# Iasonaspg/GPU-Randomized-Block-Lanczos

Measured on AMD Instinct MI355X. Metric: RBL iters/sec + time-to-k=20 eigenpairs, n=1e7 nnz/row=100 b=32; 1/2/4/8 GPU, higher is better.
Workload: dtype f64

## Files before the change

gpu-randomized-block-lanczos_amd/csrc/kernels.hpp:

```cpp
#pragma once
#include "rbl_common.hpp"

namespace rbl {

struct Panels {
  static constexpr int kMax = 2;
  const double* ptr[kMax] = {nullptr, nullptr};
  int count = 0;
  int w = 0;
};
struct PanelRun {
  const double* base = nullptr;
  const float* base32 = nullptr;
  int64_t stride = 0;
  int count = 0;
  int w = 0;
};

constexpr int64_t kCsrPad = 256;
constexpr int64_t kRowPad = 16;
constexpr int64_t kRowPad32 = 32;

struct CsrDev {
  int64_t nrows = 0;
  int64_t nnz = 0;
  const int64_t* rowptr = nullptr;
  const int32_t* col = nullptr;
  const double* val = nullptr;
  const int64_t* tile_cmin = nullptr;
  const int64_t* tile_cmax = nullptr;
  const int64_t* tile_info = nullptr;
  int64_t ntiles = 0;
  int64_t tiles_per_wg = 0;
  const int32_t* panel_blk = nullptr;
  const uint16_t* panel_cnt = nullptr;
  const uint32_t* panel_st = nullptr;
  const uint8_t* panel_col = nullptr;
  const double* panel_val = nullptr;
  int64_t panel_nblk = 0;
  int panel_rpg = 4;
  int panel_ch = 32;
  bool panel_auto = false;
  bool window_ok16 = false;
  bool window_ok32 = false;
  bool band_ok16 = false;
  bool band_ok32 = false;
  bool band_gram = false;
  bool band_pair = false;
  int64_t row0 = 0;
  const uint16_t* band_pos = nullptr;
  const double* bt = nullptr;
  int bt_ng = 0;
  int64_t bt_tiles_per_wg = 0;
  int64_t q_lo = 0, q_hi = 0;
  const double* zrow = nullptr;
  const void* qloc = nullptr;
  int64_t loc_lo = 0, loc_hi = 0;
  const double* lfix_c = nullptr;
  double* lfix_q = nullptr;
  int* two_wave = nullptr;
  int64_t lfix_lo = 0, lfix_hi = 0;
  const uint64_t* btp_hdr = nullptr;
  const double* btp_val = nullptr;
  const double* bth = nullptr;
  const double* bte = nullptr;
  int64_t seg_ntasks = 0;
  const int64_t* seg_trow = nullptr;
  const int32_t* seg_tinfo = nullptr;
  const int64_t* seg_slot_k0 = nullptr;
  int64_t seg_nlong = 0;
  const int64_t* seg_lrow = nullptr;
  const int64_t* seg_lslot = nullptr;
  double* seg_scratch = nullptr;
  int seg_ntiers = 0;
  bool seg_split = false;
  hipEvent_t seg_wait = nullptr;
  struct Tier {
    const int64_t* rowptr = nullptr;
    const int32_t* col = nullptr;
    const double* val = nullptr;
    int64_t ntasks = 0, nlong = 0;
    const int64_t* trow = nullptr;
    const int32_t* tinfo = nullptr;
    const int64_t* slot_k0 = nullptr;
    const int64_t* lrow = nullptr;
    const int64_t* lslot = nullptr;
    double* scratch = nullptr;
  } seg_tier[3];
};
constexpr int kMaxSegTiers = 3;
constexpr int64_t kSegLen = 4096;
constexpr int64_t kSegPack = 512;

bool rowgram_ok(int b);
int rowgram_grid(int64_t nrows, int per_cu = 2);
constexpr int kRowgramMaxPerCu = 4;
void rowgram(int64_t nrows, int b, const double* X, const double* C, int ldc, double* Y,
             double alpha, double beta, double* slab, int grid, const int* skip, hipStream_t s,
             const float* X32 = nullptr, float* Y32 = nullptr, const int* f64flag = nullptr,
             bool tri = false);
struct RowOpArgs {
  const double* X = nullptr;
  const double* C = nullptr;
  int ldc = 0;
  double* Y = nullptr;
  double alpha = 1.0, beta = 0.0;
  double* slab = nullptr;
  const int* skip = nullptr;
  const float* X32 = nullptr;
  float* Y32 = nullptr;
  const int* f64flag = nullptr;
  const double* C2 = nullptr;
  const double* Z = nullptr;
  double* slab2 = nullptr;
// ... 3 lines not shown
};
bool rowgram_ex(int64_t nrows, int b, const RowOpArgs& a, int grid, hipStream_t s);

int spmm(const CsrDev& A, const double* Qin, int64_t col_off, int b, double* U,
         const double* Qprev, const double* Bi, int variant, hipStream_t s,
         double* ai_slab = nullptr);

bool spmm_seg_ok(const CsrDev& A, int b);
void seg_tier_count(int64_t m, const int64_t* rowptr, const int32_t* col, const uint8_t* tier_of,
                    int ntiers, int32_t* cnt, hipStream_t s);
void seg_tier_fill(int64_t m, const int64_t* rowptr, const int32_t* col, const double* val,
                   const uint8_t* tier_of, int ntiers, int64_t* const* trp, int32_t* const* tcol,
                   double* const* tval, hipStream_t s);
struct TierRule {
  const int32_t* deg = nullptr;
  int64_t row0 = 0, r0 = 0, r1 = 0;
};
void seg_tier_count_rule(int64_t m, const int64_t* rowptr, const int32_t* col, TierRule rule,
                         int32_t* cnt, hipStream_t s);
void seg_tier_fill_rule(int64_t m, const int64_t* rowptr, const int32_t* col, const double* val,
                        TierRule rule, int64_t* const* trp, int32_t* const* tcol,
                        double* const* tval, hipStream_t s);
void spmm_seg_tier(const CsrDev::Tier& T, const double* Q, int64_t col_off, int b, double* out,
                   hipStream_t s);
void push_add(const int64_t* rows, const int64_t* ptr, const int64_t* slot, int64_t nrows,
              const double* recv, int b, double* U, hipStream_t s);
constexpr int64_t kRectSegLen = 1024;
constexpr int64_t kRectPack = 512;
int rect_transpose(int64_t rows, int64_t cols, int64_t nnz, const int64_t* ptr, const int32_t* ind,
                   const double* val, int64_t* tptr, int32_t* tind, double* tval, hipStream_t s);
void spmm_rect(const CsrDev::Tier& T, const double* Q, int b, double* out, const double* Qprev,
               const double* Bi, const double* scale, hipStream_t s, const double* sa = nullptr,
               const double* sw = nullptr);
int rect_colsum_grid(int64_t rows, int b);
void rect_colsum(int64_t rows, int b, const double* a, const double* X, double* part, double* w,
                 hipStream_t s);
bool spmm_panel(const CsrDev& A, const double* Qin, int64_t col_off, int b, double* U,
                const double* Qprev, const double* Bi, hipStream_t s);
int panel_width();
int panel_format(const CsrDev& A, const int32_t* binfo, int R, int64_t nblk, uint16_t* cnt,
                 uint32_t* st, int64_t ncnt, uint8_t* pcol, double* pval, hipStream_t s);
bool spmm_window(const CsrDev& A, const double* Qin, int64_t col_off, int b, double* U,
                 const double* Qprev, const double* Bi, hipStream_t s);
int window_grid();
void ensure_lds_attr(const void* kernel, int bytes);
bool spmm_band(const CsrDev& A, const double* Qin, int64_t col_off, int b, double* U,
               const double* Qprev, const double* Bi, hipStream_t s, double* ai_slab = nullptr,
               int* ai_parts = nullptr);
bool spmm_bt_locfix_ok(const CsrDev& A, int b);
int spmm_bt_halfwidth(const CsrDev& A);
void spmm_bt_locfix_edges(const CsrDev& A, double* Q, const double* Qprev, const double* C,
                          int64_t lo0, int64_t hi0, int64_t lo1, int64_t hi1, hipStream_t s);
void spmm_bt_locfix_rest(const CsrDev& A, double* Q, const double* Qprev, const double* C,
                         hipStream_t s);
bool spmm_bt(const CsrDev& A, const double* Qin, int64_t col_off, int b, double* U,
             const double* Qprev, const double* Bi, hipStream_t s, double* ai_slab = nullptr,
             int* ai_parts = nullptr, const float* Q32 = nullptr, const float* Qprev32 = nullptr);
int bt_half(const double* full, int64_t ntiles, int64_t tpw, int NG, double** half,
            double** edge, hipStream_t s);
int64_t bt_tile_slots(int64_t ntiles, int64_t tiles_per_wg);
void bt_fill(const CsrDev& A, int H, int NG, double* out, hipStream_t s);
constexpr int bt_pack_words(int NG) { return (4 * NG + (2 * NG + 4) / 4 + 2) & ~1; }
int bt_pack(const double* dense, int64_t nslots, int NG, uint64_t* hdr, double** val_out,
            int64_t* nval_out, hipStream_t s);
constexpr int kWindowTileRows = 16;
constexpr int kBandMaxK = 176;
constexpr int kBandLd = 196;
constexpr int kBandRing = 256;
void band_positions(const CsrDev& A, uint16_t* pos, hipStream_t s);

void cheb_axpby(int64_t len, const double* W, const double* Y, const double* Z, double alpha,
                double beta, double gamma, double* out, hipStream_t s);
void cheb_series_term(int64_t len, const double* W, const double* T1, const double* T2, double alpha,
                      double beta, double mu, double mu0, double* Tout, double* ACC, bool first,
                      bool last, hipStream_t s);
int moment_grid(int64_t nrows, int b);
void cheb_moment_term(int64_t nrows, int b, const double* W, const double* T1, const double* T2,
                      double alpha, double beta, double* Tout, double* part, int grid, bool first,
                      bool last, hipStream_t s);
int resid_grid(int64_t nrows);
void resid_partial(int64_t nrows, int kp, const double* Z, const double* X, const double* theta,
                   double* part, int grid, hipStream_t s);
void copy_cols(int64_t nrows, int w, const double* src, int lds, int s0, double* dst, int ldd, int d0,
               hipStream_t s);

int lr_padded_width(int r);
int lr_project_grid(int64_t rows, int b, int rp);
void lr_project(int64_t rows, int b, int rp, const double* P, const double* X, double* part,
                double* w, hipStream_t s);
void lr_small(int r, int rp, int b, const double* S, const double* w, double* c, hipStream_t s);
void lr_update(int64_t rows, int b, int rp, const double* P, const double* c, double* U,
               hipStream_t s);

int gram_splits(int64_t nrows, int nW, int w, int xcols);
void gram_partial(int64_t nrows, const PanelRun& W, const Panels& X, double* slab, int splits,
                  const int* skip, hipStream_t s);
void reduce_slab(const double* slab, int splits, int64_t len, double* out, const int* skip,
                 hipStream_t s);
int reduce_scratch_splits(int splits);
void reduce_slab_many(double* slab, int splits, int64_t len, double* out, hipStream_t s);
void tsmm(int64_t nrows, const PanelRun& X, const double* C, int ldc, const Panels& Y,
          double alpha, double beta, const int* skip, hipStream_t s, double* xslab = nullptr,
          int* xgrid = nullptr);

bool gram44_ok(int64_t nrows, int nW, int w, int xcount, int xw);
int gram44_splits(int64_t nrows, int nW, int w = 32);
void gram44_partial(int64_t nrows, const PanelRun& W, const Panels& X, double* slab, int splits,
                    const int* skip, hipStream_t s);
bool tsmm44_ok(int xw, int ky, int yw);
void tsmm44_f32x(int64_t nrows, const PanelRun& X, const double* C, int ldc, const Panels& Y,
                 double alpha, double beta, hipStream_t s);
int tsmm44_xg_grid(int64_t nrows);
void tsmm44(int64_t nrows, const PanelRun& X, const double* C, int ldc, const Panels& Y,
            double alpha, double beta, const int* skip, hipStream_t s, double* xslab = nullptr,
            int* xgrid = nullptr);

int gram32_splits(int64_t nrows);
void gram32_partial(int64_t nrows, const float* Wb, int64_t wstride, int nW, int w, const float* X0,
                    const float* X1, int xcount, double* slab, int splits, hipStream_t s);
void tsmm32(int64_t nrows, const float* Xb, int64_t xstride, int nX, int w, const double* C, int ldc,
            float* Y0, float* Y1, int ycount, float alpha, float beta, hipStream_t s);
void cvt_f32_to_f64(const float* src, double* dst, int64_t n, hipStream_t s);
void cvt_f64_to_f32(const double* src, float* dst, int64_t n, hipStream_t s);

void chol_step(const double* G, int b, int64_t nglobal, int mode, double* R, double* Rinv,
               double* Rtot, int* need3, int* status, const int* skip, hipStream_t s,
               double* scratch);
void copy_small(const double* src, double* dst, int64_t len, hipStream_t s, const int* skip = nullptr);
void cloc_rinv(double* C, const double* Rinv, int b, const int* skip, hipStream_t s);
void transpose_small(const double* src, double* dst, int b, hipStream_t s);
void stash_step(const double* Ai, const double* Rtot, double* Bprev, int* flags, double* stash,
                int b, hipStream_t s);

struct RmatParams {
  int64_t n = 0;
  int scale = 0;
  int64_t edges = 0;
  double a = 0.57, b = 0.19, c = 0.19;
  uint64_t seed = 0;
  bool relabel = false;
  Scatter perm;
};
constexpr uint64_t kRelabelK = 0x52454C4142454C31ull;
void rmat_degree(const RmatParams& p, int32_t* deg, hipStream_t s);
int rmat_local_csr(const RmatParams& p, int64_t r0, int64_t r1, int64_t max_keys, int nplant,
                   const double* plant_dev, int64_t* rowptr_dev, int32_t** col_dev,
                   double** val_dev, int64_t* nnz_out, hipStream_t s);
void col_footprint(const int32_t* col, int64_t nnz, const int64_t* bounds_dev, int P,
                   unsigned long long* lo, unsigned long long* hi, hipStream_t s);

void circ_count(int64_t n, int64_t width, double p, uint64_t seed, int64_t r0, int64_t r1,
                int32_t* counts, hipStream_t s);
void circ_fill(int64_t n, int64_t width, double p, uint64_t seed, int64_t r0, int64_t r1,
               const int64_t* rowptr, int nplant, const double* plant_dev, int32_t* col,
               double* val, hipStream_t s);
void gather_rows(const double* Q, const int32_t* idx, int64_t nrows, int b, double* out,
                 hipStream_t s);
void mark_cols(const int32_t* col, int64_t nnz, int64_t r0, int64_t r1, uint8_t* mark,
               hipStream_t s);
void remap_cols(int32_t* col, int64_t nnz, const int32_t* map, hipStream_t s);
void hw_count(int64_t n, int64_t W, double p, uint64_t seed, int64_t r0, int64_t r1,
              int32_t* counts, hipStream_t s);
void hw_fill(int64_t n, int64_t W, double p, uint64_t seed, int64_t r0, int64_t r1,
             const int64_t* rowptr, int nplant, const double* plant_dev, int32_t* col,
             double* val, hipStream_t s);
void randn_block(double* Q, int64_t nrows, int b, int64_t r0, uint64_t seed, hipStream_t s,
                 const Scatter* perm = nullptr);
void tile_col_range(const CsrDev& A, int tile_rows, int64_t* cmin, int64_t* cmax, hipStream_t s);
void colmajor_to_rowmajor(const double* src, int64_t nrows, int w, double* dst, hipStream_t s);
void rowmajor_to_colmajor(const double* src, int64_t nrows, int w, double* dst, hipStream_t s);

}
```

gpu-randomized-block-lanczos_amd/csrc/rbl_api.cpp:

```cpp
#include <hip/hip_runtime.h>
#include <rocprofiler-sdk-roctx/roctx.h>

#include <algorithm>
#include <cstdlib>
#include <chrono>
#include <cmath>
#include <cstdio>
#include <cstring>
#include <string>
#include <thread>
#include <vector>

#include "../../include/rbl_hip.h"
#include "comm.hpp"
#include "kernels.hpp"

using namespace rbl;

struct rbl_ctx {
  int device = 0;
  hipStream_t stream = nullptr;
  int nranks = 1, rank = 0;
  Comm* comm = nullptr;
  std::string err;
// ... 116 lines not shown
  std::vector<void*> h_spill;
  double* d_stage = nullptr;
  hipStream_t cstream = nullptr;
  hipEvent_t ev_fin = nullptr, ev_d2h[2] = {nullptr, nullptr};
  std::vector<hipEvent_t> step_ev;
  bool d2h_pending[2] = {false, false};
  float* d_basis32 = nullptr;
  float* d_stage32 = nullptr;
  double* d_Qi64 = nullptr;
  double* d_Qm64 = nullptr;
  double* d_U = nullptr;
  double* d_T = nullptr;
  int64_t T_cols = 0;
  double* d_qext = nullptr;
  size_t qext_cap = 0;
  double* d_slab = nullptr;
  size_t slab_elems = 0;
  double* d_C = nullptr;
  size_t C_elems = 0;
  double* d_small = nullptr;
  int* d_flags = nullptr;
  double* h_pin = nullptr;
  void* h_d2h[2] = {nullptr, nullptr};
  hipEvent_t ev_d2h_slot[2] = {nullptr, nullptr};
  hipStream_t rstream = nullptr;
  hipEvent_t ev_ritz[9] = {};
  double* h_hist = nullptr;
  double* d_stash = nullptr;
  bool stash_direct = true;
  double* dv_pin = nullptr;
  double* dv_hist = nullptr;
  bool flags_clean = false;
  int fetched = 1;
  bool have_bprev = false;
  double* d_lock = nullptr;
  int nlock = 0, lock_cap = 0;
  int filt_deg = 0;
  double filt_lo = 0.0, filt_hi = 0.0, filt_ref = 0.0;
  double* d_filt[3] = {nullptr, nullptr, nullptr};
  int filt_cols = 0;
  std::vector<double> ser_mu;
  double ser_lo = 0.0, ser_hi = 0.0;
  double* d_rv = nullptr;
  double* d_rw = nullptr;
  int ritz_k = 0;

  int timers = 0;
  int reorth_order = 0;
  int spmm_variant = 0;
  int fuse = 7;
  int cloc_step = 0;
  bool cloc_final = false;
  std::vector<int> step_flags;
  double stage_ms[RBL_NUM_STAGES] = {0};
  int64_t comm_stats[RBL_COMM_NSTATS] = {0};
  int64_t comm_host_ns[2] = {0, 0};
  double comm_dev_ms[2] = {0.0, 0.0};
  int64_t path_stats[RBL_PATH_NSTATS] = {0};
  struct Mark { int stage; hipEvent_t a, b; int parent = -1; };
  std::vector<Mark> marks;
  struct OpenStage { int stage; hipStream_t st; };
  std::vector<OpenStage> open_stages;
  std::vector<hipEvent_t> ev_pool;
  size_t ev_used = 0;
};

namespace {

const char* kStageNames[RBL_NUM_STAGES] = {"AQ", "3-term", "qr", "part reorth", "loc reorth",
                                           "Ritz vectors", "comm", "spill wait"};

int fail(rbl_ctx* c, int code, const std::string& msg) {
  if (c) c->err = msg;
  return code;
}

struct DevBuf {
  void* p = nullptr;
  DevBuf() = default;
  DevBuf(const DevBuf&) = delete;
  DevBuf& operator=(const DevBuf&) = delete;
  ~DevBuf() {
    if (p) (void)hipFree(p);
  }
  double* d() const { return static_cast<double*>(p); }
};

#define HIPC(expr)                                                                    \
  do {                                                                                \
    hipError_t _e = (expr);                                                           \
    if (_e != hipSuccess)                                                             \
      return fail(ctx, _e == hipErrorOutOfMemory ? RBL_ERR_OOM : RBL_ERR_HIP,          \
                  std::string(#expr) + ": " + hipGetErrorString(_e));                 \
  } while (0)
#define COMMC(expr)               \
  do {                            \
    int _s = (expr);              \
    if (_s < 0) return _s;        \
  } while (0)
#define CHK(expr)             \
  do {                        \
    int _s = (expr);          \
    if (_s < 0) return _s;    \
  } while (0)

double* slotp(rbl_ctx* ctx, int j) {
// ... 1110 lines not shown
  hipFree(ctx->d_qext);
  ctx->d_qext = nullptr;
  ctx->qext_cap = 0;
  HIPC(hipMalloc(&ctx->d_qext, need * sizeof(double)));
  HIPC(hipMemsetAsync(ctx->d_qext, 0, need * sizeof(double), st));
  ctx->qext_cap = need;
  return RBL_OK;
}

int apply_A_stored(rbl_ctx* ctx, const double* Qin, int64_t off, int b, double* U, const double* Qprev,
                   const double* Bi, double* slab, const double* qloc, const double* lfix_c,
                   double* lfix_q, int64_t lf_lo, int64_t lf_hi, hipEvent_t seg_wait) {
  if (ctx->nloc <= 0) return 0;
  if (ctx->rect) {
    CHK(ensure_rect_y(ctx, b));
    const double* Q = Qin + (0 - off) * b;
    if (ctx->rect_shift) {
      double *t = ctx->d_rect_ts, *sv = ctx->d_rect_ts + b;
      rect_colsum(ctx->n, b, ctx->d_shift_v, Q, ctx->d_rect_part, t, ctx->stream);
      spmm_rect(rect_tier(ctx, 0), Q, b, ctx->d_rect_y, nullptr, nullptr, nullptr, ctx->stream,
                ctx->d_shift_u, t);
      rect_colsum(ctx->rect_m, b, ctx->d_shift_u, ctx->d_rect_y, ctx->d_rect_part, sv, ctx->stream);
      spmm_rect(rect_tier(ctx, 1), ctx->d_rect_y, b, U, Qprev, Bi, nullptr, ctx->stream,
                ctx->d_shift_v, sv);
      ctx->path_stats[RBL_PATH_SPMM] += 1;
      return 0;
    }
    spmm_rect(rect_tier(ctx, 0), Q, b, ctx->d_rect_y, nullptr, nullptr, nullptr, ctx->stream);
    spmm_rect(rect_tier(ctx, 1), ctx->d_rect_y, b, U, Qprev, Bi, nullptr, ctx->stream);
    ctx->path_stats[RBL_PATH_SPMM] += 1;
    return 0;
  }
  if (ctx->csr_dropped && rbl_spmm_kernel_for(ctx, b) != 5)
    return fail(ctx, RBL_ERR_STATE, "the CSR was released (RBL_OPT_KEEP_CSR = 0): only the band-tile "
                                    "SpMM (b in {16, 32}) can run");
  if (!ctx->dense) {
    CsrDev A = csr(ctx);
    if (!qloc && ctx->ghost_active && ctx->nranks > 1 && rbl_spmm_kernel_for(ctx, b) == 6)
      qloc = ctx->ghost_local;
    if (qloc) {
      A.qloc = qloc;
      A.loc_lo = ctx->r0;
      A.loc_hi = ctx->r0 + ctx->nloc;
    }
    A.seg_wait = seg_wait;
    int two_wave = 0;
    A.two_wave = &two_wave;
    if (lfix_c) {
      A.lfix_c = lfix_c;
      A.lfix_q = lfix_q;
      A.lfix_lo = lf_lo;
      A.lfix_hi = lf_hi;
    }
    const int parts = spmm(A, Qin, off, b, U, Qprev, Bi, ctx->spmm_variant, ctx->stream, slab);
    if (parts < 0) return fail(ctx, RBL_ERR_INVALID, "internal: split-source SpMM needs the band-tile kernel");
    ctx->path_stats[RBL_PATH_SPMM] += 1;
    ctx->path_stats[RBL_PATH_SPMM_TWO_WAVE] += two_wave;
    if (lfix_c) {
      ctx->path_stats[RBL_PATH_SPMM_LOC_FUSED] += 1;
      ctx->path_stats[RBL_PATH_LOCFIX_REST] += 1;
      StageScope t(ctx, RBL_STAGE_LOC_REORTH);
      spmm_bt_locfix_rest(A, lfix_q, Qprev, lfix_c, ctx->stream);
    }
    return parts;
  }
  if (b > ctx->qfull_cols) {
    hipFree(ctx->d_qfull);
    ctx->d_qfull = nullptr;
    ctx->qfull_cols = 0;
    HIPC(hipMalloc(&ctx->d_qfull, (size_t)ctx->dense_panels * 32 * b * sizeof(double)));
    HIPC(hipMemsetAsync(ctx->d_qfull, 0, (size_t)ctx->dense_panels * 32 * b * sizeof(double), ctx->stream));
    ctx->qfull_cols = b;
  }
  HIPC(hipMemcpyAsync(ctx->d_qfull, Qin + (0 - off) * b, ctx->n * b * sizeof(double),
                      hipMemcpyDeviceToDevice, ctx->stream));
  PanelRun X;
  X.base = ctx->d_dense;
  X.stride = ctx->nloc * 32;
  X.w = 32;
  X.count = (int)ctx->dense_panels;
  CHK(tsmm_checked(ctx, X, ctx->d_qfull, b, pan1(U, b), 1.0, 0.0, nullptr));
  if (Qprev) {
    transpose_small(Bi, smallp(ctx, S_BT), b, ctx->stream);
    CHK(tsmm_checked(ctx, run1(Qprev, b), smallp(ctx, S_BT), b, pan1(U, b), -1.0, 1.0, nullptr));
  }
  return 0;
}

int ensure_lr_bufs(rbl_ctx* ctx, int b) {
  if (ctx->d_lr_wc && ctx->lr_cols >= b) return RBL_OK;
  HIPC(hipStreamSynchronize(ctx->stream));
  hipFree(ctx->d_lr_wc);
  hipFree(ctx->d_lr_part);
  ctx->d_lr_wc = ctx->d_lr_part = nullptr;
  ctx->lr_cols = 0;
  const size_t grid = (size_t)lr_project_grid(ctx->nloc, b, ctx->lr_rp);
  HIPC(hipMalloc(&ctx->d_lr_wc, (size_t)2 * ctx->lr_rp * b * sizeof(double)));
  HIPC(hipMalloc(&ctx->d_lr_part, grid * ctx->lr_rp * b * sizeof(double)));
  ctx->lr_cols = b;
  return RBL_OK;
}

int apply_A(rbl_ctx* ctx, const double* Qin, int64_t off, int b, double* U, const double* Qprev,
            const double* Bi, double* slab, const double* qloc = nullptr,
            const double* lfix_c = nullptr, double* lfix_q = nullptr, int64_t lf_lo = 0,
            int64_t lf_hi = 0, hipEvent_t seg_wait = nullptr) {
  if (ctx->lr_r == 0 || ctx->nloc <= 0)
    return apply_A_stored(ctx, Qin, off, b, U, Qprev, Bi, slab, qloc, lfix_c, lfix_q, lf_lo, lf_hi,
                          seg_wait);
  if (ctx->nranks > 1 || ctx->rect)
    return fail(ctx, RBL_ERR_STATE, "internal: a low-rank update needs one rank and a square A");
  CHK(ensure_lr_bufs(ctx, b));
  const int parts = apply_A_stored(ctx, Qin, off, b, U, Qprev, Bi, lfix_c ? slab : nullptr, qloc,
                                   lfix_c, lfix_q, lf_lo, lf_hi, seg_wait);
  if (parts < 0) return parts;
// ... 212 lines not shown
    PanelRun X;
    X.base32 = slotp32(ctx, 0);
    X.stride = ctx->slot;
    X.count = nres;
    X.w = b;
    tsmm44_f32x(ctx->nloc, X, d_S, kcols, pan1(Y, kcols), 1.0, 0.0, ctx->stream);
    HIPC(hipGetLastError());
    j0 = nres;
  }
  if (j0 < nblocks) CHK(ensure_qm64(ctx));
  for (int j = j0; j < nblocks; ++j) {
    int st = 0;
    const float* Qj = block_dev32(ctx, j, ctx->nblocks, &st);
    if (st) return fail(ctx, st, "Ritz: H2D of a spilled block failed");
    cvt_f32_to_f64(Qj, ctx->d_Qm64, ctx->nloc * b, ctx->stream);
    CHK(tsmm_checked(ctx, run1(ctx->d_Qm64, b), d_S + (int64_t)j * b * kcols, kcols, pan1(Y, kcols),
                     1.0, j == 0 ? 0.0 : 1.0, nullptr));
  }
  return RBL_OK;
}

int gram32(rbl_ctx* ctx, const float* Wb, int nW, const float* X0, const float* X1, int xcount,
           double* C) {
  const int b = ctx->b;
  const int splits = gram32_splits(ctx->nloc);
  const int64_t len = (int64_t)nW * b * xcount * b;
  if ((size_t)splits * len > ctx->slab_elems)
    return fail(ctx, RBL_ERR_INVALID, "internal: Gram slab too small (fp32)");
  if (ctx->nloc > 0) {
    gram32_partial(ctx->nloc, Wb, ctx->slot, nW, b, X0, X1, xcount, ctx->d_slab, splits, ctx->stream);
    reduce_slab(ctx->d_slab, splits, len, C, nullptr, ctx->stream);
  } else {
    HIPC(hipMemsetAsync(C, 0, len * sizeof(double), ctx->stream));
  }
  HIPC(hipGetLastError());
  return allreduce(ctx, C, (size_t)len);
}
int upd32(rbl_ctx* ctx, const float* Xb, int nX, const double* C, int ldc, float* Y0, float* Y1,
          int ycount) {
  if (ctx->nloc <= 0) return RBL_OK;
  tsmm32(ctx->nloc, Xb, ctx->slot, nX, ctx->b, C, ldc, Y0, Y1, ycount, -1.f, 1.f, ctx->stream);
  HIPC(hipGetLastError());
  return RBL_OK;
}

int rowop_ex(rbl_ctx* ctx, RowOpArgs a, double* G, double* Gx, bool reduce_x, bool comm_x = true) {
  const int b = ctx->b;
  const int gmax = rowgram_grid(ctx->nloc, kRowgramMaxPerCu);
  if ((size_t)2 * gmax * b * b > ctx->slab_elems)
    return fail(ctx, RBL_ERR_INVALID, "internal: row-op slab too small");
  if (G) a.slab = ctx->d_slab;
  if (a.Z) a.slab2 = ctx->d_slab + (size_t)gmax * b * b;
  const int xgrid = rowgram_grid(ctx->nloc, 2);
  int grid = a.Z ? xgrid : 0;
  a.grid_out = &grid;
  if (ctx->nloc > 0) {
    if (!rowgram_ex(ctx->nloc, b, a, grid, ctx->stream))
      return fail(ctx, RBL_ERR_INVALID, "internal: unsupported fused row-op form");
  } else {
    grid = 1;
    if (G) HIPC(hipMemsetAsync(a.slab, 0, (size_t)b * b * sizeof(double), ctx->stream));
    if (a.Z && a.skip == nullptr)
      HIPC(hipMemsetAsync(a.slab2, 0, (size_t)xgrid * b * b * sizeof(double), ctx->stream));
  }
  HIPC(hipGetLastError());
  if (G) {
    reduce_slab(ctx->d_slab, grid, (int64_t)b * b, G, a.skip, ctx->stream);
    CHK(allreduce(ctx, G, (size_t)b * b));
  }
  if (Gx && reduce_x) {
    reduce_slab(ctx->d_slab + (size_t)gmax * b * b, xgrid, (int64_t)b * b, Gx, nullptr, ctx->stream);
    if (comm_x) CHK(allreduce(ctx, Gx, (size_t)b * b));
  }
  return RBL_OK;
}

int tsqr(rbl_ctx* ctx, const double* U, double* Qout, bool g1_ready = false, float* Qout32 = nullptr,
         const double* Zloc = nullptr) {
  StageScope t(ctx, RBL_STAGE_QR);
  ctx->flags_clean = false;
  const int b = ctx->b;
  int* need3 = ctx->d_flags;
  int* status = ctx->d_flags + 2;
  double* G = smallp(ctx, S_G);
  const int* skip3 = need3 + 1;
  const bool fused = rowgram_ok(b);
  auto apply_inplace = [&](const int* skip) -> int {
    if (b <= 64)
      return tsmm_checked(ctx, run1(Qout, b), smallp(ctx, S_RINV), b, pan1(Qout, b), 1.0, 0.0, skip);
    CHK(tsmm_checked(ctx, run1(Qout, b), smallp(ctx, S_RINV), b, pan1(ctx->d_T, b), 1.0, 0.0, skip));
    copy_small(ctx->d_T, Qout, ctx->nloc * b, ctx->stream, skip);
    return RBL_OK;
  };
  const bool three = fused && (ctx->fuse & 1);
  if (!g1_ready) CHK(gram(ctx, run1(U, b), pan1(U, b), G, nullptr));
  chol_step(G, b, ctx->n, 0, smallp(ctx, S_R), smallp(ctx, three ? S_RINV1 : S_RINV), smallp(ctx, S_RTOT),
            need3, status, nullptr, ctx->stream, smallp(ctx, S_CHS0));
  if (three) {
    RowOpArgs a1;
    a1.X = U;
    a1.C = smallp(ctx, S_RINV1);
    a1.ldc = b;
    a1.mode = 1;
    a1.tri = true;
    CHK(rowop_ex(ctx, a1, G, nullptr, false));
    chol_step(G, b, ctx->n, 1, smallp(ctx, S_R), smallp(ctx, S_RINV), smallp(ctx, S_RTOT), need3,
              status, nullptr, ctx->stream, smallp(ctx, S_CHS0));
    RowOpArgs a2;
    a2.X = U;
    a2.C = smallp(ctx, S_RINV1);
    a2.C2 = smallp(ctx, S_RINV);
    a2.ldc = b;
    a2.tri = true;
    a2.Y = Qout;
    a2.Y32 = Qout32;
    a2.f64flag = Qout32 ? need3 : nullptr;
    a2.Z = Zloc;
    a2.mode = 2;
    CHK(rowop_ex(ctx, a2, nullptr, Zloc ? smallp(ctx, S_CLOC) : nullptr, Zloc != nullptr, false));
    CHK(gram(ctx, run1(Qout, b), pan1(Qout, b), G, skip3, Zloc == nullptr));
    if (Zloc) CHK(allreduce(ctx, G, (size_t)2 * b * b));
    chol_step(G, b, ctx->n, 1, smallp(ctx, S_R), smallp(ctx, S_RINV), smallp(ctx, S_RTOT), need3,
              status, skip3, ctx->stream, smallp(ctx, S_CHS0));
    RowOpArgs a3;
    a3.X = Qout;
    a3.C = smallp(ctx, S_RINV);
    a3.ldc = b;
    a3.tri = true;
    a3.Y = Qout;
    a3.skip = skip3;
    a3.Y32 = Qout32;
    a3.mode = 0;
    CHK(rowop_ex(ctx, a3, nullptr, nullptr, false));
    if (Zloc) cloc_rinv(smallp(ctx, S_CLOC), smallp(ctx, S_RINV), b, skip3, ctx->stream);
    HIPC(hipGetLastError());
    return RBL_OK;
  }
  if (Zloc) return fail(ctx, RBL_ERR_INVALID, "internal: local-reorth Gram fusion needs the 3-pass QR");
  if (fused) {
    CHK(rowop(ctx, U, smallp(ctx, S_RINV), Qout, 1.0, 0.0, G, nullptr, nullptr, nullptr, nullptr, true));
  } else {
    CHK(tsmm_checked(ctx, run1(U, b), smallp(ctx, S_RINV), b, pan1(Qout, b), 1.0, 0.0, nullptr));
    CHK(gram(ctx, run1(Qout, b), pan1(Qout, b), G, nullptr));
  }
  chol_step(G, b, ctx->n, 1, smallp(ctx, S_R), smallp(ctx, S_RINV), smallp(ctx, S_RTOT), need3,
            status, nullptr, ctx->stream, smallp(ctx, S_CHS0));
  if (fused) {
    CHK(rowop(ctx, Qout, smallp(ctx, S_RINV), Qout, 1.0, 0.0, G, nullptr, nullptr, Qout32,
              Qout32 ? need3 : nullptr, true));
  } else {
    CHK(apply_inplace(nullptr));
    CHK(gram(ctx, run1(Qout, b), pan1(Qout, b), G, skip3));
  }
  chol_step(G, b, ctx->n, 1, smallp(ctx, S_R), smallp(ctx, S_RINV), smallp(ctx, S_RTOT), need3,
            status, skip3, ctx->stream, smallp(ctx, S_CHS0));
  if (fused) {
    CHK(rowop(ctx, Qout, smallp(ctx, S_RINV), Qout, 1.0, 0.0, nullptr, skip3, nullptr, Qout32,
              nullptr, true));
  } else {
    CHK(apply_inplace(skip3));
    if (Qout32) cvt_f64_to_f32(Qout, Qout32, ctx->nloc * b, ctx->stream);
  }
  HIPC(hipGetLastError());
  return RBL_OK;
}

int halo_exchange(rbl_ctx* ctx, const double* Q, const double** Qin, int64_t* off,
                  bool copy_local = true, hipStream_t st = nullptr) {
  if (ctx->nranks == 1) {
    *Qin = Q;
    *off = 0;
    return RBL_OK;
  }
  if (!st) st = ctx->stream;
  StageScope t(ctx, RBL_STAGE_COMM, st);
  const int b = ctx->b;
  CHK(ensure_qext(ctx, b, st));
  double* ext = ctx->d_qext;
  ctx->ghost_active = use_ghost(ctx, b);
  if (ctx->ghost_active) {
    gather_rows(Q, ctx->d_send_idx, ctx->n_send, b, ctx->d_sendbuf, st);
    HIPC(hipGetLastError());
    std::vector<Comm::Xfer> x(ctx->nranks);
    for (int q = 0; q < ctx->nranks; ++q) {
      if (q == ctx->rank) continue;
      x[q].send = ctx->d_sendbuf + ctx->send_off[q] * b;
      x[q].nsend = (size_t)ctx->send_cnt[q] * b;
      x[q].recv = ext + ctx->ghost_off[q] * b;
      x[q].nrecv = (size_t)ctx->ghost_cnt[q] * b;
    }
    CHK(exchange(ctx, x, st));
    ctx->ghost_local = Q;
    *Qin = ext;
    *off = 0;
    return RBL_OK;
  }
  if (copy_local)
    HIPC(hipMemcpyAsync(ext + (ctx->r0 - ctx->ext_lo) * b, Q, ctx->nloc * b * sizeof(double),
                        hipMemcpyDeviceToDevice, st));
  std::vector<Comm::Xfer> x(ctx->nranks);
  for (int q = 0; q < ctx->nranks; ++q) {
    if (q == ctx->rank) continue;
    const int64_t gl = ctx->give_lo[q], gh = ctx->give_hi[q];
    if (gh > gl) {
      x[q].send = Q + (gl - ctx->r0) * b;
      x[q].nsend = (size_t)(gh - gl) * b;
    }
    const int64_t nl = ctx->need_lo[q], nh = ctx->need_hi[q];
    if (nh > nl) {
      x[q].recv = ext + (nl - ctx->ext_lo) * b;
      x[q].nrecv = (size_t)(nh - nl) * b;
    }
  }
  CHK(exchange(ctx, x, st));
  *Qin = ext;
  *off = ctx->ext_lo;
  return RBL_OK;
}

// ... 76 lines not shown
  return RBL_OK;
}

int push_products(rbl_ctx* ctx, const double* Q, int b, hipStream_t st) {
  StageScope t(ctx, RBL_STAGE_AQ, st);
  CHK(ensure_push(ctx, b));
  const auto& P = ctx->push_tier;
  CsrDev::Tier T;
  T.rowptr = P.rowptr;
  T.col = P.col;
  T.val = P.val;
  T.ntasks = P.ntasks;
  T.nlong = P.nlong;
  T.trow = P.trow;
  T.tinfo = P.tinfo;
  T.slot_k0 = P.slot_k0;
  T.lrow = P.lrow;
  T.lslot = P.lslot;
  T.scratch = P.scratch;
  spmm_seg_tier(T, Q, ctx->r0, b, ctx->d_pushbuf, st);
  HIPC(hipGetLastError());
  return RBL_OK;
}

int push_exchange(rbl_ctx* ctx, int b, hipStream_t st) {
  StageScope t(ctx, RBL_STAGE_COMM, st);
  std::vector<Comm::Xfer> x(ctx->nranks);
  for (int q = 0; q < ctx->nranks; ++q) {
    if (q == ctx->rank) continue;
    x[q].send = ctx->d_pushbuf + ctx->ghost_off[q] * b;
    x[q].nsend = (size_t)ctx->ghost_cnt[q] * b;
    x[q].recv = ctx->d_precv + ctx->send_off[q] * b;
    x[q].nrecv = (size_t)ctx->send_cnt[q] * b;
  }
  CHK(exchange(ctx, x, st));
  return RBL_OK;
}

int push_finish(rbl_ctx* ctx, double* U, int b, hipStream_t st) {
  StageScope t(ctx, RBL_STAGE_AQ, st);
  push_add(ctx->d_ps_rows, ctx->d_ps_ptr, ctx->d_ps_slot, ctx->n_ps_rows, ctx->d_precv, b, U, st);
  HIPC(hipGetLastError());
  return RBL_OK;
}

int push_halo(rbl_ctx* ctx, const double* Q, int b, double* U) {
  if (!push_on(ctx)) return RBL_OK;
  CHK(push_products(ctx, Q, b, ctx->stream));
  CHK(push_exchange(ctx, b, ctx->stream));
  return push_finish(ctx, U, b, ctx->stream);
}

void free_run(rbl_ctx* ctx) {
  if (ctx->cstream) hipStreamSynchronize(ctx->cstream);
  hipFree(ctx->d_basis); ctx->d_basis = nullptr;
  for (void* h : ctx->h_spill)
    if (h) hipHostFree(h);
  ctx->h_spill.clear();
  hipFree(ctx->d_stage); ctx->d_stage = nullptr;
  ctx->resident = INT32_MAX;
  ctx->d2h_pending[0] = ctx->d2h_pending[1] = false;
  hipFree(ctx->d_basis32); ctx->d_basis32 = nullptr;
  hipFree(ctx->d_stage32); ctx->d_stage32 = nullptr;
  hipFree(ctx->d_Qi64); ctx->d_Qi64 = nullptr;
  hipFree(ctx->d_Qm64); ctx->d_Qm64 = nullptr;
  ctx->basis_bits = 64;
  hipFree(ctx->d_U); ctx->d_U = nullptr;
  hipFree(ctx->d_T); ctx->d_T = nullptr;
  hipFree(ctx->d_qext); ctx->d_qext = nullptr; ctx->qext_cap = 0;
  hipFree(ctx->d_sendbuf); ctx->d_sendbuf = nullptr;
  if (ctx->hstream) hipStreamSynchronize(ctx->hstream);
  hipFree(ctx->d_pushbuf); ctx->d_pushbuf = nullptr;
  hipFree(ctx->d_precv); ctx->d_precv = nullptr;
  ctx->push_cap = 0;
  hipFree(ctx->d_slab); ctx->d_slab = nullptr;
  hipFree(ctx->d_C); ctx->d_C = nullptr;
  hipFree(ctx->d_small); ctx->d_small = nullptr;
  hipFree(ctx->d_flags); ctx->d_flags = nullptr;
  hipFree(ctx->d_lock); ctx->d_lock = nullptr;
  ctx->nlock = ctx->lock_cap = 0;
  hipFree(ctx->d_filt[0]); hipFree(ctx->d_filt[1]); hipFree(ctx->d_filt[2]);
  ctx->d_filt[0] = ctx->d_filt[1] = ctx->d_filt[2] = nullptr;
  ctx->filt_cols = 0;
  hipFree(ctx->d_rv); ctx->d_rv = nullptr;
  hipFree(ctx->d_rw); ctx->d_rw = nullptr;
  ctx->ritz_k = 0;
  if (ctx->h_pin) hipHostFree(ctx->h_pin);
  ctx->h_pin = nullptr;
  if (ctx->h_hist) hipHostFree(ctx->h_hist);
  ctx->h_hist = nullptr;
  hipFree(ctx->d_stash);
  ctx->d_stash = nullptr;
  ctx->dv_pin = ctx->dv_hist = nullptr;
  ctx->nblocks = 0;
  ctx->b = 0;
  ctx->have_bprev = false;
}

void free_rect_shift(rbl_ctx* ctx) {
  hipFree(ctx->d_shift_u); ctx->d_shift_u = nullptr;
  hipFree(ctx->d_shift_v); ctx->d_shift_v = nullptr;
  hipFree(ctx->d_rect_ts); ctx->d_rect_ts = nullptr;
  hipFree(ctx->d_rect_part); ctx->d_rect_part = nullptr;
  ctx->rect_ts_cols = 0;
  ctx->rect_shift = false;
}
// ... 331 lines not shown
  const char* name = "none";
  if (ctx->comm) {
    hipSetDevice(ctx->device);
    const int s = ctx->comm->count(&cnt, &ctx->err);
    if (s < 0) return s;
    name = ctx->comm->name();
  }
  *nranks = cnt;
  *rank = ctx->rank;
  if (transport && transport_len > 0) snprintf(transport, (size_t)transport_len, "%s", name);
  return RBL_OK;
}

int rbl_rccl_version(int* version, char* path, int path_len) {
  if (!version) return RBL_ERR_INVALID;
  std::string p, err;
  const int s = rbl::rccl_library(version, &p, &err);
  if (path && path_len > 0) snprintf(path, (size_t)path_len, "%s", s ? err.c_str() : p.c_str());
  return s ? RBL_ERR_RCCL : RBL_OK;
}

int rbl_set_option(rbl_ctx* ctx, int option, int64_t value) {
  if (!ctx) return RBL_ERR_INVALID;
  switch (option) {
    case RBL_OPT_TIMERS:
      if (value < 0 || value > 2) return fail(ctx, RBL_ERR_INVALID, "RBL_OPT_TIMERS: 0, 1 or 2");
      ctx->timers = (int)value;
      return RBL_OK;
    case RBL_OPT_REORTH_ORDER:
      if (value < 0 || value > 1) return fail(ctx, RBL_ERR_INVALID, "reorth order must be 0|1");
      ctx->reorth_order = (int)value;
      return RBL_OK;
    case RBL_OPT_DEVICE_BLOCKS:
      if (value < -1 || value == 1 || value == 2 || value > INT32_MAX)
        return fail(ctx, RBL_ERR_INVALID, "device blocks: 0 (all), -1 (auto) or >= 3");
      ctx->dev_blocks_opt = (int)value;
      return RBL_OK;
    case RBL_OPT_SPMM_KERNEL:
      if (value < 0 || value > 7 || value == 4)
        return fail(ctx, RBL_ERR_INVALID, "spmm kernel must be 0 (auto) or a kernel id 1, 2, 3, 5, 6, 7");
      ctx->spmm_variant = value == 5 ? 4 : value == 6 ? 5 : (int)value;
      return RBL_OK;
    case RBL_OPT_SPLIT_HALO: ctx->split_halo = value != 0; return RBL_OK;
    case RBL_OPT_HALO_OVERLAP: ctx->halo_overlap = value != 0; return RBL_OK;
    case RBL_OPT_HALO_PUSH:
      if (value < 0 || value > 2) return fail(ctx, RBL_ERR_INVALID, "RBL_OPT_HALO_PUSH must be 0|1|2");
      ctx->halo_push_opt = (int)value;
      return RBL_OK;
    case RBL_OPT_KEEP_CSR: ctx->keep_csr = value != 0; return RBL_OK;
    case RBL_OPT_RELABEL:
      if (value < 0 || value > 1) return fail(ctx, RBL_ERR_INVALID, "RBL_OPT_RELABEL must be 0|1");
      ctx->relabel_opt = (int)value;
      return RBL_OK;
    case RBL_OPT_FUSE:
      if (value < 0 || value > 7) return fail(ctx, RBL_ERR_INVALID, "RBL_OPT_FUSE is a 3-bit mask");
      ctx->fuse = (int)value;
      return RBL_OK;
    default: return fail(ctx, RBL_ERR_INVALID, "unknown option");
  }
}

int rbl_set_matrix_csc(rbl_ctx* ctx, int64_t n, int64_t nnz, const int64_t* colptr,
                       const int64_t* rowval, const double* nzval, int index_base) {
  if (!ctx || n < 1 || nnz < 0 || !colptr || (nnz && (!rowval || !nzval)) ||
      (index_base != 0 && index_base != 1))
    return fail(ctx, RBL_ERR_INVALID, "rbl_set_matrix_csc: bad arguments");
  if (colptr[n] - colptr[0] != nnz) return fail(ctx, RBL_ERR_INVALID, "colptr[n] != nnz");
  HIPC(hipSetDevice(ctx->device));
  std::vector<int64_t> rp(n + 1);
  for (int64_t i = 0; i <= n; ++i) rp[i] = colptr[i] - colptr[0];
  ctx->bounds.assign(ctx->nranks + 1, 0);
  rbl_plan_row_partition(n, rp.data(), ctx->nranks, ctx->bounds.data());
  const int64_t r0 = ctx->bounds[ctx->rank], r1 = ctx->bounds[ctx->rank + 1];
  return upload_csr(ctx, n, r0, r1, colptr + r0, rowval, nzval, index_base, index_base);
}

int rbl_set_matrix_csr_rows(rbl_ctx* ctx, int64_t n, int64_t row_begin, int64_t row_end,
                            const int64_t* rowptr, const int64_t* colind, const double* val,
                            int index_base) {
  if (!ctx || n < 1 || row_begin < 0 || row_end < row_begin || row_end > n || !rowptr ||
      (index_base != 0 && index_base != 1))
    return fail(ctx, RBL_ERR_INVALID, "rbl_set_matrix_csr_rows: bad arguments");
  HIPC(hipSetDevice(ctx->device));
  if (ctx->nranks > 1) {
    int64_t mine[2] = {row_begin, row_end};
    std::vector<int64_t> all(2 * ctx->nranks);
    COMMC(ctx->comm->allgather_host(mine, all.data(), 2, ctx->stream, &ctx->err));
    ctx->bounds.assign(ctx->nranks + 1, 0);
    for (int p = 0; p < ctx->nranks; ++p) {
      if (all[2 * p] != (p == 0 ? 0 : all[2 * p - 1]))
        return fail(ctx, RBL_ERR_INVALID, "row slices must tile [0,n) in rank order");
      ctx->bounds[p + 1] = all[2 * p + 1];
    }
    if (ctx->bounds[ctx->nranks] != n) return fail(ctx, RBL_ERR_INVALID, "row slices != n");
  } else {
    if (row_begin != 0 || row_end != n)
      return fail(ctx, RBL_ERR_INVALID, "single rank must own all rows");
    ctx->bounds = {0, n};
  }
  return upload_csr(ctx, n, row_begin, row_end, rowptr, colind, val, index_base, index_base);
}

int rbl_set_matrix_dense(rbl_ctx* ctx, int64_t n, int64_t row_begin, int64_t row_end,
                         const double* A, int64_t lda) {
  if (!ctx || n < 1 || row_begin < 0 || row_end < row_begin || row_end > n || !A ||
      lda < row_end - row_begin || lda < 1)
// ... 501 lines not shown
    double* keep_send = ctx->d_sendbuf;
    const int keep_b = ctx->b;
    ctx->d_qext = ext.d();
    ctx->qext_cap = (size_t)ext_rows * b;
    ctx->d_sendbuf = sendbuf.d();
    ctx->b = b;
    const int st = halo_exchange(ctx, xr.d(), &Qin, &off);
    ctx->d_qext = keep_ext;
    ctx->qext_cap = keep_cap;
    ctx->d_sendbuf = keep_send;
    ctx->b = keep_b;
    if (st < 0) return st;
  }
  {
    const int st = apply_A(ctx, Qin, off, b, y.d(), nullptr, nullptr, nullptr);
    if (st < 0) return st;
  }
  HIPC(hipGetLastError());
  CHK(push_halo(ctx, xr.d(), b, y.d()));
  rowmajor_to_colmajor(y.d(), ctx->nloc, b, x.d(), ctx->stream);
  HIPC(hipMemcpyAsync(Y, x.p, ctx->nloc * b * sizeof(double), hipMemcpyDeviceToHost, ctx->stream));
  HIPC(hipStreamSynchronize(ctx->stream));
  return RBL_OK;
}

int rbl_start(rbl_ctx* ctx, int b, int max_blocks, int basis_bits, const double* omega,
              uint64_t seed) {
  if (!ctx) return RBL_ERR_INVALID;
  if (!has_matrix(ctx)) return fail(ctx, RBL_ERR_STATE, "rbl_start: no matrix");
  if (b < 1 || b > RBL_MAX_BLOCK)
    return fail(ctx, RBL_ERR_INVALID, "block size must be in [1," + std::to_string(RBL_MAX_BLOCK) + "]");
  if (max_blocks < 1) return fail(ctx, RBL_ERR_INVALID, "max_blocks must be >= 1");
  if (basis_bits != 64 && basis_bits != 32)
    return fail(ctx, RBL_ERR_INVALID, "basis_bits must be 64 or 32");
  if (ctx->rect && basis_bits != 64)
    return fail(ctx, RBL_ERR_INVALID, "rbl_start: a rectangular B (rbl_set_matrix_normal) needs the "
                                      "fp64 basis (basis_bits = 64)");
  if (ctx->filt_deg > 0 && basis_bits != 64)
    return fail(ctx, RBL_ERR_INVALID, "rbl_start: a Chebyshev filter (rbl_set_filter) needs the fp64 "
                                      "basis (basis_bits = 64)");
  if (ctx->filt_deg > 0 && (ctx->rect || ctx->nranks > 1))
    return fail(ctx, RBL_ERR_INVALID, "rbl_start: a Chebyshev filter (rbl_set_filter) runs on one rank "
                                      "and a square A only");
  if (ctx->lr_r > 0 && basis_bits != 64)
    return fail(ctx, RBL_ERR_INVALID, "rbl_start: a low-rank update (rbl_set_lowrank) needs the fp64 "
                                      "basis (basis_bits = 64)");
  if (has_series(ctx) && basis_bits != 64)
    return fail(ctx, RBL_ERR_INVALID, "rbl_start: a Chebyshev series (rbl_set_filter_series) needs the "
                                      "fp64 basis (basis_bits = 64)");
  if (has_series(ctx) && (ctx->rect || ctx->nranks > 1))
    return fail(ctx, RBL_ERR_INVALID, "rbl_start: a Chebyshev series (rbl_set_filter_series) runs on "
                                      "one rank and a square A only");
  HIPC(hipSetDevice(ctx->device));
  HIPC(hipStreamSynchronize(ctx->stream));
  int dev_slots = max_blocks + 1;
  const bool same_shape = (ctx->d_basis || ctx->d_basis32) && ctx->b == b &&
                          ctx->max_blocks == max_blocks && ctx->slot == ctx->nloc * b &&
                          ctx->basis_bits == basis_bits;
  const int cur_slots = ctx->resident == INT32_MAX ? ctx->max_blocks + 1 : ctx->resident + 2;
  if (ctx->dev_blocks_opt < 0 && same_shape && ctx->auto_planned) {
    dev_slots = cur_slots;
  } else if (ctx->dev_blocks_opt != 0) {
    int g = ctx->dev_blocks_opt;
    if (g < 0) {
      size_t fr = 0, tot = 0;
      HIPC(hipMemGetInfo(&fr, &tot));
      const double blk64 = (double)std::max<int64_t>(ctx->nloc, 1) * b * 8.0;
      const double blk = blk64 * (basis_bits == 64 ? 1.0 : 0.5);
      const double mine = ctx->d_basis ? (double)(ctx->resident == INT32_MAX ? ctx->max_blocks + 1 : ctx->resident + 2) * blk64
                        : ctx->d_basis32 ? (double)(ctx->resident == INT32_MAX ? ctx->max_blocks + 1 : ctx->resident + 2) * blk64 * 0.5
                        : 0.0;
      const double work = 2.0 + (ctx->nranks > 1 ? 1.0 : 0.0) +
                          (basis_bits == 32 ? 1.0 + (direct32_ok(ctx, b) ? 0.0 : 1.0) : 0.0);
      const double other = work * blk64 + blk + 8.0 * (double)gram_slab_elems(ctx, b, max_blocks, basis_bits);
      g = (int)std::max(3.0, std::floor((0.8 * ((double)fr + mine) - other) / blk));
    }
    dev_slots = std::min(dev_slots, std::max(3, g));
  }
  const bool reuse = same_shape && cur_slots == dev_slots;
  ctx->nlock = 0;
  ctx->cloc_step = 0;
  ctx->step_flags.clear();
  const int alloc_st = [&]() -> int {
  if (reuse) {
    ctx->nblocks = 0;
    if (ctx->cstream) HIPC(hipStreamSynchronize(ctx->cstream));
    ctx->d2h_pending[0] = ctx->d2h_pending[1] = false;
    HIPC(hipMemsetAsync(ctx->d_flags, 0, 4 * sizeof(int), ctx->stream));
  } else {
  free_run(ctx);
  ctx->b = b;
  ctx->max_blocks = max_blocks;
  ctx->slot = ctx->nloc * b;
  const int64_t nl = std::max<int64_t>(ctx->nloc, 1);
  ctx->basis_bits = basis_bits;
  ctx->auto_planned = ctx->dev_blocks_opt < 0;
  if (basis_bits == 64) {
    HIPC(hipMalloc(&ctx->d_basis, (size_t)dev_slots * nl * b * sizeof(double)));
    if (dev_slots < max_blocks + 1) {
      ctx->resident = dev_slots - 2;
      ctx->h_spill.assign(max_blocks + 1 - ctx->resident, nullptr);
      HIPC(hipMalloc(&ctx->d_stage, (size_t)nl * b * sizeof(double)));
      if (!ctx->cstream) {
        HIPC(hipStreamCreateWithFlags(&ctx->cstream, hipStreamNonBlocking));
        HIPC(hipEventCreateWithFlags(&ctx->ev_fin, hipEventDisableTiming));
        HIPC(hipEventCreateWithFlags(&ctx->ev_d2h[0], hipEventDisableTiming));
        HIPC(hipEventCreateWithFlags(&ctx->ev_d2h[1], hipEventDisableTiming));
      }
    }
  } else {
    const size_t bytes32 = ((size_t)dev_slots * nl + kRowPad32) * b * sizeof(float);
    HIPC(hipMalloc(&ctx->d_basis32, bytes32));
    HIPC(hipMemsetAsync(ctx->d_basis32, 0, bytes32, ctx->stream));
    if (dev_slots < max_blocks + 1) {
      ctx->resident = dev_slots - 2;
      ctx->h_spill.assign(max_blocks + 1 - ctx->resident, nullptr);
      HIPC(hipMalloc(&ctx->d_stage32, ((size_t)nl + kRowPad32) * b * sizeof(float)));
      HIPC(hipMemsetAsync(ctx->d_stage32, 0, ((size_t)nl + kRowPad32) * b * sizeof(float), ctx->stream));
      if (!ctx->cstream) {
        HIPC(hipStreamCreateWithFlags(&ctx->cstream, hipStreamNonBlocking));
        HIPC(hipEventCreateWithFlags(&ctx->ev_fin, hipEventDisableTiming));
        HIPC(hipEventCreateWithFlags(&ctx->ev_d2h[0], hipEventDisableTiming));
        HIPC(hipEventCreateWithFlags(&ctx->ev_d2h[1], hipEventDisableTiming));
      }
    }
    HIPC(hipMalloc(&ctx->d_Qi64, (nl + kRowPad) * b * sizeof(double)));
    if (!direct32_ok(ctx, b)) HIPC(hipMalloc(&ctx->d_Qm64, (nl + kRowPad) * b * sizeof(double)));
  }
  HIPC(hipMalloc(&ctx->d_U, (nl + kRowPad) * b * sizeof(double)));
  ctx->T_cols = b;
  HIPC(hipMalloc(&ctx->d_T, nl * b * sizeof(double)));
  if (ctx->nranks > 1) {
    CHK(ensure_qext(ctx, b, ctx->stream));
    if (ctx->ghost)
      HIPC(hipMalloc(&ctx->d_sendbuf, std::max<int64_t>(ctx->n_send, 1) * b * sizeof(double)));
  }
  const size_t slab = gram_slab_elems(ctx, b, max_blocks, basis_bits);
  ctx->slab_elems = slab;
  HIPC(hipMalloc(&ctx->d_slab, slab * sizeof(double)));
  ctx->C_elems = (size_t)std::max(1, max_blocks) * b * 2 * b;
  HIPC(hipMalloc(&ctx->d_C, ctx->C_elems * sizeof(double)));
  HIPC(hipMalloc(&ctx->d_small, (size_t)S_NSMALL * b * b * sizeof(double)));
  HIPC(hipMalloc(&ctx->d_flags, 4 * sizeof(int)));
  HIPC(hipMemset(ctx->d_flags, 0, 4 * sizeof(int)));
  {
#ifdef RBL_VARIANTS
    const char* e = std::getenv("RBL_STASH_COPY");
    ctx->stash_direct = !(e && std::atoi(e) == 1);
#else
    ctx->stash_direct = true;
#endif
    const unsigned hf = ctx->stash_direct ? (hipHostMallocMapped | hipHostMallocCoherent) : hipHostMallocDefault;
    HIPC(hipHostMalloc(&ctx->h_pin, stash_rec(b) * sizeof(double), hf));
    HIPC(hipHostMalloc(&ctx->h_hist, (size_t)(max_blocks + 2) * stash_rec(b) * sizeof(double), hf));
    if ((size_t)ctx->nloc * b * sizeof(double) >= 4 * kD2HPiece && !d2h_direct()) {
      CHK(ensure_d2h_slots(ctx));
      CHK(ensure_ritz_stream(ctx));
    }
    if (ctx->stash_direct) {
      HIPC(hipHostGetDevicePointer(reinterpret_cast<void**>(&ctx->dv_pin), ctx->h_pin, 0));
      HIPC(hipHostGetDevicePointer(reinterpret_cast<void**>(&ctx->dv_hist), ctx->h_hist, 0));
    } else {
      HIPC(hipMalloc(&ctx->d_stash, stash_rec(b) * sizeof(double)));
    }
  }
  }
  if (ctx->push && ctx->nranks > 1 && use_ghost(ctx, b)) {
    const char* inj = std::getenv("RBL_FAULT_PUSH_ALLOC");
    if (inj && *inj && std::atoi(inj) == ctx->rank)
      return fail(ctx, RBL_ERR_OOM, "rbl_start: push buffers (injected by RBL_FAULT_PUSH_ALLOC)");
    CHK(ensure_push(ctx, b));
  }
  if (has_filter(ctx)) CHK(ensure_filter_bufs(ctx, b));
  return RBL_OK;
  }();
  if (ctx->nranks > 1) {
    const int64_t mine = alloc_st;
    std::vector<int64_t> all(ctx->nranks);
    COMMC(ctx->comm->allgather_host(&mine, all.data(), 1, ctx->stream, &ctx->err));
    int bad = -1;
    for (int q = 0; q < ctx->nranks && bad < 0; ++q)
      if (all[q] != RBL_OK) bad = q;
    if (bad >= 0) {
      (void)hipGetLastError();
      free_run(ctx);
      if (alloc_st != RBL_OK) return alloc_st;
      return fail(ctx, (int)all[bad], "rbl_start: rank " + std::to_string(bad) +
                                          " could not allocate its run buffers");
    }
  } else if (alloc_st != RBL_OK) {
    (void)hipGetLastError();
    return alloc_st;
  }

  if (omega) {
    double* d_tmp = ctx->d_U;
    HIPC(hipMemcpyAsync(d_tmp, omega, ctx->nloc * b * sizeof(double), hipMemcpyHostToDevice,
// ... 39 lines not shown
    return fail(ctx, RBL_ERR_STATE, "rbl_step: rbl_fetch the asynchronous steps first");
  const int rc = step_impl(ctx, i, part_reorth, A_out, B_out, false);
  if (ctx && rc >= 0) ctx->fetched = ctx->nblocks;
  return rc;
}
int rbl_step_async(rbl_ctx* ctx, int i, int part_reorth) {
  return step_impl(ctx, i, part_reorth, nullptr, nullptr, true);
}
int rbl_fetch(rbl_ctx* ctx, int i0, int i1, double* A_out, double* B_out, int* status_out) {
  if (!ctx) return RBL_ERR_INVALID;
  if (i0 != ctx->fetched || i1 < i0 || i1 > ctx->nblocks)
    return fail(ctx, RBL_ERR_INVALID, "rbl_fetch: [i0, i1) must start at the first unfetched step");
  HIPC(hipSetDevice(ctx->device));
  const int last = i1 - 1;
  if (last >= 1 && last < (int)ctx->step_ev.size() && ctx->step_ev[last])
    HIPC(hipEventSynchronize(ctx->step_ev[last]));
  else
    HIPC(hipStreamSynchronize(ctx->stream));
  harvest_timers(ctx);
  const int b = ctx->b;
  int rc = RBL_OK;
  for (int j = i0; j < i1; ++j) {
    const double* h = ctx->h_hist + (size_t)j * stash_rec(b);
    const int* fl = reinterpret_cast<const int*>(h + 2 * b * b);
    double* A = A_out ? A_out + (size_t)(j - i0) * b * b : nullptr;
    double* B = B_out ? B_out + (size_t)(j - i0) * b * b : nullptr;
    for (int r = 0; r < b; ++r)
      for (int c = 0; c < b; ++c) {
        if (A) A[c * b + r] = h[r * b + c];
        if (B) B[c * b + r] = h[b * b + r * b + c];
      }
    const int st = fl[2] ? RBL_ERR_NUMERIC : fl[3] ? RBL_WARN_QR_SHIFTED : RBL_OK;
    if (status_out) status_out[j - i0] = st;
    if (st == RBL_ERR_NUMERIC && rc >= 0) rc = fail(ctx, RBL_ERR_NUMERIC, "QR breakdown (shifted CholQR failed)");
  }
  ctx->fetched = i1;
  return rc;
}
namespace {
int step_impl(rbl_ctx* ctx, int i, int part_reorth, double* A_out, double* B_out, bool async) {
  if (!ctx) return RBL_ERR_INVALID;
  if ((!ctx->d_basis && !ctx->d_basis32) || ctx->nblocks < 1) return fail(ctx, RBL_ERR_STATE, "rbl_step before rbl_start");
  if (i != ctx->nblocks) return fail(ctx, RBL_ERR_STATE, "rbl_step: i must equal the current block count");
  if (i > ctx->max_blocks) return fail(ctx, RBL_ERR_STATE, "rbl_step: basis full (max_blocks)");
  HIPC(hipSetDevice(ctx->device));
  const int b = ctx->b;
  const bool f32 = ctx->basis_bits == 32;
  if (!ctx->flags_clean) HIPC(hipMemsetAsync(ctx->d_flags, 0, 4 * sizeof(int), ctx->stream));
  ctx->flags_clean = false;
  if (f32 && (part_reorth & 2))
    return fail(ctx, RBL_ERR_INVALID, "rbl_step: locked-vector reorth needs the fp64 basis");
  const bool direct32 = f32 && i >= 2 && direct32_ok(ctx, b);
  if (f32 && !direct32) CHK(ensure_qm64(ctx));
  double* Qi = f32 ? ctx->d_Qi64 : slotp(ctx, i - 1);
  double* Qm = i >= 2 ? (f32 ? ctx->d_Qm64 : slotp(ctx, i - 2)) : nullptr;
  float* Qi32 = f32 ? slotp32(ctx, i - 1) : nullptr;
  float* Qm32 = f32 && i >= 2 ? slotp32(ctx, i - 2) : nullptr;
  if (f32) {
    if ((part_reorth & 1) && i >= 3) {
      StageScope t(ctx, RBL_STAGE_PART_REORTH);
      const int nW = i - 2;
      const int nres = std::min(nW, ctx->resident);
      if (ctx->reorth_order == 0) {
        CHK(gram32(ctx, slotp32(ctx, 0), nres, Qi32, Qm32, 2, ctx->d_C));
        CHK(upd32(ctx, slotp32(ctx, 0), nres, ctx->d_C, 2 * b, Qi32, Qm32, 2));
      } else {
        for (int j = 0; j < nres; ++j) {
          CHK(gram32(ctx, slotp32(ctx, j), 1, Qi32, Qm32, 2, ctx->d_C));
          CHK(upd32(ctx, slotp32(ctx, j), 1, ctx->d_C, 2 * b, Qi32, Qm32, 2));
        }
      }
      for (int j = nres; j < nW; ++j) {
        int st = 0;
        const float* Wj = block_dev32(ctx, j, i, &st);
        if (st) return fail(ctx, st, "partial reorth: H2D of a spilled block failed");
        CHK(gram32(ctx, Wj, 1, Qi32, Qm32, 2, ctx->d_C));
        CHK(upd32(ctx, Wj, 1, ctx->d_C, 2 * b, Qi32, Qm32, 2));
      }
    }
    if (spilled(ctx) && i >= 2 && i - 2 >= ctx->resident) {
      HIPC(hipEventRecord(ctx->ev_fin, ctx->stream));
      HIPC(hipStreamWaitEvent(ctx->cstream, ctx->ev_fin, 0));
      CHK(spill_slot(ctx, i - 2, sizeof(float)));
      HIPC(hipMemcpyAsync(ctx->h_spill[i - 2 - ctx->resident], Qm32,
                          ctx->slot * sizeof(float), hipMemcpyDeviceToHost, ctx->cstream));
      HIPC(hipEventRecord(ctx->ev_d2h[i & 1], ctx->cstream));
      ctx->d2h_pending[i & 1] = true;
    }
    if (i >= 2) {
      StageScope t(ctx, RBL_STAGE_LOC_REORTH);
      CHK(gram32(ctx, Qm32, 1, Qi32, nullptr, 1, ctx->d_C));
      CHK(upd32(ctx, Qm32, 1, ctx->d_C, b, Qi32, nullptr, 1));
      if (!direct32) {
        cvt_f32_to_f64(Qi32, ctx->d_Qi64, ctx->nloc * b, ctx->stream);
        cvt_f32_to_f64(Qm32, ctx->d_Qm64, ctx->nloc * b, ctx->stream);
      }
      HIPC(hipGetLastError());
    }
  }

  if (!f32) CHK(reorth_pair(ctx, i, part_reorth));
  if (!f32 && spilled(ctx) && i >= 2 && i - 2 >= ctx->resident) {
    HIPC(hipEventRecord(ctx->ev_fin, ctx->stream));
    HIPC(hipStreamWaitEvent(ctx->cstream, ctx->ev_fin, 0));
    CHK(spill_slot(ctx, i - 2, sizeof(double)));
    HIPC(hipMemcpyAsync(ctx->h_spill[i - 2 - ctx->resident], slotp(ctx, i - 2),
// ... 54 lines not shown
      CHK(tsmm_checked(ctx, run1(Qm, b), smallp(ctx, S_BT), b, pan1(ctx->d_U, b), -1.0, 1.0, nullptr));
    }
    HIPC(hipGetLastError());
  } else {
    const double* Qin = nullptr;
    const float* Qin32 = nullptr;
    int64_t off = 0;
    const int kid = rbl_spmm_kernel_for(ctx, b);
    const bool seg_split = !direct32 && kid == 6 && ctx->seg_split;
    const bool split = ctx->nranks > 1 && !ctx->dense &&
                       (direct32 || kid == 5 || seg_split) && ctx->split_halo;
    const bool overlap = split && seg_split && ctx->halo_overlap;
    hipEvent_t halo_ev = nullptr;
    if (overlap) {
      if (!ctx->hstream) {
        HIPC(hipStreamCreateWithFlags(&ctx->hstream, hipStreamNonBlocking));
        HIPC(hipEventCreateWithFlags(&ctx->ev_qready, hipEventDisableTiming));
        HIPC(hipEventCreateWithFlags(&ctx->ev_halo, hipEventDisableTiming));
      }
      HIPC(hipEventRecord(ctx->ev_qready, ctx->stream));
      HIPC(hipStreamWaitEvent(ctx->hstream, ctx->ev_qready, 0));
      CHK(halo_exchange(ctx, Qi, &Qin, &off, false, ctx->hstream));
      HIPC(hipEventRecord(ctx->ev_halo, ctx->hstream));
      halo_ev = ctx->ev_halo;
      if (push_on(ctx)) {
        if (!ctx->ev_push_ready) {
          HIPC(hipEventCreateWithFlags(&ctx->ev_push_ready, hipEventDisableTiming));
          HIPC(hipEventCreateWithFlags(&ctx->ev_push_done, hipEventDisableTiming));
        }
        CHK(push_products(ctx, Qi, b, ctx->stream));
        HIPC(hipEventRecord(ctx->ev_push_ready, ctx->stream));
        HIPC(hipStreamWaitEvent(ctx->hstream, ctx->ev_push_ready, 0));
        CHK(push_exchange(ctx, b, ctx->hstream));
        HIPC(hipEventRecord(ctx->ev_push_done, ctx->hstream));
        pushed = true;
      }
    } else if (direct32) {
      CHK(halo_exchange32(ctx, Qi32, &Qin32, &off, !split));
    } else {
      CHK(halo_exchange(ctx, Qi, &Qin, &off, !split));
    }
    StageScope t(ctx, RBL_STAGE_AQ);
    if (direct32) {
      CsrDev A = csr(ctx);
      if (split) {
        A.qloc = Qi32;
        A.loc_lo = ctx->r0;
        A.loc_hi = ctx->r0 + ctx->nloc;
      }
      if (!spmm_bt(A, nullptr, off, b, ctx->d_U, nullptr, smallp(ctx, S_BPREV), ctx->stream,
                   ctx->d_slab, &ai_parts, Qin32, Qm32))
        return fail(ctx, RBL_ERR_INVALID, "internal: fp32 band-tile SpMM not applicable");
    } else {
      ai_parts = apply_A(ctx, Qin, off, b, ctx->d_U, Qm, i >= 2 ? smallp(ctx, S_BPREV) : nullptr,
                         ctx->d_slab, split ? Qi : nullptr, Cloc, Qi, lf_lo, lf_hi, halo_ev);
    }
    if (ai_parts < 0) return ai_parts;
    HIPC(hipGetLastError());
    if (halo_ev) HIPC(hipStreamWaitEvent(ctx->stream, halo_ev, 0));
  }
  if (pushed) {
    HIPC(hipStreamWaitEvent(ctx->stream, ctx->ev_push_done, 0));
    CHK(push_finish(ctx, ctx->d_U, b, ctx->stream));
  } else if (!direct32 && ai_parts == 0) {
    CHK(push_halo(ctx, Qi, b, ctx->d_U));
  }
  {
    StageScope t(ctx, RBL_STAGE_3TERM);
    if (ai_parts > 0) {
      reduce_slab(ctx->d_slab, ai_parts, (int64_t)b * b, smallp(ctx, S_AI), nullptr, ctx->stream);
      HIPC(hipGetLastError());
      CHK(allreduce(ctx, smallp(ctx, S_AI), (size_t)b * b));
    } else {
      CHK(gram(ctx, run1(Qi, b), pan1(ctx->d_U, b), smallp(ctx, S_AI), nullptr));
    }
    if (fused)
      CHK(rowop(ctx, Qi, smallp(ctx, S_AI), ctx->d_U, -1.0, 1.0, smallp(ctx, S_G), nullptr,
                direct32 ? Qi32 : nullptr));
    else
      CHK(tsmm_checked(ctx, run1(Qi, b), smallp(ctx, S_AI), b, pan1(ctx->d_U, b), -1.0, 1.0, nullptr));
  }
  if (ctx->d2h_pending[i & 1]) {
    StageScope t(ctx, RBL_STAGE_SPILL_WAIT);
    HIPC(hipStreamWaitEvent(ctx->stream, ctx->ev_d2h[i & 1], 0));
    ctx->d2h_pending[i & 1] = false;
  }
  if (!f32) {
    const int guess = i >= 2 ? ctx->step_flags[i - 1] : 0;
    const bool zfuse = fused && (ctx->fuse & 3) == 3 && !modifies(i + 1, guess) && i + 1 <= ctx->max_blocks;
    CHK(tsqr(ctx, ctx->d_U, slotp(ctx, i), fused, nullptr, zfuse ? Qi : nullptr));
    if (zfuse) {
      ctx->cloc_step = i + 1;
      ctx->cloc_final = false;
    }
  } else {
    CHK(tsqr(ctx, ctx->d_U, ctx->d_Qi64, fused, slotp32(ctx, i)));
  }
  const size_t rec = stash_rec(b);
  double* rec_dev = !ctx->stash_direct ? ctx->d_stash
                    : async            ? ctx->dv_hist + (size_t)i * rec
                                       : ctx->dv_pin;
  stash_step(smallp(ctx, S_AI), smallp(ctx, S_RTOT), smallp(ctx, S_BPREV), ctx->d_flags, rec_dev,
             b, ctx->stream);
  ctx->flags_clean = true;
  if (async) {
    if (!ctx->stash_direct)
      HIPC(hipMemcpyAsync(ctx->h_hist + (size_t)i * rec, ctx->d_stash, rec * sizeof(double),
                          hipMemcpyDeviceToHost, ctx->stream));
    if ((int)ctx->step_ev.size() <= i) ctx->step_ev.resize(i + 1, nullptr);
    if (!ctx->step_ev[i]) HIPC(hipEventCreateWithFlags(&ctx->step_ev[i], hipEventDisableTiming));
    HIPC(hipEventRecord(ctx->step_ev[i], ctx->stream));
    HIPC(hipGetLastError());
    ctx->nblocks = i + 1;
    return RBL_OK;
  }
  if (!ctx->stash_direct)
    HIPC(hipMemcpyAsync(ctx->h_pin, ctx->d_stash, rec * sizeof(double), hipMemcpyDeviceToHost, ctx->stream));
  HIPC(hipStreamSynchronize(ctx->stream));
  int flags[4];
  memcpy(flags, ctx->h_pin + 2 * b * b, sizeof(flags));
  harvest_timers(ctx);
  for (int r = 0; r < b; ++r)
    for (int c = 0; c < b; ++c) {
      if (A_out) A_out[c * b + r] = ctx->h_pin[r * b + c];
      if (B_out) B_out[c * b + r] = ctx->h_pin[b * b + r * b + c];
    }
  ctx->nblocks = i + 1;
  if (flags[2]) return fail(ctx, RBL_ERR_NUMERIC, "QR breakdown (shifted CholQR failed)");
  return flags[3] ? RBL_WARN_QR_SHIFTED : RBL_OK;
}
int d2h_staged(rbl_ctx* ctx, void* dst, const void* src, size_t bytes) {
  if (bytes < 4 * kD2HPiece || d2h_direct()) {
    HIPC(hipMemcpyAsync(dst, src, bytes, hipMemcpyDeviceToHost, ctx->stream));
    return RBL_OK;
  }
  CHK(ensure_d2h_slots(ctx));
  const unsigned hw = std::max(1u, std::thread::hardware_concurrency());
  const char* envt = std::getenv("RBL_D2H_THREADS");
  const int nthr = (int)std::min(envt ? std::max(1u, (unsigned)atoi(envt)) : 8u, hw);
  auto host_copy = [&](size_t p) {
    const size_t off = p * kD2HPiece, len = std::min(kD2HPiece, bytes - off);
    char* d = static_cast<char*>(dst) + off;
    const char* s = static_cast<const char*>(ctx->h_d2h[p & 1]);
    const size_t part = ((len + nthr - 1) / nthr + 4095) & ~size_t(4095);
    std::vector<std::thread> th;
    for (size_t o = part; o < len; o += part)
// ... 61 lines not shown
    while (p + 1 < kRitzPieces && (size_t)r0p[p + 1] * kcp * sizeof(double) <= o) ++p;
    return p;
  };
  auto scatter = [&](size_t q, size_t a, size_t e) {
    const char* slot = static_cast<const char*>(ctx->h_d2h[q & 1]);
    const size_t base = q * kD2HPiece;
    for (size_t o = base + a; o < base + e;) {
      const int p = piece_of(o);
      const int64_t r0 = r0p[p], m = r0p[p + 1] - r0;
      const size_t colb = (size_t)m * sizeof(double);
      const size_t within = o - (size_t)r0 * kcp * sizeof(double);
      const size_t c = within / colb, inr = within % colb;
      const size_t run = std::min(base + e, o + (colb - inr));
      if ((int)c < k)
        memcpy(reinterpret_cast<char*>(V_out + (int64_t)c * nl + r0) + inr, slot + (o - base), run - o);
      o = run;
    }
  };
  const unsigned hw = std::max(1u, std::thread::hardware_concurrency());
  const char* envt = std::getenv("RBL_D2H_THREADS");
  const int nthr = (int)std::min(envt ? std::max(1u, (unsigned)atoi(envt)) : 8u, hw);
  const size_t nq = (bytes + kD2HPiece - 1) / kD2HPiece;
  int waited = -1;
  for (size_t q = 0; q <= nq; ++q) {
    if (q < nq) {
      const size_t off = q * kD2HPiece, len = std::min(kD2HPiece, bytes - off);
      for (const int pl = piece_of(off + len - 1); waited < pl;)
        HIPC(hipEventSynchronize(ctx->ev_ritz[++waited]));
      HIPC(hipMemcpyAsync(ctx->h_d2h[q & 1], src + off, len, hipMemcpyDeviceToHost, ctx->stream));
      HIPC(hipEventRecord(ctx->ev_d2h_slot[q & 1], ctx->stream));
    }
    if (q > 0) {
      const size_t pq = q - 1, len = std::min(kD2HPiece, bytes - pq * kD2HPiece);
      HIPC(hipEventSynchronize(ctx->ev_d2h_slot[pq & 1]));
      const size_t part = ((len + nthr - 1) / nthr + 4095) & ~size_t(4095);
      std::vector<std::thread> th;
      for (size_t o = part; o < len; o += part)
        th.emplace_back([=, &scatter] { scatter(pq, o, std::min(len, o + part)); });
      scatter(pq, 0, std::min(part, len));
      for (auto& t : th) t.join();
    }
  }
  HIPC(hipStreamSynchronize(ctx->rstream));
  HIPC(hipStreamSynchronize(ctx->stream));
  return RBL_OK;
}
}

int rbl_ritz(rbl_ctx* ctx, int nblocks, int k, const double* S, double* V_out) {
  if (!ctx || nblocks < 1 || k < 1 || !S) return fail(ctx, RBL_ERR_INVALID, "rbl_ritz: bad arguments");
  if (nblocks > ctx->nblocks) return fail(ctx, RBL_ERR_INVALID, "rbl_ritz: more blocks than computed");
  if (k > nblocks * ctx->b) return fail(ctx, RBL_ERR_INVALID, "rbl_ritz: k > nblocks*b");
  HIPC(hipSetDevice(ctx->device));
  const int b = ctx->b;
  const int64_t rows = (int64_t)nblocks * b;
  const int64_t nl = std::max<int64_t>(ctx->nloc, 1);
  size_t free_b = 0, total_b = 0;
  HIPC(hipMemGetInfo(&free_b, &total_b));
  int kc = std::min(k, 64);
  auto chunk_bytes = [&](int w) { return (double)((w + 1) & ~1) * (double)(rows + 2 * nl) * 8.0; };
  while (kc > 1 && chunk_bytes(kc) > 0.7 * (double)free_b) kc = (kc + 1) / 2;
  const int kcp = (kc + 1) & ~1;
  if (chunk_bytes(kc) > 0.7 * (double)free_b)
    return fail(ctx, RBL_ERR_OOM, "rbl_ritz: no room for one Ritz column");
#ifdef RBL_VARIANTS
  const bool trace = std::getenv("RBL_RITZ_TRACE") != nullptr;
#else
  const bool trace = false;
#endif
  auto tnow = [] { return std::chrono::duration<double, std::milli>(
                       std::chrono::steady_clock::now().time_since_epoch()).count(); };
  const double t0 = trace ? tnow() : 0.0;
  double t_alloc = 0.0, t_comp = 0.0, t_d2h = 0.0;
  DevBuf own_S, own_V, own_Vcm;
  double *pS = nullptr, *pV = nullptr, *pVcm = nullptr;
  if (kcp <= b && ctx->d_U && ctx->d_T && ctx->d_C && (size_t)rows * kcp <= ctx->C_elems) {
    pS = ctx->d_C;
    pV = ctx->d_U;
    pVcm = ctx->d_T;
  } else {
    HIPC(hipMalloc(&own_S.p, rows * kcp * sizeof(double)));
    HIPC(hipMalloc(&own_V.p, nl * kcp * sizeof(double)));
    HIPC(hipMalloc(&own_Vcm.p, nl * kcp * sizeof(double)));
    pS = own_S.d();
    pV = own_V.d();
    pVcm = own_Vcm.d();
  }
  if (trace) t_alloc = tnow() - t0;
  const bool pipelined = V_out && ctx->nloc > 0 && kc >= k && pV == ctx->d_U &&
                         (ctx->basis_bits == 64 || tsmm44_ok(b, kcp, kcp)) &&
                         nblocks <= ctx->resident && ctx->nloc >= 64 * kRitzPieces &&
                         (size_t)ctx->nloc * kcp * sizeof(double) >= 4 * kD2HPiece &&
                         !d2h_direct() && !ritz_serial();
  std::vector<double> srm((size_t)rows * kcp);
  if (pipelined) {
    for (int64_t r = 0; r < rows; ++r)
      for (int c = 0; c < kcp; ++c) srm[(size_t)r * kcp + c] = c < k ? S[(size_t)c * rows + r] : 0.0;
    HIPC(hipMemcpyAsync(pS, srm.data(), rows * kcp * sizeof(double), hipMemcpyHostToDevice, ctx->stream));
    ctx->path_stats[RBL_PATH_RITZ_PIECES] += 1;
    CHK(ritz_pipelined(ctx, nblocks, k, kcp, pS, pV, pVcm, V_out));
    harvest_timers(ctx);
    if (trace) fprintf(stderr, "rbl_ritz: pipelined, %d row pieces, total %.2f ms\n", kRitzPieces, tnow() - t0);
    return RBL_OK;
  }
  for (int c0 = 0; c0 < k; c0 += kc) {
    const int w = std::min(kc, k - c0);
// ... 328 lines not shown
    m[2] = 2.0 * d[col] - m0;
    for (int j = 2; j <= degree; ++j) {
      const double* dj = d.data() + (size_t)3 * b + (size_t)(j - 2) * 2 * b;
      m[2 * j] = 2.0 * dj[col] - m0;
      m[2 * j - 1] = 2.0 * dj[b + col] - m1;
    }
  }
  return RBL_OK;
}

int rbl_bench_moment_pass(rbl_ctx* ctx, int64_t len_rows, int b, int reps, double* ms) {
  if (!ctx || len_rows < 1 || b < 1 || b > RBL_MAX_BLOCK || reps < 1 || !ms)
    return fail(ctx, RBL_ERR_INVALID, "rbl_bench_moment_pass: bad arguments");
  HIPC(hipSetDevice(ctx->device));
  const int grid = moment_grid(len_rows, b);
  DevBuf w, t1, t2, slab, dots;
  const size_t bytes = (size_t)len_rows * b * sizeof(double);
  for (DevBuf* p : {&w, &t1, &t2}) {
    HIPC(hipMalloc(&p->p, bytes));
    HIPC(hipMemsetAsync(p->p, 0, bytes, ctx->stream));
  }
  HIPC(hipMalloc(&slab.p, (size_t)grid * 2 * b * sizeof(double)));
  HIPC(hipMalloc(&dots.p, (size_t)2 * b * sizeof(double)));
  hipEvent_t e0 = nullptr, e1 = nullptr;
  HIPC(hipEventCreate(&e0));
  HIPC(hipEventCreate(&e1));
  auto pass = [&] {
    cheb_moment_term(len_rows, b, w.d(), t1.d(), t2.d(), 0.5, 0.25, w.d(), slab.d(), grid, false, false,
                     ctx->stream);
    reduce_slab(slab.d(), grid, (int64_t)2 * b, dots.d(), nullptr, ctx->stream);
  };
  int st = RBL_OK;
  pass();
  if (hipEventRecord(e0, ctx->stream) != hipSuccess) st = RBL_ERR_HIP;
  for (int r = 0; r < reps; ++r) pass();
  if (hipEventRecord(e1, ctx->stream) != hipSuccess || hipEventSynchronize(e1) != hipSuccess) st = RBL_ERR_HIP;
  float el = 0.f;
  if (hipEventElapsedTime(&el, e0, e1) != hipSuccess || hipGetLastError() != hipSuccess) st = RBL_ERR_HIP;
  *ms = (double)el / reps;
  (void)hipEventDestroy(e0);
  (void)hipEventDestroy(e1);
  if (st != RBL_OK) return fail(ctx, st, "rbl_bench_moment_pass: a HIP call failed");
  return RBL_OK;
}

int rbl_ritz_project(rbl_ctx* ctx, int nblocks, int k, const double* S, double* H_out) {
  if (!ctx || nblocks < 1 || k < 1 || !S || !H_out)
    return fail(ctx, RBL_ERR_INVALID, "rbl_ritz_project: bad arguments");
  if (k > RBL_MAX_BLOCK)
    return fail(ctx, RBL_ERR_INVALID, "rbl_ritz_project: k must be <= " + std::to_string(RBL_MAX_BLOCK));
  if (ctx->nranks > 1) return fail(ctx, RBL_ERR_INVALID, "rbl_ritz_project: one rank only");
  if (!ctx->d_basis && !ctx->d_basis32) return fail(ctx, RBL_ERR_STATE, "rbl_ritz_project before rbl_start");
  if (nblocks > ctx->nblocks) return fail(ctx, RBL_ERR_INVALID, "rbl_ritz_project: more blocks than computed");
  if (k > nblocks * ctx->b) return fail(ctx, RBL_ERR_INVALID, "rbl_ritz_project: k > nblocks*b");
  HIPC(hipSetDevice(ctx->device));
  HIPC(hipStreamSynchronize(ctx->stream));
  hipFree(ctx->d_rv);
  hipFree(ctx->d_rw);
  ctx->d_rv = ctx->d_rw = nullptr;
  ctx->ritz_k = 0;
  const int b = ctx->b;
  const int kp = (k + 1) & ~1;
  const int64_t rows = (int64_t)nblocks * b;
  const int64_t nl = std::max<int64_t>(ctx->nloc, 1);
  const size_t vbytes = (size_t)(nl + kRowPad) * kp * sizeof(double);
  HIPC(hipMalloc(&ctx->d_rv, vbytes));
  HIPC(hipMalloc(&ctx->d_rw, vbytes));
  HIPC(hipMemsetAsync(ctx->d_rv, 0, vbytes, ctx->stream));
  HIPC(hipMemsetAsync(ctx->d_rw, 0, vbytes, ctx->stream));
  std::vector<double> srm((size_t)rows * kp);
  for (int64_t r = 0; r < rows; ++r)
    for (int c = 0; c < kp; ++c) srm[(size_t)r * kp + c] = c < k ? S[(size_t)c * rows + r] : 0.0;
  DevBuf dS;
  HIPC(hipMalloc(&dS.p, rows * kp * sizeof(double)));
  HIPC(hipMemcpyAsync(dS.p, srm.data(), rows * kp * sizeof(double), hipMemcpyHostToDevice, ctx->stream));
  {
    StageScope t(ctx, RBL_STAGE_RITZ);
    if (ctx->basis_bits == 64) CHK(combine_blocks(ctx, nblocks, kp, dS.d(), ctx->d_rv));
    else CHK(combine_blocks32(ctx, nblocks, kp, dS.d(), ctx->d_rv));
  }
  {
    StageScope t(ctx, RBL_STAGE_AQ);
    const int cw = (b == 16 || b == 32) ? b : kp;
    if (cw == kp) {
      const int st = apply_A(ctx, ctx->d_rv, 0, kp, ctx->d_rw, nullptr, nullptr, nullptr);
      if (st < 0) return st;
    } else {
      const size_t cbytes = (size_t)(nl + kRowPad) * cw * sizeof(double);
      DevBuf xc, yc;
      HIPC(hipMalloc(&xc.p, cbytes));
      HIPC(hipMalloc(&yc.p, cbytes));
      HIPC(hipMemsetAsync(xc.p, 0, cbytes, ctx->stream));
      HIPC(hipMemsetAsync(yc.p, 0, cbytes, ctx->stream));
      for (int c0 = 0; c0 < kp; c0 += cw) {
        const int w = std::min(cw, kp - c0);
        if (w < cw && c0 > 0) HIPC(hipMemsetAsync(xc.p, 0, cbytes, ctx->stream));
        copy_cols(ctx->nloc, w, ctx->d_rv, kp, c0, xc.d(), cw, 0, ctx->stream);
        const int st = apply_A(ctx, xc.d(), 0, cw, yc.d(), nullptr, nullptr, nullptr);
        if (st < 0) return st;
        copy_cols(ctx->nloc, w, yc.d(), cw, 0, ctx->d_rw, kp, c0, ctx->stream);
      }
      HIPC(hipGetLastError());
      HIPC(hipStreamSynchronize(ctx->stream));
    }
    HIPC(hipGetLastError());
  }
  std::vector<double> h((size_t)kp * kp, 0.0);
  if (ctx->nloc > 0) {
    StageScope t(ctx, RBL_STAGE_RITZ);
    const int splits = gram_splits(ctx->nloc, 1, kp, kp);
    DevBuf slab, dH;
    HIPC(hipMalloc(&slab.p, (size_t)splits * kp * kp * sizeof(double)));
    HIPC(hipMalloc(&dH.p, (size_t)kp * kp * sizeof(double)));
    gram_partial(ctx->nloc, run1(ctx->d_rv, kp), pan1(ctx->d_rw, kp), slab.d(), splits, nullptr, ctx->stream);
    reduce_slab(slab.d(), splits, (int64_t)kp * kp, dH.d(), nullptr, ctx->stream);
    HIPC(hipGetLastError());
    HIPC(hipMemcpyAsync(h.data(), dH.p, (size_t)kp * kp * sizeof(double), hipMemcpyDeviceToHost, ctx->stream));
    HIPC(hipStreamSynchronize(ctx->stream));
  }
  HIPC(hipStreamSynchronize(ctx->stream));
  harvest_timers(ctx);
  for (int r = 0; r < k; ++r)
    for (int c = 0; c < k; ++c) H_out[(size_t)c * k + r] = h[(size_t)r * kp + c];
  ctx->ritz_k = k;
  return RBL_OK;
}

int rbl_ritz_finish(rbl_ctx* ctx, int k, const double* Y, const double* theta, double* V_out,
                    double* resid_out) {
  if (!ctx || k < 1 || !Y || !theta) return fail(ctx, RBL_ERR_INVALID, "rbl_ritz_finish: bad arguments");
  if (!ctx->d_rv || !ctx->d_rw || ctx->ritz_k != k)
    return fail(ctx, RBL_ERR_STATE, "rbl_ritz_finish: no rbl_ritz_project of this k precedes it");
  return rbl_ritz_finish_cols(ctx, k, k, Y, theta, V_out, resid_out);
}

int rbl_ritz_finish_cols(rbl_ctx* ctx, int kproj, int k, const double* Y, const double* theta,
                         double* V_out, double* resid_out) {
  if (!ctx || k < 1 || kproj < k || !Y || !theta)
    return fail(ctx, RBL_ERR_INVALID, "rbl_ritz_finish_cols: bad arguments (needs 1 <= k <= kproj)");
  if (!ctx->d_rv || !ctx->d_rw || ctx->ritz_k != kproj)
    return fail(ctx, RBL_ERR_STATE, "rbl_ritz_finish_cols: no rbl_ritz_project of this kproj precedes it");
  HIPC(hipSetDevice(ctx->device));
  const int kpr = (kproj + 1) & ~1;
  const int kp = (k + 1) & ~1;
  const int64_t nl = std::max<int64_t>(ctx->nloc, 1);
  std::vector<double> yrm((size_t)kpr * kp, 0.0), th(kp, 0.0), res(kp, 0.0);
  for (int r = 0; r < kproj; ++r)
    for (int c = 0; c < k; ++c) yrm[(size_t)r * kp + c] = Y[(size_t)c * kproj + r];
  for (int c = 0; c < k; ++c) th[c] = theta[c];
  const int grid = resid_grid(ctx->nloc);
  DevBuf dY, dTh, X, Z, part, dres;
  HIPC(hipMalloc(&dY.p, (size_t)kpr * kp * sizeof(double)));
  HIPC(hipMalloc(&dTh.p, kp * sizeof(double)));
  HIPC(hipMalloc(&X.p, (size_t)nl * kp * sizeof(double)));
  HIPC(hipMalloc(&Z.p, (size_t)nl * kp * sizeof(double)));
  HIPC(hipMalloc(&part.p, (size_t)grid * kp * sizeof(double)));
  HIPC(hipMalloc(&dres.p, kp * sizeof(double)));
  HIPC(hipMemcpyAsync(dY.p, yrm.data(), (size_t)kpr * kp * sizeof(double), hipMemcpyHostToDevice, ctx->stream));
  HIPC(hipMemcpyAsync(dTh.p, th.data(), kp * sizeof(double), hipMemcpyHostToDevice, ctx->stream));
  if (ctx->nloc > 0) {
    StageScope t(ctx, RBL_STAGE_RITZ);
    CHK(tsmm_checked(ctx, run1(ctx->d_rv, kpr), dY.d(), kp, pan1(X.d(), kp), 1.0, 0.0, nullptr));
    CHK(tsmm_checked(ctx, run1(ctx->d_rw, kpr), dY.d(), kp, pan1(Z.d(), kp), 1.0, 0.0, nullptr));
    resid_partial(ctx->nloc, kp, Z.d(), X.d(), dTh.d(), part.d(), grid, ctx->stream);
    reduce_slab(part.d(), grid, kp, dres.d(), nullptr, ctx->stream);
    HIPC(hipGetLastError());
    HIPC(hipMemcpyAsync(res.data(), dres.p, kp * sizeof(double), hipMemcpyDeviceToHost, ctx->stream));
    if (V_out) {
      rowmajor_to_colmajor(X.d(), ctx->nloc, kp, ctx->d_rw, ctx->stream);
      HIPC(hipGetLastError());
      CHK(d2h_staged(ctx, V_out, ctx->d_rw, (size_t)ctx->nloc * k * sizeof(double)));
    }
  }
  HIPC(hipStreamSynchronize(ctx->stream));
  harvest_timers(ctx);
  if (resid_out)
    for (int c = 0; c < k; ++c) resid_out[c] = std::sqrt(res[c]);
  hipFree(ctx->d_rv);
  hipFree(ctx->d_rw);
  ctx->d_rv = ctx->d_rw = nullptr;
  ctx->ritz_k = 0;
  return RBL_OK;
}

int rbl_get_block(rbl_ctx* ctx, int j, double* Q_out) {
  if (!ctx || j < 1 || j > ctx->nblocks || !Q_out) return fail(ctx, RBL_ERR_INVALID, "rbl_get_block: bad block");
  HIPC(hipSetDevice(ctx->device));
  const int b = ctx->b;
  int st = 0;
  const double* src = ctx->basis_bits == 64 ? block_dev(ctx, j - 1, ctx->nblocks, &st) : nullptr;
  if (st) return fail(ctx, st, "rbl_get_block: H2D of a spilled block failed");
  if (ctx->basis_bits == 32) {
    CHK(ensure_qm64(ctx));
    const float* s32 = block_dev32(ctx, j - 1, ctx->nblocks, &st);
    if (st) return fail(ctx, st, "rbl_get_block: H2D of a spilled block failed");
    cvt_f32_to_f64(s32, ctx->d_Qm64, ctx->nloc * b, ctx->stream);
    src = ctx->d_Qm64;
  }
  rowmajor_to_colmajor(src, ctx->nloc, b, ctx->d_T, ctx->stream);
  HIPC(hipMemcpyAsync(Q_out, ctx->d_T, ctx->nloc * b * sizeof(double), hipMemcpyDeviceToHost,
                      ctx->stream));
  HIPC(hipStreamSynchronize(ctx->stream));
  return RBL_OK;
}

int rbl_num_blocks(rbl_ctx* ctx) { return ctx ? ctx->nblocks : 0; }

int rbl_restart(rbl_ctx* ctx, int nblocks, const double* S) {
  if (ctx) ctx->cloc_step = 0;
  if (!ctx || !S || nblocks < 1 || nblocks > ctx->nblocks)
    return fail(ctx, RBL_ERR_INVALID, "rbl_restart: bad arguments");
  if (!ctx->d_basis) return fail(ctx, RBL_ERR_STATE, "rbl_restart: needs an fp64 run (rbl_start)");
  if (spilled(ctx)) return fail(ctx, RBL_ERR_STATE, "rbl_restart: needs an HBM-resident basis");
  HIPC(hipSetDevice(ctx->device));
  const int b = ctx->b;
  CHK(basis_combine(ctx, nblocks, b, S, ctx->d_T));
  HIPC(hipMemcpyAsync(slotp(ctx, 0), ctx->d_T, ctx->nloc * b * sizeof(double),
                      hipMemcpyDeviceToDevice, ctx->stream));
  HIPC(hipMemsetAsync(ctx->d_flags, 0, 4 * sizeof(int), ctx->stream));
  HIPC(hipStreamSynchronize(ctx->stream));
  ctx->nblocks = 1;
  ctx->fetched = 1;
  return RBL_OK;
}

int rbl_lock(rbl_ctx* ctx, int nblocks, int nvec, const double* S) {
  if (ctx) ctx->cloc_step = 0;
  if (!ctx || !S || nblocks < 1 || nblocks > ctx->nblocks || nvec < 0)
    return fail(ctx, RBL_ERR_INVALID, "rbl_lock: bad arguments");
  if (!ctx->d_basis) return fail(ctx, RBL_ERR_STATE, "rbl_lock: needs an fp64 run (rbl_start)");
  if (spilled(ctx)) return fail(ctx, RBL_ERR_STATE, "rbl_lock: needs an HBM-resident basis");
  if (nvec == 0) return RBL_OK;
  HIPC(hipSetDevice(ctx->device));
  const int64_t nl = std::max<int64_t>(ctx->nloc, 1);
  if (ctx->nlock + nvec > ctx->lock_cap) {
    const int cap = std::max(2 * ctx->lock_cap, ctx->nlock + nvec);
    double* d = nullptr;
    HIPC(hipMalloc(&d, (size_t)cap * nl * sizeof(double)));
    if (ctx->nlock)
      HIPC(hipMemcpyAsync(d, ctx->d_lock, (size_t)ctx->nlock * nl * sizeof(double),
                          hipMemcpyDeviceToDevice, ctx->stream));
    HIPC(hipStreamSynchronize(ctx->stream));
    hipFree(ctx->d_lock);
    ctx->d_lock = d;
    ctx->lock_cap = cap;
  }
  const int64_t rows = (int64_t)nblocks * ctx->b;
  for (int v = 0; v < nvec; ++v)
    CHK(basis_combine(ctx, nblocks, 1, S + v * rows, ctx->d_lock + (int64_t)(ctx->nlock + v) * nl));
  ctx->nlock += nvec;
  return RBL_OK;
}

int rbl_num_locked(rbl_ctx* ctx) { return ctx ? ctx->nlock : 0; }

int rbl_get_locked(rbl_ctx* ctx, double* V_out) {
  if (!ctx || !V_out) return fail(ctx, RBL_ERR_INVALID, "rbl_get_locked: bad arguments");
  if (ctx->nlock == 0) return RBL_OK;
  HIPC(hipSetDevice(ctx->device));
  const int64_t nl = std::max<int64_t>(ctx->nloc, 1);
  for (int j = 0; j < ctx->nlock; ++j)
    HIPC(hipMemcpy(V_out + (int64_t)j * ctx->nloc, ctx->d_lock + (int64_t)j * nl,
                   ctx->nloc * sizeof(double), hipMemcpyDeviceToHost));
  return RBL_OK;
}

int rbl_reorth_last(rbl_ctx* ctx, int nblocks, int flags) {
  if (ctx) ctx->cloc_step = 0;
  if (!ctx || nblocks < 1 || nblocks > ctx->nblocks)
    return fail(ctx, RBL_ERR_INVALID, "rbl_reorth_last: bad arguments");
  if (!ctx->d_basis) return fail(ctx, RBL_ERR_STATE, "rbl_reorth_last: needs an fp64 run");
  if (spilled(ctx)) return fail(ctx, RBL_ERR_STATE, "rbl_reorth_last: needs an HBM-resident basis");
  HIPC(hipSetDevice(ctx->device));
  CHK(reorth_pair(ctx, nblocks, flags));
  HIPC(hipStreamSynchronize(ctx->stream));
  harvest_timers(ctx);
  return RBL_OK;
}

int rbl_num_stages(void) { return RBL_NUM_STAGES; }
const char* rbl_stage_name(int stage) {
  return (stage >= 0 && stage < RBL_NUM_STAGES) ? kStageNames[stage] : "";
}
int rbl_timers(rbl_ctx* ctx, double* ms, int nstages) {
  if (!ctx || !ms) return RBL_ERR_INVALID;
  for (int s = 0; s < nstages && s < RBL_NUM_STAGES; ++s) ms[s] = ctx->stage_ms[s];
  return RBL_OK;
}
int rbl_allgather_host(rbl_ctx* ctx, const int64_t* mine, int64_t* all, int n) {
  if (!ctx || n < 0 || (n > 0 && (!mine || !all))) return fail(ctx, RBL_ERR_INVALID, "rbl_allgather_host: bad arguments");
  if (n == 0) return RBL_OK;
  HIPC(hipSetDevice(ctx->device));
  if (ctx->nranks == 1) {
    memcpy(all, mine, (size_t)n * sizeof(int64_t));
    return RBL_OK;
  }
  COMMC(ctx->comm->allgather_host(mine, all, (size_t)n, ctx->stream, &ctx->err));
  return RBL_OK;
}

int rbl_comm_stats(rbl_ctx* ctx, int64_t* out, int nstats, int reset) {
  if (!ctx || nstats < 0 || (nstats > 0 && !out)) return RBL_ERR_INVALID;
  for (int i = 0; i < nstats && i < RBL_COMM_NSTATS; ++i) out[i] = ctx->comm_stats[i];
  if (nstats > RBL_COMM_HALO_PUSH) out[RBL_COMM_HALO_PUSH] = ctx->push ? 1 : 0;
  if (nstats > RBL_COMM_PUSH_ROWS) out[RBL_COMM_PUSH_ROWS] = ctx->push_pred_rows;
  if (nstats > RBL_COMM_PULL_ROWS) out[RBL_COMM_PULL_ROWS] = ctx->pull_pred_rows;
  const int64_t tm[4] = {ctx->comm_host_ns[0], ctx->comm_host_ns[1],
                         (int64_t)(ctx->comm_dev_ms[0] * 1e6), (int64_t)(ctx->comm_dev_ms[1] * 1e6)};
  for (int i = RBL_COMM_PULL_ROWS + 1; i < nstats; ++i)
    out[i] = i <= RBL_COMM_EXCHANGE_DEV_NS ? tm[i - RBL_COMM_ALLREDUCE_HOST_NS] : 0;
  if (reset) {
    for (int64_t& v : ctx->comm_stats) v = 0;
    ctx->comm_host_ns[0] = ctx->comm_host_ns[1] = 0;
    ctx->comm_dev_ms[0] = ctx->comm_dev_ms[1] = 0.0;
  }
  return RBL_OK;
}

int rbl_path_stats(rbl_ctx* ctx, int64_t* out, int nstats, int reset) {
  if (!ctx || nstats < 0 || (nstats > 0 && !out)) return RBL_ERR_INVALID;
  for (int i = 0; i < nstats; ++i) out[i] = i < RBL_PATH_NSTATS ? ctx->path_stats[i] : 0;
  if (reset)
    for (int64_t& v : ctx->path_stats) v = 0;
  return RBL_OK;
}

// ... 15 lines not shown
```

gpu-randomized-block-lanczos_amd/csrc/rowop.hip:

```cpp
#include <atomic>

#include "kernels.hpp"

namespace rbl {

namespace {

constexpr int kRowThreads = 256;
#ifndef RBL_RG_WPE_G
#define RBL_RG_WPE_G 2
#endif
#ifndef RBL_RG_WPE
#define RBL_RG_WPE 3
#endif
#ifndef RBL_RG_WPE_M1
#define RBL_RG_WPE_M1 RBL_RG_WPE_G
#endif
constexpr int kBlockRows = 16;

typedef double d4v __attribute__((ext_vector_type(4)));
__device__ __forceinline__ double mfma4r(double a, double b, double c) {
  return __builtin_amdgcn_mfma_f64_4x4x4f64(a, b, c, 0, 0, 0);
}
#ifndef RBL_ROWOP_NT
#define RBL_ROWOP_NT 1
#endif
__device__ __forceinline__ d2v ldnt(const d2v* p) {
  if constexpr (RBL_ROWOP_NT) return __builtin_nontemporal_load(p);
  return *p;
}
__device__ __forceinline__ void stnt(d2v v, d2v* p) {
  if constexpr (RBL_ROWOP_NT) __builtin_nontemporal_store(v, p);
  else *p = v;
}

template <bool TRI, int CG>
__device__ __forceinline__ void mfma_row(const int k0, double a, const double* cb, double (&acc)[CG]) {
#pragma unroll
  for (int cp = 0; cp < CG / 2; ++cp) {
    const bool z0 = TRI && k0 > 8 * cp + 3, z1 = TRI && k0 > 8 * cp + 7;
    if (z0 && z1) continue;
    const d2v bf = *reinterpret_cast<const d2v*>(cb + 8 * cp);
    if (!z0) acc[2 * cp] = mfma4r(a, bf.x, acc[2 * cp]);
    if (!z1) acc[2 * cp + 1] = mfma4r(a, bf.y, acc[2 * cp + 1]);
  }
  if constexpr (CG % 2) {
    if (!(TRI && k0 > 4 * (CG - 1) + 3)) acc[CG - 1] = mfma4r(a, cb[8 * (CG / 2)], acc[CG - 1]);
  }
}

template <int B, bool GRAM, bool XF = false, bool YF = false, int MODE = 0, bool XG = false,
          bool TRI = false>
__global__ __launch_bounds__(kRowThreads) __attribute__((amdgpu_waves_per_eu(MODE == 1 ? RBL_RG_WPE_M1 : GRAM || XG ? RBL_RG_WPE_G : RBL_RG_WPE))) void k_rowgram(int64_t nrows, const double* X,
                                                         const double* __restrict__ C, int ldc,
                                                         double* Y, double alpha, double beta,
                                                         double* __restrict__ slab, const int* skip,
                                                         const float* X32, float* Y32,
                                                         const int* f64flag, const double* __restrict__ C2,
                                                         const double* __restrict__ Z,
                                                         double* __restrict__ slab2) {
  if (skip && *skip) return;
  constexpr bool TWO = MODE == 2, STORE = MODE != 1;
  const bool w64 = !YF || (f64flag && *f64flag);
  constexpr int CG = B / 4;
  constexpr int NH = B / 8;
  constexpr int LDC = B + 8;
  constexpr int kYPer = 16 * B / 128;
  constexpr int NG = CG * (CG + 1) / 2;
  constexpr int NT = B / 16;
  constexpr int kMain = B * LDC + (TWO ? B * LDC : 0) + 4 * 16 * B;
  constexpr int kRed = GRAM || XG ? 4 * B * B : 0;
  __shared__ __attribute__((aligned(16))) double lds[kMain > kRed ? kMain : kRed];
  double* cs = lds;
  double* cs2 = lds + B * LDC;
  double* gs = lds;
  const int tid = threadIdx.x, lane = tid & 63, wave = tid >> 6;
  const int q = lane >> 4, g = (lane >> 2) & 3, j = lane & 3;

  for (int e = tid; e < B * B; e += kRowThreads) {
    const int k = e / B, c = e % B;
    cs[k * LDC + perm8(c)] = alpha * C[(int64_t)k * ldc + c];
    if constexpr (TWO) cs2[k * LDC + perm8(c)] = C2[(int64_t)k * ldc + c];
  }
  __syncthreads();

  double* ot = lds + B * LDC + (TWO ? B * LDC : 0) + wave * 16 * B;
  auto swz = [](int row, int c) { return row * B + (c ^ (4 * ((row >> 2) & 3))); };

  const int64_t nblk = (nrows + kBlockRows - 1) / kBlockRows;
  const int64_t stride = (int64_t)gridDim.x * 4;
  int64_t blk = (int64_t)blockIdx.x * 4 + wave;

  auto load_x = [&](int64_t b0, d2v (&xa)[1][NH]) {
#pragma unroll
    for (int rt = 0; rt < 1; ++rt) {
      int64_t r = b0 * kBlockRows + 16 * rt + (lane & 15);
      r = r < nrows ? r : nrows - 1;
#pragma unroll
      for (int h = 0; h < NH; ++h)
        if constexpr (XF) {
          const float2 f = *reinterpret_cast<const float2*>(X32 + r * B + 8 * h + 2 * q);
          xa[rt][h] = d2v{(double)f.x, (double)f.y};
        } else {
          xa[rt][h] = ldnt(reinterpret_cast<const d2v*>(X + r * B + 8 * h + 2 * q));
        }
    }
  };
  auto load_y = [&](int64_t b0, d2v (&yr)[1][kYPer]) {
#pragma unroll
    for (int rt = 0; rt < 1; ++rt)
#pragma unroll
      for (int m = 0; m < kYPer; ++m) {
        const int e = 2 * lane + 128 * m;
        int64_t r = b0 * kBlockRows + 16 * rt + e / B;
        r = r < nrows ? r : nrows - 1;
        yr[rt][m] = ldnt(reinterpret_cast<const d2v*>(Y + r * B + (e % B)));
      }
  };

  auto load_z = [&](int64_t b0, double (&za)[4][NT]) {
#pragma unroll
    for (int s4 = 0; s4 < 4; ++s4) {
      int64_t r = b0 * kBlockRows + 4 * s4 + q;
      r = r < nrows ? r : nrows - 1;
#pragma unroll
      for (int it = 0; it < NT; ++it) za[s4][it] = Z[r * B + 16 * it + (lane & 15)];
    }
  };

  double gacc[GRAM ? NG : 1];
#pragma unroll
  for (int p = 0; p < (GRAM ? NG : 1); ++p) gacc[p] = 0.0;
  d4v gx[XG ? NT : 1][XG ? NT : 1];
#pragma unroll
  for (int it = 0; it < (XG ? NT : 1); ++it)
#pragma unroll
    for (int jt = 0; jt < (XG ? NT : 1); ++jt) gx[it][jt] = d4v{0.0, 0.0, 0.0, 0.0};

  d2v xa[1][NH], ya[1][kYPer];
  double za[XG ? 4 : 1][XG ? NT : 1];
  const bool by = MODE == 0 && beta != 0.0;
  const int64_t blk_c = blk < nblk ? blk : nblk - 1;
  load_x(blk_c, xa);
  if (by) load_y(blk_c, ya);
  if constexpr (XG) load_z(blk_c, za);
  for (; blk < nblk; blk += stride) {
    asm volatile("" ::: "memory");
    d2v xn[1][NH], yn[1][kYPer];
    double zn[XG ? 4 : 1][XG ? NT : 1];
    {
      const int64_t bn = blk + stride < nblk ? blk + stride : nblk - 1;
      load_x(bn, xn);
      if (by) load_y(bn, yn);
      if constexpr (XG) load_z(bn, zn);
    }
    double acc[1][CG];
#pragma unroll
    for (int rt = 0; rt < 1; ++rt) {
      if (by) {
#pragma unroll
        for (int m = 0; m < kYPer; ++m) {
          const int e = 2 * lane + 128 * m;
          *reinterpret_cast<d2v*>(ot + swz(e / B, e % B)) = beta * ya[rt][m];
        }
#pragma unroll
        for (int cg = 0; cg < CG; ++cg) acc[rt][cg] = ot[swz(4 * g + q, 4 * cg + j)];
      } else {
#pragma unroll
        for (int cg = 0; cg < CG; ++cg) acc[rt][cg] = 0.0;
      }
#pragma unroll
      for (int h = 0; h < NH; ++h)
#pragma unroll
        for (int v = 0; v < 2; ++v) {
          const double a = v ? xa[rt][h].y : xa[rt][h].x;
          const double* cb = cs + (8 * h + 2 * q + v) * LDC + 2 * j;
          mfma_row<TRI>(8 * h + v, a, cb, acc[rt]);
        }
      if constexpr (TWO) {
#pragma unroll
        for (int cg = 0; cg < CG; ++cg) ot[swz(4 * g + q, 4 * cg + j)] = acc[rt][cg];
        d2v x2[NH];
#pragma unroll
        for (int h = 0; h < NH; ++h) x2[h] = *reinterpret_cast<const d2v*>(ot + swz(lane & 15, 8 * h + 2 * q));
#pragma unroll
        for (int cg = 0; cg < CG; ++cg) acc[rt][cg] = 0.0;
#pragma unroll
        for (int h = 0; h < NH; ++h)
#pragma unroll
          for (int v = 0; v < 2; ++v) {
            const double a = v ? x2[h].y : x2[h].x;
            const double* cb = cs2 + (8 * h + 2 * q + v) * LDC + 2 * j;
            mfma_row<TRI>(8 * h + v, a, cb, acc[rt]);
          }
      }
      const int64_t rbase = blk * kBlockRows + 16 * rt;
      if constexpr (GRAM) {
        const bool live = rbase + 4 * g + q < nrows;
        double am[CG];
#pragma unroll
        for (int cg = 0; cg < CG; ++cg) am[cg] = live ? acc[rt][cg] : 0.0;
        int p = 0;
#pragma unroll
        for (int ic = 0; ic < CG; ++ic)
#pragma unroll
          for (int jc = ic; jc < CG; ++jc, ++p) gacc[p] = mfma4r(am[ic], am[jc], gacc[p]);
      }
      if constexpr (STORE || XG) {
#pragma unroll
        for (int cg = 0; cg < CG; ++cg) ot[swz(4 * g + q, 4 * cg + j)] = acc[rt][cg];
      }
      if constexpr (XG) {
#pragma unroll
        for (int s4 = 0; s4 < 4; ++s4) {
          const bool lz = rbase + 4 * s4 + q < nrows;
#pragma unroll
          for (int jt = 0; jt < NT; ++jt) {
            const double yb = ot[swz(4 * s4 + q, 16 * jt + (lane & 15))];
#pragma unroll
            for (int it = 0; it < NT; ++it)
              gx[it][jt] = __builtin_amdgcn_mfma_f64_16x16x4f64(lz ? za[s4][it] : 0.0, yb, gx[it][jt], 0, 0, 0);
          }
        }
      }
#pragma unroll
      for (int m = 0; m < (STORE ? kYPer : 0); ++m) {
        const int e = 2 * lane + 128 * m;
        const int64_t r = rbase + e / B;
        const d2v v = *reinterpret_cast<const d2v*>(ot + swz(e / B, e % B));
        if (r < nrows) {
          if (w64) stnt(v, reinterpret_cast<d2v*>(Y + r * B + (e % B)));
          else *reinterpret_cast<float2*>(Y32 + r * B + (e % B)) = make_float2((float)v.x, (float)v.y);
        }
      }
    }
#pragma unroll
    for (int rt = 0; rt < 1; ++rt) {
#pragma unroll
      for (int h = 0; h < NH; ++h) xa[rt][h] = xn[rt][h];
#pragma unroll
      for (int m = 0; m < kYPer; ++m) ya[rt][m] = yn[rt][m];
    }
    if constexpr (XG) {
#pragma unroll
      for (int s4 = 0; s4 < 4; ++s4)
#pragma unroll
        for (int it = 0; it < NT; ++it) za[s4][it] = zn[s4][it];
// ... 45 lines not shown
  int v = per.load(std::memory_order_relaxed);
  if (v == 0) {
    int nb = 0;
    if (hipOccupancyMaxActiveBlocksPerMultiprocessor(&nb, k_rowgram<B, GRAM, XF, YF, MODE, XG, TRI>,
                                                     kRowThreads, 0) != hipSuccess || nb < 1)
      nb = 2;
    v = nb < kMaxPerCu ? nb : kMaxPerCu;
    per.store(v, std::memory_order_relaxed);
  }
  return v;
}

template <int B, bool GRAM, bool XF, bool YF, int MODE, bool XG, bool TRI>
void launch_rg_t(const RowOpArgs& a, int64_t nrows, int grid, hipStream_t s) {
  if (grid <= 0) grid = rowgram_grid(nrows, rg_per_cu<B, GRAM, XF, YF, MODE, XG, TRI>());
  if (a.grid_out) *a.grid_out = grid;
  hipLaunchKernelGGL((k_rowgram<B, GRAM, XF, YF, MODE, XG, TRI>), dim3(grid), dim3(kRowThreads), 0, s,
                     nrows, a.X, a.C, a.ldc, a.Y, a.alpha, a.beta, a.slab, a.skip, a.X32, a.Y32,
                     a.f64flag, a.C2, a.Z, a.slab2);
}
template <int B, bool GRAM, bool XF, bool YF, int MODE, bool XG>
void launch_rg(const RowOpArgs& a, int64_t nrows, int grid, hipStream_t s) {
  if constexpr (!XF) {
    if (a.tri) return launch_rg_t<B, GRAM, XF, YF, MODE, XG, true>(a, nrows, grid, s);
  }
  launch_rg_t<B, GRAM, XF, YF, MODE, XG, false>(a, nrows, grid, s);
}

template <int B>
bool launch_rowgram(const RowOpArgs& a, int64_t nrows, int grid, hipStream_t s) {
  const bool gram = a.slab != nullptr, xg = a.Z != nullptr;
  if (a.mode == 0 && !xg) {
    if (a.X32 && a.Y32) {
      if (gram) launch_rg<B, true, true, true, 0, false>(a, nrows, grid, s);
      else launch_rg<B, false, true, true, 0, false>(a, nrows, grid, s);
    } else if (a.X32) {
      if (gram) launch_rg<B, true, true, false, 0, false>(a, nrows, grid, s);
      else launch_rg<B, false, true, false, 0, false>(a, nrows, grid, s);
    } else if (a.Y32) {
      if (gram) launch_rg<B, true, false, true, 0, false>(a, nrows, grid, s);
      else launch_rg<B, false, false, true, 0, false>(a, nrows, grid, s);
    } else {
      if (gram) launch_rg<B, true, false, false, 0, false>(a, nrows, grid, s);
      else launch_rg<B, false, false, false, 0, false>(a, nrows, grid, s);
    }
    return true;
  }
  if (a.X32) return false;
  if (a.mode == 0 && xg && !gram) {
    if (a.Y32) launch_rg<B, false, false, true, 0, true>(a, nrows, grid, s);
    else launch_rg<B, false, false, false, 0, true>(a, nrows, grid, s);
    return true;
  }
  if (a.mode == 1 && gram && !xg && !a.Y32) {
    launch_rg<B, true, false, false, 1, false>(a, nrows, grid, s);
    return true;
  }
  if (a.mode == 2 && !gram) {
    if (xg) {
      if (a.Y32) launch_rg<B, false, false, true, 2, true>(a, nrows, grid, s);
      else launch_rg<B, false, false, false, 2, true>(a, nrows, grid, s);
    } else {
      if (a.Y32) launch_rg<B, false, false, true, 2, false>(a, nrows, grid, s);
      else launch_rg<B, false, false, false, 2, false>(a, nrows, grid, s);
    }
    return true;
  }
  return false;
}

}

bool rowgram_ok(int b) { return b == 16 || b == 32; }

int rowgram_grid(int64_t nrows, int per_cu) {
  int64_t g = (int64_t)per_cu * window_grid();
  const int64_t need = (nrows + 4 * kBlockRows - 1) / (4 * kBlockRows);
  if (g > need) g = need;
  return (int)(g < 1 ? 1 : g);
}

bool rowgram_ex(int64_t nrows, int b, const RowOpArgs& a, int grid, hipStream_t s) {
  if (b == 32) return launch_rowgram<32>(a, nrows, grid, s);
  if (b == 16) return launch_rowgram<16>(a, nrows, grid, s);
  return false;
}

void rowgram(int64_t nrows, int b, const double* X, const double* C, int ldc, double* Y,
             double alpha, double beta, double* slab, int grid, const int* skip, hipStream_t s,
             const float* X32, float* Y32, const int* f64flag, bool tri) {
  RowOpArgs a;
  a.tri = tri;
  a.X = X;
  a.C = C;
  a.ldc = ldc;
  a.Y = Y;
  a.alpha = alpha;
  a.beta = beta;
  a.slab = slab;
  a.skip = skip;
  a.X32 = X32;
  a.Y32 = Y32;
  a.f64flag = f64flag;
  rowgram_ex(nrows, b, a, grid, s);
}

}
```

gpu-randomized-block-lanczos_amd/csrc/smallmat.hip:

```cpp
#include <cstdlib>

#include "kernels.hpp"

namespace rbl {

constexpr int kMaxB = 64;

template <bool LDS>
struct SmallMat {
  double* p;
  int ld;
  __device__ double& operator()(int r, int c) const { return p[r * ld + c]; }
};

template <bool LDS>
__global__ __launch_bounds__(256) void k_chol(const double* __restrict__ G, int b, int64_t nglob,
                                              int mode, double* R, double* Rinv, double* Rtot,
                                              int* need3, int* status, const int* skip,
                                              double* scratch) {
  if (skip && *skip) return;
  __shared__ double Ml[LDS ? kMaxB * (kMaxB + 1) : 1];
  __shared__ double Xl[LDS ? kMaxB * (kMaxB + 1) : 1];
  __shared__ int fail;
  __shared__ double shift;
// ... 448 lines not shown
__global__ void k_copy(const double* __restrict__ src, double* __restrict__ dst, int64_t len,
                       const int* skip) {
  if (skip && *skip) return;
  for (int64_t e = (int64_t)blockIdx.x * blockDim.x + threadIdx.x; e < len;
       e += (int64_t)gridDim.x * blockDim.x)
    dst[e] = src[e];
}
void copy_small(const double* src, double* dst, int64_t len, hipStream_t s, const int* skip) {
  int64_t blocks = (len + 255) / 256;
  if (blocks > 8192) blocks = 8192;
  if (blocks < 1) blocks = 1;
  hipLaunchKernelGGL(k_copy, dim3((unsigned)blocks), dim3(256), 0, s, src, dst, len, skip);
}

__global__ void k_stash(const double* __restrict__ Ai, const double* __restrict__ Rtot,
                        double* __restrict__ Bprev, int* __restrict__ flags,
                        double* __restrict__ stash, int bb) {
  for (int e = threadIdx.x; e < bb; e += blockDim.x) {
    stash[e] = Ai[e];
    const double r = Rtot[e];
    stash[bb + e] = r;
    Bprev[e] = r;
  }
  if (threadIdx.x < 4) {
    reinterpret_cast<int*>(stash + 2 * bb)[threadIdx.x] = flags[threadIdx.x];
    flags[threadIdx.x] = 0;
  }
  __threadfence_system();
}
void stash_step(const double* Ai, const double* Rtot, double* Bprev, int* flags, double* stash,
                int b, hipStream_t s) {
  hipLaunchKernelGGL(k_stash, dim3(1), dim3(256), 0, s, Ai, Rtot, Bprev, flags, stash, b * b);
}

__global__ void k_cloc_rinv(double* __restrict__ C, const double* __restrict__ Rinv, int b,
                            const int* __restrict__ skip) {
  if (skip && *skip) return;
  __shared__ double c[kMaxB * kMaxB];
  const int bb = b * b;
  for (int e = threadIdx.x; e < bb; e += blockDim.x) c[e] = C[e];
  __syncthreads();
  for (int e = threadIdx.x; e < bb; e += blockDim.x) {
    const int r = e / b, col = e % b;
    double acc = 0.0;
    for (int k = 0; k <= col; ++k) acc += c[r * b + k] * Rinv[k * b + col];
    C[e] = acc;
  }
}
void cloc_rinv(double* C, const double* Rinv, int b, const int* skip, hipStream_t s) {
  if (getenv("RBL_DIAG_CLOC_NOFIX")) return;
  hipLaunchKernelGGL(k_cloc_rinv, dim3(1), dim3(256), 0, s, C, Rinv, b, skip);
}

__global__ void k_transpose_small(const double* __restrict__ src, double* __restrict__ dst, int b) {
  for (int e = threadIdx.x; e < b * b; e += blockDim.x) dst[(e % b) * b + e / b] = src[e];
}
void transpose_small(const double* src, double* dst, int b, hipStream_t s) {
  hipLaunchKernelGGL(k_transpose_small, dim3(1), dim3(256), 0, s, src, dst, b);
}

}
```

gpu-randomized-block-lanczos_amd/csrc/spmm_bt.hip:

```cpp
#include <cstdlib>
#include <type_traits>

#include <hipcub/hipcub.hpp>

#include "kernels.hpp"

namespace rbl {

namespace bt {
constexpr int kThreads = 256;
constexpr int kRing = 256;
template <int B>
struct Geo {
  static constexpr int kRowBytes = B == 32 ? 320 : 128;
  static constexpr int kRingBytes = kRing * kRowBytes;
  static constexpr int kBtOff = kRingBytes;
  static constexpr int kBtBytes = B * B * 8;
  static constexpr int kUStride = B == 32 ? 336 : 128;
  static constexpr int kUWave = 16 * kUStride;
  static constexpr int kUOff = kBtOff + kBtBytes;
  static constexpr int kLds = kUOff + 4 * kUWave;
  static constexpr int kCtOff = kLds;
  static constexpr int kTrOff = kLds + 9216;
  static_assert(kLds + 9216 + 4 * 4 * 2304 <= 160 * 1024, "LDS budget");
};
__device__ __forceinline__ int pi_slot(int i) {
  const int c = (i >> 2) == 0 ? 0 : (i >> 2) == 1 ? 2 : (i >> 2) == 2 ? 3 : 1;
  return 4 * (i & 3) + c;
}
}

__device__ __forceinline__ double mfma44(double a, double b, double c) {
  return __builtin_amdgcn_mfma_f64_4x4x4f64(a, b, c, 0, 0, 0);
}

struct BtArgs {
  int64_t nrows;
  int64_t ntiles;
  int64_t tiles_per_wg;
  const double* A;
  const double* Q;
  int64_t col_off;
  int64_t q_lo, q_hi;
  const double* zrow;
  const void* Qloc;
  int64_t loc_lo, loc_hi;
  int64_t row0;
  double* U;
  const double* Qprev;
  const float* Q32;
  const float* Qprev32;
  const double* Bi;
  double* ai_slab;
  const uint64_t* hdr;
  const double* pv;
  const double* Ah;
  const double* Ae;
  const double* Cl;
  double* Qw;
  int64_t lf_lo, lf_hi;
};

constexpr int kCtLd = 36;
constexpr int kCtBytes = 32 * kCtLd * 8;
constexpr int kTrLd = 18;
constexpr int kTrBytes = 16 * kTrLd * 8;
#ifndef RBL_BT_QNT
#define RBL_BT_QNT 0
#endif
__device__ __forceinline__ d2v qld(const d2v* p) {
  if constexpr (RBL_BT_QNT) return __builtin_nontemporal_load(p);
  return *p;
}
__device__ __forceinline__ void lf_loads(const double* rraw, const double* rprev, int lane,
                                         d2v (&raw)[4], d2v (&qa)[4]) {
  const int q = lane >> 4, j = lane & 3;
#pragma unroll
  for (int p = 0; p < 4; ++p) raw[p] = qld(reinterpret_cast<const d2v*>(rraw + 2 * j) + 4 * p);
#pragma unroll
  for (int m = 0; m < 4; ++m) qa[m] = qld(reinterpret_cast<const d2v*>(rprev + 2 * q) + 4 * m);
}
__device__ __forceinline__ void lf_table(const double* C, double* ct, int tid, int nthreads) {
  for (int idx = tid; idx < 32 * 32; idx += nthreads) ct[(idx >> 5) * kCtLd + (idx & 31)] = -C[idx];
}
__device__ __forceinline__ void lf_block(const d2v (&raw)[4], const d2v (&qa)[4], const double* ct,
                                         int lane, double (&acc)[4][2]) {
  const int q = lane >> 4, j = lane & 3;
#pragma unroll
  for (int p = 0; p < 4; ++p) {
    acc[p][0] = raw[p].x;
    acc[p][1] = raw[p].y;
  }
#pragma unroll
  for (int m = 0; m < 4; ++m)
#pragma unroll
    for (int s = 0; s < 2; ++s) {
      const double av = s ? qa[m].y : qa[m].x;
      const double* crow = ct + (8 * m + 2 * q + s) * kCtLd + 2 * j;
#pragma unroll
      for (int p = 0; p < 4; ++p) {
        const d2v bv = *reinterpret_cast<const d2v*>(crow + 8 * p);
        acc[p][0] = __builtin_amdgcn_mfma_f64_4x4x4f64(av, bv.x, acc[p][0], 0, 0, 0);
        acc[p][1] = __builtin_amdgcn_mfma_f64_4x4x4f64(av, bv.y, acc[p][1], 0, 0, 0);
      }
    }
}

template <int B, int NG, bool EPI, bool AIG, int VAR = 0>
__global__ __launch_bounds__(bt::kThreads) __attribute__((amdgpu_waves_per_eu(1, 1)))
void k_spmm_bt(BtArgs a) {
  using L = bt::Geo<B>;
  constexpr int NP = B / 8;
  constexpr int NS = B / 2;
  constexpr int NE = B / 4;
  constexpr int H = 8 * (NG - 1);
  constexpr int kRoundRows = 64;
  constexpr int kRingSpan = kRoundRows + 2 * H;
  static_assert(kRingSpan + kRoundRows <= bt::kRing, "ring holds a round and the next one's rows");
  extern __shared__ __attribute__((aligned(16))) unsigned char smem[];

  const int tid = threadIdx.x, lane = tid & 63;
  const int wave = __builtin_amdgcn_readfirstlane(tid >> 6);
  const int64_t T0 = (int64_t)blockIdx.x * a.tiles_per_wg;
  const int64_t T1 = T0 + a.tiles_per_wg < a.ntiles ? T0 + a.tiles_per_wg : a.ntiles;
  if (T0 >= T1) return;
  const int q = lane >> 4, j = lane & 3, G = (lane >> 2) & 3, i16 = lane & 15;
  const int64_t gq = a.row0 - H;

  auto qload = [&](int64_t rho, int s) -> d2v {
    const int64_t c = rho + gq;
    const bool in = c >= a.q_lo && c < a.q_hi;
    const bool own = c >= a.loc_lo && c < a.loc_hi;
    if constexpr (VAR & 64) {
      const float* p = own ? static_cast<const float*>(a.Qloc) + (c - a.loc_lo) * B
                           : in ? a.Q32 + (c - a.col_off) * B : reinterpret_cast<const float*>(a.zrow);
      const float2 f = reinterpret_cast<const float2*>(p)[s];
      return d2v{(double)f.x, (double)f.y};
    } else {
      const double* p = own ? static_cast<const double*>(a.Qloc) + (c - a.loc_lo) * B
                            : in ? a.Q + (c - a.col_off) * B : a.zrow;
      return qld(reinterpret_cast<const d2v*>(p) + s);
    }
  };
  auto ring_ptr = [&](int64_t rho, int s) -> d2v* {
    return reinterpret_cast<d2v*>(smem + (unsigned)(rho & (bt::kRing - 1)) * L::kRowBytes + 16u * s);
  };

  if constexpr (EPI) {
    double* btab = reinterpret_cast<double*>(smem + L::kBtOff);
    for (int idx = tid; idx < B * B; idx += bt::kThreads) {
      const int sp = idx & 1, jj = (idx >> 1) & 3, qq = (idx >> 3) & 3, p = (idx >> 5) % NP,
                e = (idx >> 5) / NP;
      const int x = 8 * (e >> 1) + 2 * qq + (e & 1), y = 8 * p + 2 * jj + sp;
      btab[idx] = -a.Bi[y * B + x];
    }
  }
  constexpr bool LF = (VAR & 1024) != 0;
  static_assert(!LF || (B == 32 && !(VAR & (64 | 128))), "fused local reorth: b = 32, fp64, dense tiles");
  double* const ct = reinterpret_cast<double*>(smem + L::kCtOff);
  const int64_t own_lo = 16 * T0 + H > a.lf_lo ? 16 * T0 + H : a.lf_lo;
  int64_t own_hi = 16 * T1 - H < a.nrows ? 16 * T1 - H : a.nrows;
  own_hi = own_hi < a.lf_hi ? own_hi : a.lf_hi;
  auto lf_issue = [&](int64_t rho0, d2v (&raw)[4], d2v (&qa)[4]) {
    const int64_t cr = rho0 + gq + 4 * G + q, ca = rho0 + gq + i16;
    const bool inr = cr >= a.q_lo && cr < a.q_hi;
    const bool ownr = cr >= a.loc_lo && cr < a.loc_hi;
    const int64_t la = ca - a.row0;
    const double* rp = ownr ? static_cast<const double*>(a.Qloc) + (cr - a.loc_lo) * B
                            : inr ? a.Q + (cr - a.col_off) * B : a.zrow;
    lf_loads(rp, la >= a.lf_lo && la < a.lf_hi ? a.Qprev + la * B : a.zrow, lane, raw, qa);
  };
  auto lf_finish = [&](int64_t rho0, const d2v (&raw)[4], const d2v (&qa)[4]) {
    double f[4][2];
    lf_block(raw, qa, ct, lane, f);
    const int64_t rr = rho0 + 4 * G + q;
    const int64_t lr = rr + gq - a.row0;
    const bool wb = lr >= own_lo && lr < own_hi;
#pragma unroll
    for (int p = 0; p < 4; ++p) {
      const d2v v = d2v{f[p][0], f[p][1]};
      *ring_ptr(rr, 4 * p + j) = v;
      if (wb) reinterpret_cast<d2v*>(a.Qw + lr * B + 2 * j)[4 * p] = v;
    }
  };
  if constexpr (LF) {
    lf_table(a.Cl, ct, tid, bt::kThreads);
    __syncthreads();
    for (int bb = wave; bb < kRingSpan / 16; bb += 4) {
      d2v raw[4], qa[4];
      lf_issue(16 * T0 + 16 * bb, raw, qa);
      lf_finish(16 * T0 + 16 * bb, raw, qa);
    }
  } else {
    for (int idx = tid; idx < kRingSpan * NS; idx += bt::kThreads) {
      const int64_t rho = 16 * T0 + idx / NS;
      *ring_ptr(rho, idx % NS) = qload(rho, idx % NS);
    }
  }

  const int64_t tslot0 = 4 * (int64_t)blockIdx.x;
  const int64_t tslot_r = 4 * (int64_t)gridDim.x;
  constexpr bool HALF = (VAR & 2048) != 0;
  constexpr int NGL = (NG - 1) / 2, NGH = NG - NGL;
  static_assert(!HALF || !(VAR & 128), "half tiles are dense");
  auto slot_of = [&](int64_t t) -> int64_t {
    const int64_t w = t / a.tiles_per_wg, lt = t - w * a.tiles_per_wg;
    return ((lt >> 2) * gridDim.x + w) * 4 + (lt & 3);
  };
  struct HalfPlan {
    int64_t own = 0;
    int64_t src[NG / 2 > 0 ? NG / 2 : 1] = {};
    bool edge = false;
  };
  auto half_plan = [&](int64_t t) -> HalfPlan {
    HalfPlan hp;
    if constexpr (HALF) {
      const int64_t lt = t - T0;
      hp.own = (lt >> 2) * tslot_r + tslot0 + (lt & 3);
      hp.edge = t < NGL;
      if (!hp.edge) {
#pragma unroll
        for (int g = 0; g < NGL; ++g) {
          const int64_t ls = lt - NGL + g;
          hp.src[g] = ls >= 0 ? (ls >> 2) * tslot_r + tslot0 + (ls & 3) : 0;
        }
        if (lt < NGL) {
#pragma unroll
          for (int g = 0; g < NGL; ++g)
            if (lt - NGL + g < 0) hp.src[g] = slot_of(t - NGL + g);
        }
      }
    }
    return hp;
  };
  auto tile_a = [&](int64_t t, int g, int h, const HalfPlan& hp) -> d2v {
    if constexpr (HALF) {
      const int64_t ts = g >= NGL ? hp.own : hp.src[g < NGL ? g : 0];
      const int gh = g >= NGL ? g - NGL : NGL - g;
      const double* ph = a.Ah + ((((ts * NGH + gh) * 2 + h) * 64) + lane) * 2;
// ... 579 lines not shown
        } else {
#pragma unroll
          for (int i = 0; i < 4; ++i) *ring_ptr(rn + 4 * i + q, i16) = st[i];
        }
      }
      __syncthreads();
    }
    double* red = reinterpret_cast<double*>(smem);
    if constexpr (AIG && !R1) {
      if (p4 > 0) {
#pragma unroll
        for (int x = 0; x < NXG; ++x)
#pragma unroll
          for (int y = 0; y < NYQ; ++y) red[((p4 - 1) * NA + x * NYQ + y) * 64 + lane] = ai[x][y];
      }
    }
    __syncthreads();
    if constexpr (AIG && !R1) {
      if (p4 == 0) {
        double* out = a.ai_slab + (int64_t)blockIdx.x * B * B;
        const int xb = 2 * bt::pi_slot(4 * G + q);
#pragma unroll
        for (int x = 0; x < NXG; ++x)
#pragma unroll
          for (int y = 0; y < NYQ; ++y) {
            double v = ai[x][y];
#pragma unroll
            for (int w = 0; w < 3; ++w) v += red[(w * NA + x * NYQ + y) * 64 + lane];
            out[(xb + x) * B + 8 * (y >> 1) + 2 * j + (y & 1)] = v;
          }
      }
    }
  };
  if (role) run(std::integral_constant<int, 1>());
  else run(std::integral_constant<int, 0>());
}

template <int NG, bool EPI, bool AIG, int VAR>
static void launch_bt2_v(const BtArgs& a, int grid, hipStream_t s) {
  constexpr int lds = bt::Geo<32>::kLds + ((VAR & 2048) ? 9216 + 4 * ((NG - 1) / 2) * kTrBytes
                                                       : (VAR & 1024) ? kCtBytes : 0);
  ensure_lds_attr(reinterpret_cast<const void*>(&k_spmm_bt2<NG, EPI, AIG, VAR>), lds);
  hipLaunchKernelGGL((k_spmm_bt2<NG, EPI, AIG, VAR>), dim3(grid), dim3(512), lds, s, a);
}
static bool bt2_on() {
  const char* e = getenv("RBL_BT2");
  return e ? atoi(e) != 0 : false;
}
#endif

template <int B, int NG, bool EPI, bool AIG, int VAR>
static void launch_bt_v(const BtArgs& a, int grid, hipStream_t s) {
  constexpr int lds = bt::Geo<B>::kLds + ((VAR & 2048) ? 9216 + 4 * ((NG - 1) / 2) * kTrBytes
                                                      : (VAR & 1024) ? kCtBytes : 0);
  ensure_lds_attr(reinterpret_cast<const void*>(&k_spmm_bt<B, NG, EPI, AIG, VAR>), lds);
  hipLaunchKernelGGL((k_spmm_bt<B, NG, EPI, AIG, VAR>), dim3(grid), dim3(bt::kThreads), lds, s, a);
}
template <int B, int NG, bool EPI, bool AIG>
static void launch_bt_t(const BtArgs& a, int grid, hipStream_t s, bool f32) {
#ifndef RBL_VARIANTS
  if (f32) return launch_bt_v<B, NG, EPI, AIG, 3 | 64>(a, grid, s);
  launch_bt_v<B, NG, EPI, AIG, 3>(a, grid, s);
#else
  static const int var = [] {
    const char* e = getenv("RBL_BT_VAR");
    return e ? atoi(e) : 3;
  }();
  if (a.hdr) {
    if (f32) return launch_bt_v<B, NG, EPI, AIG, 3 | 64 | 128>(a, grid, s);
    if constexpr (B == 32 && NG == 9 && EPI && AIG) {
      if (var == 35) return launch_bt_v<B, NG, EPI, AIG, 35 | 128>(a, grid, s);
    }
    return launch_bt_v<B, NG, EPI, AIG, 3 | 128>(a, grid, s);
  }
  if (a.Ah) {
    if (f32) return launch_bt_v<B, NG, EPI, AIG, 3 | 64 | 2048>(a, grid, s);
    if constexpr (B == 32 && NG == 9 && EPI && AIG) {
      if (var == 2) return launch_bt_v<B, NG, EPI, AIG, 2 | 2048>(a, grid, s);
      if (var == 4099) return launch_bt_v<B, NG, EPI, AIG, 3 | 2048 | 4096>(a, grid, s);
    }
    return launch_bt_v<B, NG, EPI, AIG, 3 | 2048>(a, grid, s);
  }
  if (f32) return launch_bt_v<B, NG, EPI, AIG, 3 | 64>(a, grid, s);
  if constexpr (B == 32 && NG == 9 && EPI && AIG) {
    if (var == 0) return launch_bt_v<B, NG, EPI, AIG, 0>(a, grid, s);
    if (var == 35) return launch_bt_v<B, NG, EPI, AIG, 35>(a, grid, s);
    if (var == 259) return launch_bt_v<B, NG, EPI, AIG, 259>(a, grid, s);
    if (var == 515) return launch_bt_v<B, NG, EPI, AIG, 515>(a, grid, s);
  }
  launch_bt_v<B, NG, EPI, AIG, 3>(a, grid, s);
#endif
}

bool spmm_bt(const CsrDev& A, const double* Qin, int64_t col_off, int b, double* U,
             const double* Qprev, const double* Bi, hipStream_t s, double* ai_slab, int* ai_parts,
             const float* Q32, const float* Qprev32) {
  if ((b != 32 && b != 16) || !(A.bt || A.bth || A.btp_hdr) || A.ntiles <= 0 || !(A.bt_ng == 5 || A.bt_ng == 9)) return false;
  BtArgs a;
  a.nrows = A.nrows;
  a.ntiles = A.ntiles;
  a.tiles_per_wg = A.bt_tiles_per_wg;
  a.A = A.bt;
  a.Ah = A.bth;
  a.Ae = A.bte;
  a.Q = Qin;
  a.col_off = col_off;
  a.q_lo = A.q_lo;
  a.q_hi = A.q_hi;
  a.zrow = A.zrow;
  a.Qloc = A.qloc;
  a.loc_lo = A.qloc ? A.loc_lo : 0;
  a.loc_hi = A.qloc ? A.loc_hi : 0;
  a.row0 = A.row0;
  a.U = U;
  a.Qprev = Qprev;
  a.Q32 = Q32;
  a.Qprev32 = Qprev32;
  a.Bi = Bi;
  a.hdr = A.btp_hdr;
  a.pv = A.btp_val;
  const int grid = (int)((A.ntiles + A.bt_tiles_per_wg - 1) / A.bt_tiles_per_wg);
  const bool f32 = Q32 != nullptr;
  const bool epi = Qprev != nullptr || Qprev32 != nullptr;
  const bool aig = ai_slab != nullptr;
  a.ai_slab = ai_slab;
  if (ai_parts) *ai_parts = aig ? grid : 0;
  a.Cl = A.lfix_c;
  a.Qw = A.lfix_q;
  if (A.lfix_c) {
    if (b != 32 || f32 || a.hdr || !epi || !aig) return false;
    a.lf_lo = A.lfix_lo;
    a.lf_hi = A.lfix_hi;
#ifdef RBL_VARIANTS
    if (bt2_on()) {
      if (A.two_wave) *A.two_wave = 1;
      if (a.Ah) {
        if (A.bt_ng == 9) launch_bt2_v<9, true, true, 1024 | 2048>(a, grid, s);
        else launch_bt2_v<5, true, true, 1024 | 2048>(a, grid, s);
      } else {
        if (A.bt_ng == 9) launch_bt2_v<9, true, true, 1024>(a, grid, s);
        else launch_bt2_v<5, true, true, 1024>(a, grid, s);
      }
      return true;
    }
    if (a.Ah) {
      if (A.bt_ng == 9) launch_bt_v<32, 9, true, true, 3 | 1024 | 2048>(a, grid, s);
      else launch_bt_v<32, 5, true, true, 3 | 1024 | 2048>(a, grid, s);
      return true;
    }
#endif
    {
      if (A.bt_ng == 9) launch_bt_v<32, 9, true, true, 3 | 1024>(a, grid, s);
      else launch_bt_v<32, 5, true, true, 3 | 1024>(a, grid, s);
    }
    return true;
  }
#ifdef RBL_VARIANTS
  if (bt2_on() && b == 32 && epi && aig && !f32 && !a.hdr) {
    if (A.two_wave) *A.two_wave = 1;
    a.lf_lo = 0;
    a.lf_hi = 0;
    if (a.Ah) {
      if (A.bt_ng == 9) launch_bt2_v<9, true, true, 2048>(a, grid, s);
      else launch_bt2_v<5, true, true, 2048>(a, grid, s);
    } else {
      if (A.bt_ng == 9) launch_bt2_v<9, true, true, 0>(a, grid, s);
      else launch_bt2_v<5, true, true, 0>(a, grid, s);
    }
    return true;
  }
#endif
  const int key = (b == 32 ? 8 : 0) | (A.bt_ng == 9 ? 4 : 0) | (epi ? 2 : 0) | (aig ? 1 : 0);
  switch (key) {
#define RBL_BT_CASE(K, BB, NG, E, G) \
    case K: launch_bt_t<BB, NG, E, G>(a, grid, s, f32); break;
    RBL_BT_CASE(0, 16, 5, false, false) RBL_BT_CASE(1, 16, 5, false, true)
    RBL_BT_CASE(2, 16, 5, true, false)  RBL_BT_CASE(3, 16, 5, true, true)
    RBL_BT_CASE(4, 16, 9, false, false) RBL_BT_CASE(5, 16, 9, false, true)
    RBL_BT_CASE(6, 16, 9, true, false)  RBL_BT_CASE(7, 16, 9, true, true)
    RBL_BT_CASE(8, 32, 5, false, false) RBL_BT_CASE(9, 32, 5, false, true)
    RBL_BT_CASE(10, 32, 5, true, false) RBL_BT_CASE(11, 32, 5, true, true)
    RBL_BT_CASE(12, 32, 9, false, false) RBL_BT_CASE(13, 32, 9, false, true)
    RBL_BT_CASE(14, 32, 9, true, false) RBL_BT_CASE(15, 32, 9, true, true)
#undef RBL_BT_CASE
  }
  return true;
}

template <int H>
__global__ __launch_bounds__(64) void k_locfix(double* Q, const double* __restrict__ Qprev,
                                               const double* __restrict__ C, int64_t nrows,
                                               int64_t ntiles, int64_t tpw, const double* zrow,
                                               int64_t wlo, int64_t whi) {
  __shared__ __attribute__((aligned(16))) double ct[32 * kCtLd];
  const int lane = threadIdx.x;
  lf_table(C, ct, lane, 64);
  __syncthreads();
  constexpr int per = H / 16;
  const int64_t wg = blockIdx.x / (2 * per);
  const int side = (blockIdx.x / per) & 1, kb = blockIdx.x % per;
  const int64_t T0 = wg * tpw, T1 = T0 + tpw < ntiles ? T0 + tpw : ntiles;
  const int64_t lo = side == 0 ? 16 * T0 : (16 * T0 + H > 16 * T1 - H ? 16 * T0 + H : 16 * T1 - H);
  int64_t hi = side == 0 ? (16 * T1 < 16 * T0 + H ? 16 * T1 : 16 * T0 + H) : 16 * T1;
  hi = hi < nrows ? hi : nrows;
  const int64_t r0 = lo + 16 * kb;
  if (r0 >= hi) return;
  const int q = lane >> 4, j = lane & 3, G = (lane >> 2) & 3, i16 = lane & 15;
  const int64_t rr = r0 + 4 * G + q, ra = r0 + i16;
  d2v raw[4], qa[4];
  lf_loads(rr < nrows ? Q + rr * 32 : zrow, ra < nrows ? Qprev + ra * 32 : zrow, lane, raw, qa);
  double f[4][2];
  lf_block(raw, qa, ct, lane, f);
  if (rr < hi && rr >= wlo && rr < whi) {
#pragma unroll
    for (int p = 0; p < 4; ++p) reinterpret_cast<d2v*>(Q + rr * 32 + 2 * j)[4 * p] = d2v{f[p][0], f[p][1]};
  }
}

__global__ __launch_bounds__(64) void k_locfix_ranges(double* Q, const double* __restrict__ Qprev,
                                                      const double* __restrict__ C, int64_t nrows,
                                                      const double* zrow, int64_t lo0, int64_t hi0,
                                                      int64_t lo1, int64_t hi1) {
  __shared__ __attribute__((aligned(16))) double ct[32 * kCtLd];
  const int lane = threadIdx.x;
  lf_table(C, ct, lane, 64);
  __syncthreads();
  const int64_t nb0 = (hi0 - lo0 + 15) / 16;
  const int64_t r0 = blockIdx.x < nb0 ? lo0 + 16 * (int64_t)blockIdx.x : lo1 + 16 * ((int64_t)blockIdx.x - nb0);
  const int64_t hi = blockIdx.x < nb0 ? hi0 : hi1;
  if (r0 >= hi) return;
  const int q = lane >> 4, j = lane & 3, G = (lane >> 2) & 3, i16 = lane & 15;
  const int64_t rr = r0 + 4 * G + q, ra = r0 + i16;
  d2v raw[4], qa[4];
  lf_loads(rr < nrows ? Q + rr * 32 : zrow, ra < nrows ? Qprev + ra * 32 : zrow, lane, raw, qa);
  double f[4][2];
  lf_block(raw, qa, ct, lane, f);
  if (rr < hi) {
#pragma unroll
    for (int p = 0; p < 4; ++p) reinterpret_cast<d2v*>(Q + rr * 32 + 2 * j)[4 * p] = d2v{f[p][0], f[p][1]};
  }
}

bool spmm_bt_locfix_ok(const CsrDev& A, int b) {
  return b == 32 && (A.bt || A.bth) && !A.btp_hdr && A.ntiles > 0 && (A.bt_ng == 5 || A.bt_ng == 9);
}

int spmm_bt_halfwidth(const CsrDev& A) { return 8 * (A.bt_ng - 1); }

void spmm_bt_locfix_edges(const CsrDev& A, double* Q, const double* Qprev, const double* C,
                          int64_t lo0, int64_t hi0, int64_t lo1, int64_t hi1, hipStream_t s) {
  const int64_t nb = (hi0 - lo0 + 15) / 16 + (hi1 - lo1 + 15) / 16;
  if (nb > 0)
    hipLaunchKernelGGL(k_locfix_ranges, dim3((unsigned)nb), dim3(64), 0, s, Q, Qprev, C, A.nrows, A.zrow,
                       lo0, hi0, lo1, hi1);
}

void spmm_bt_locfix_rest(const CsrDev& A, double* Q, const double* Qprev, const double* C,
                         hipStream_t s) {
  const int64_t grid = (A.ntiles + A.bt_tiles_per_wg - 1) / A.bt_tiles_per_wg;
  if (A.bt_ng == 9)
    hipLaunchKernelGGL(k_locfix<64>, dim3((unsigned)(grid * 8)), dim3(64), 0, s, Q, Qprev, C, A.nrows,
                       A.ntiles, A.bt_tiles_per_wg, A.zrow, A.lfix_lo, A.lfix_hi);
  else
    hipLaunchKernelGGL(k_locfix<32>, dim3((unsigned)(grid * 4)), dim3(64), 0, s, Q, Qprev, C, A.nrows,
                       A.ntiles, A.bt_tiles_per_wg, A.zrow, A.lfix_lo, A.lfix_hi);
}

__global__ void k_bt_fill(int64_t nrows, const int64_t* __restrict__ rowptr,
                          const int32_t* __restrict__ col, const double* __restrict__ val,
                          int64_t row0, int H, int NG, int64_t tpw, int64_t grid,
                          double* __restrict__ out) {
  const int64_t r = ((int64_t)blockIdx.x * blockDim.x + threadIdx.x) >> 6;
  const int lane = threadIdx.x & 63;
  if (r >= nrows) return;
  const int64_t t = r >> 4;
  const int64_t wg = t / tpw, lt = t % tpw;
  const int64_t ts = ((lt >> 2) * grid + wg) * 4 + (lt & 3);
  const int i = (int)(r & 15);
  for (int64_t e = rowptr[r] + lane; e < rowptr[r + 1]; e += 64) {
    const int rho = (int)((int64_t)col[e] - (row0 - H) - 16 * t);
    const int g = rho >> 4, u = (rho >> 2) & 3, qq = rho & 3;
    const int64_t idx = ((((ts * NG + g) * 2 + (u >> 1)) * 64) + 16 * qq + i) * 2 + (u & 1);
    atomicAdd(out + idx, val[e]);
  }
}

#ifdef RBL_VARIANTS
__global__ void k_bt_symcheck(const double* __restrict__ full, int64_t ntiles, int64_t tpw,
                              int64_t grid, int NG, int* bad) {
  const int NGL = (NG - 1) / 2;
  const int64_t per = (int64_t)NGL * 256;
  const int64_t total = (ntiles - NGL) * per;
  auto slot = [&](int64_t t) {
    const int64_t w = t / tpw, lt = t - w * tpw;
    return ((lt >> 2) * grid + w) * 4 + (lt & 3);
  };
  auto at = [&](int64_t ts, int g, int r, int c) {
    const int u = c >> 2;
    return full[((((ts * NG + g) * 2 + (u >> 1)) * 64) + r + 16 * (c & 3)) * 2 + (u & 1)];
  };
  for (int64_t e = (int64_t)blockIdx.x * blockDim.x + threadIdx.x; e < total;
       e += (int64_t)gridDim.x * blockDim.x) {
    const int64_t t = NGL + e / per;
    const int g = (int)((e % per) >> 8), r = (int)(e & 15), c = (int)((e >> 4) & 15);
    const double x = at(slot(t), g, r, c), y = at(slot(t - NGL + g), NG - 1 - g, c, r);
    if (__double_as_longlong(x) != __double_as_longlong(y)) *bad = 1;
  }
}
__global__ void k_bt_half(const double* __restrict__ full, int64_t nslots, int NG,
                          double* __restrict__ half) {
  const int NGL = (NG - 1) / 2, NGH = NG - NGL;
  const int64_t total = nslots * NGH * 256;
  for (int64_t e = (int64_t)blockIdx.x * blockDim.x + threadIdx.x; e < total;
       e += (int64_t)gridDim.x * blockDim.x) {
    const int64_t ts = e / (NGH * 256);
    const int64_t rest = e - ts * NGH * 256;
    half[e] = full[(ts * NG + NGL) * 256 + rest];
  }
// ... 140 lines not shown
```

gpu-randomized-block-lanczos_amd/rbl/_lib.py:

```python
from __future__ import annotations

import ctypes as C
import os

import numpy as np

_HERE = os.path.dirname(os.path.abspath(__file__))
LIB_PATH = os.environ.get("RBL_LIB") or os.path.join(_HERE, "librbl_hip.so")

RBL_OK = 0
RBL_WARN_NOT_CONVERGED = 1
RBL_WARN_QR_SHIFTED = 2
RBL_ERR_INVALID = -1
RBL_ERR_HIP = -2
RBL_ERR_OOM = -3
RBL_ERR_RCCL = -4
RBL_ERR_STATE = -5
RBL_ERR_NUMERIC = -6

RBL_OPT_TIMERS = 0
RBL_OPT_REORTH_ORDER = 1
RBL_OPT_SPMM_KERNEL = 2
RBL_OPT_DEVICE_BLOCKS = 3
RBL_OPT_SPLIT_HALO = 4
RBL_OPT_KEEP_CSR = 5
RBL_OPT_FUSE = 6
RBL_OPT_HALO_OVERLAP = 7
RBL_OPT_RELABEL = 8
RBL_OPT_HALO_PUSH = 9
RBL_PATH_SPMM = 0
RBL_PATH_SPMM_LOC_FUSED = 1
RBL_PATH_LOC_SEPARATE = 2
RBL_PATH_LOC_GRAM = 3
RBL_PATH_LOCFIX_EDGES = 4
RBL_PATH_LOCFIX_REST = 5
RBL_PATH_SPMM_TWO_WAVE = 6
RBL_PATH_RITZ_PIECES = 7
RBL_PATH_NSTATS = 8
RBL_BUILD_VARIANTS = 1
RBL_SPMM_KERNEL_RECT = 8
RBL_MATRIX_FORMAT_RECT = 5

_p = C.c_void_p
_i64 = C.c_int64
_u64 = C.c_uint64
_pd = C.POINTER(C.c_double)
_pi64 = C.POINTER(C.c_int64)
_pi32 = C.POINTER(C.c_int32)
_pu8 = C.POINTER(C.c_uint8)

SIGNATURES = {
    "rbl_abi_version": (C.c_int, []),
    "rbl_build_flags": (C.c_int, []),
    "rbl_create": (C.c_int, [C.POINTER(_p), C.c_int]),
    "rbl_get_unique_id": (C.c_int, [_pu8]),
    "rbl_create_dist": (C.c_int, [C.POINTER(_p), C.c_int, C.c_int, C.c_int, _pu8]),
    "rbl_local_group_create": (C.c_int, [C.POINTER(_p), C.c_int]),
    "rbl_local_group_free": (C.c_int, [_p]),
    "rbl_create_local": (C.c_int, [C.POINTER(_p), C.c_int, _p, C.c_int]),
    "rbl_create_shm": (C.c_int, [C.POINTER(_p), C.c_int, C.c_int, C.c_int, C.c_char_p]),
    "rbl_free": (C.c_int, [_p]),
    "rbl_last_error": (C.c_char_p, [_p]),
    "rbl_comm_info": (C.c_int, [_p, C.POINTER(C.c_int), C.POINTER(C.c_int), C.c_char_p, C.c_int]),
    "rbl_rccl_version": (C.c_int, [C.POINTER(C.c_int), C.c_char_p, C.c_int]),
    "rbl_set_option": (C.c_int, [_p, C.c_int, _i64]),
    "rbl_device_memory": (C.c_int, [_p, _pi64, _pi64]),
    "rbl_set_matrix_csc": (C.c_int, [_p, _i64, _i64, _pi64, _pi64, _pd, C.c_int]),
    "rbl_set_matrix_csr_rows": (C.c_int, [_p, _i64, _i64, _i64, _pi64, _pi64, _pd, C.c_int]),
    "rbl_set_matrix_dense": (C.c_int, [_p, _i64, _i64, _i64, _pd, _i64]),
    "rbl_set_matrix_normal": (C.c_int, [_p, _i64, _i64, _i64, _pi64, _pi64, _pd, C.c_int, C.c_int]),
    "rbl_rect_info": (C.c_int, [_p, _pi64, _pi64, _pi64]),
    "rbl_get_matrix_rect": (C.c_int, [_p, C.c_int, _pi64, _pi32, _pd]),
    "rbl_apply_rect": (C.c_int, [_p, C.c_int, C.c_int, _pd, _pd]),
    "rbl_left_vectors": (C.c_int, [_p, C.c_int, _pd, _pd, _pd]),
    "rbl_set_rect_shift": (C.c_int, [_p, _pd, _pd]),
    "rbl_get_rect_shift": (C.c_int, [_p, _pd, _pd]),
    "rbl_apply_rect_shifted": (C.c_int, [_p, C.c_int, C.c_int, _pd, _pd]),
    "rbl_gen_matrix_hashwindow": (C.c_int, [_p, _i64, _i64, C.c_double, _u64, C.c_int, _pd]),
    "rbl_gen_matrix_circuit": (C.c_int, [_p, _i64, _i64, C.c_double, _u64, C.c_int, _pd]),
    "rbl_gen_matrix_rmat": (C.c_int, [_p, _i64, C.c_int, _i64, C.c_double, C.c_double, C.c_double,
                                      _u64, C.c_int, _pd]),
    "rbl_matrix_info": (C.c_int, [_p, _pi64, _pi64, _pi64, _pi64]),
    "rbl_get_matrix_csr": (C.c_int, [_p, _pi64, _pi32, _pd]),
    "rbl_row_ids": (C.c_int, [_p, _pi64]),
    "rbl_apply": (C.c_int, [_p, C.c_int, _pd, _pd]),
    "rbl_spmm_kernel_for": (C.c_int, [_p, C.c_int]),
    "rbl_matrix_format": (C.c_int, [_p]),
    "rbl_start": (C.c_int, [_p, C.c_int, C.c_int, C.c_int, _pd, _u64]),
    "rbl_step": (C.c_int, [_p, C.c_int, C.c_int, _pd, _pd]),
    "rbl_step_async": (C.c_int, [_p, C.c_int, C.c_int]),
    "rbl_comm_selftest": (C.c_int, [C.c_int, C.c_char_p, C.c_int]),
# ... 129 lines not shown
```

gpu-randomized-block-lanczos_amd/rbl/rbl_gpu.py:

```python
from __future__ import annotations

import math
import time
from dataclasses import dataclass, field

import numpy as np
import scipy.sparse as sp

from . import _lib
from ._lib import RBLError, dptr, i32ptr, i64ptr, lib, u8ptr
from .host import (TBand, dsbev, eig_topk, fix_signs,
                   residual_norms, sort_eig_abs, speculation_depth)

KRYL_SZ_GPU = 1200
RESIDUAL_TOL = 1e-7


class LocalGroup:

    def __init__(self, nranks: int):
        import ctypes as C
        self._h = C.c_void_p()
        st = lib.rbl_local_group_create(C.byref(self._h), nranks)
        if st < 0:
# ... 371 lines not shown
        theta = np.ascontiguousarray(theta, dtype=np.float64)
        k = theta.size
        if Y.ndim != 2 or Y.shape[1] != k or Y.shape[0] < k:
            raise ValueError("ritz_finish: Y must be kk x k (kk >= k) and theta of length k")
        V = np.zeros((r1 - r0, k), order="F")
        res = np.zeros(k)
        if Y.shape[0] == k:
            self._check(lib.rbl_ritz_finish(self._h, k, dptr(Y), dptr(theta), dptr(V), dptr(res)),
                        "rbl_ritz_finish")
        else:
            self._check(lib.rbl_ritz_finish_cols(self._h, Y.shape[0], k, dptr(Y), dptr(theta), dptr(V),
                                                 dptr(res)), "rbl_ritz_finish_cols")
        return V, res

    def timers(self) -> dict:
        names = _lib.stage_names()
        ms = np.zeros(len(names))
        self._check(lib.rbl_timers(self._h, dptr(ms), len(names)), "rbl_timers")
        return dict(zip(names, ms.tolist()))

    def reset_timers(self) -> None:
        self._check(lib.rbl_reset_timers(self._h), "rbl_reset_timers")

    def device_memory(self) -> tuple:
        f, t = np.zeros(1, np.int64), np.zeros(1, np.int64)
        self._check(lib.rbl_device_memory(self._h, i64ptr(f), i64ptr(t)), "rbl_device_memory")
        return int(f[0]), int(t[0])

    def comm_info(self) -> dict:
        import ctypes as C
        n, r = C.c_int(0), C.c_int(0)
        buf = C.create_string_buffer(32)
        self._check(lib.rbl_comm_info(self._h, C.byref(n), C.byref(r), buf, 32), "rbl_comm_info")
        out = {"nranks": n.value, "rank": r.value, "transport": buf.value.decode()}
        if out["transport"] == "rccl":
            out.update(rccl_version())
        return out

    def comm_stats(self, reset: bool = False, times: bool = False) -> dict:
        out = np.zeros(12, np.int64)
        self._check(lib.rbl_comm_stats(self._h, i64ptr(out), 12, int(reset)), "rbl_comm_stats")
        keys = ("allreduce_calls", "allreduce_bytes", "exchange_calls", "send_bytes",
                "recv_bytes", "halo_push", "push_rows_pred", "pull_rows_pred")
        if times:
            keys += ("allreduce_host_ns", "exchange_host_ns", "allreduce_dev_ns", "exchange_dev_ns")
        return dict(zip(keys, (int(x) for x in out)))

    def path_stats(self, reset: bool = False) -> dict:
        from . import _lib as L
        out = np.zeros(L.RBL_PATH_NSTATS, np.int64)
        self._check(lib.rbl_path_stats(self._h, i64ptr(out), L.RBL_PATH_NSTATS, int(reset)),
                    "rbl_path_stats")
        return dict(zip(("spmm", "spmm_loc_fused", "loc_separate", "loc_gram", "locfix_edges",
                         "locfix_rest", "spmm_two_wave", "ritz_pieces"), (int(x) for x in out)))

    def allgather(self, values) -> np.ndarray:
        mine = np.ascontiguousarray(np.asarray(values, dtype=np.int64).ravel())
        out = np.zeros(self.nranks * mine.size, np.int64)
        self._check(lib.rbl_allgather_host(self._h, i64ptr(mine), i64ptr(out), mine.size),
                    "rbl_allgather_host")
        return out.reshape(self.nranks, mine.size)

    def synchronize(self) -> None:
        self._check(lib.rbl_synchronize(self._h), "rbl_synchronize")


@dataclass
class RBLInfo:
    iters: int = 0
    nblocks: int = 0
    converged: bool = False
    status: int = 0
    qr_shifted_steps: int = 0
    eig_ms: float = 0.0
    fetch_ms: float = 0.0
    ritz_ms: float = 0.0
    start_ms: float = 0.0
    enqueue_ms: float = 0.0
    spec_steps: int = 0
    spec_wasted: int = 0
    resid: list = field(default_factory=list)
    trace_A: list = field(default_factory=list)
    trace_B: list = field(default_factory=list)


def rccl_version() -> dict:
    import ctypes as C
    v = C.c_int(0)
    buf = C.create_string_buffer(512)
    st = lib.rbl_rccl_version(C.byref(v), buf, 512)
    if st != 0:
        raise RBLError(st, f"rbl_rccl_version: {buf.value.decode()}")
    code = v.value
    return {"rccl_version": f"{code // 10000}.{code // 100 % 100}.{code % 100}",
            "rccl_version_code": code, "rccl_path": buf.value.decode()}


def set_update(ctx: Context, update) -> None:
    if update is None:
        return
    try:
        P, S = update
    except (TypeError, ValueError):
        raise ValueError("update must be a pair (P, S)") from None
    ctx.set_lowrank(P, S)


# ... 121 lines not shown
```

include/rbl_hip.h:

```cpp
#ifndef RBL_HIP_H
#define RBL_HIP_H

#include <stdint.h>

#ifdef __cplusplus
extern "C" {
#endif

#define RBL_ABI_VERSION 2
#define RBL_MAX_BLOCK 512

#define RBL_OK                  0
#define RBL_WARN_NOT_CONVERGED  1
#define RBL_WARN_QR_SHIFTED     2
#define RBL_ERR_INVALID        -1
#define RBL_ERR_HIP            -2
#define RBL_ERR_OOM            -3
#define RBL_ERR_RCCL           -4
#define RBL_ERR_STATE          -5
#define RBL_ERR_NUMERIC        -6

#define RBL_STAGE_AQ          0
#define RBL_STAGE_3TERM       1
#define RBL_STAGE_QR          2
#define RBL_STAGE_PART_REORTH 3
#define RBL_STAGE_LOC_REORTH  4
#define RBL_STAGE_RITZ        5
#define RBL_STAGE_COMM        6
#define RBL_STAGE_SPILL_WAIT  7
#define RBL_NUM_STAGES        8

#define RBL_OPT_TIMERS        0
#define RBL_OPT_REORTH_ORDER  1
#define RBL_OPT_DEVICE_BLOCKS 3
#define RBL_OPT_SPMM_KERNEL   2
#define RBL_OPT_SPLIT_HALO    4
#define RBL_OPT_KEEP_CSR      5
#define RBL_OPT_FUSE          6

#define RBL_OPT_HALO_OVERLAP  7

#define RBL_OPT_RELABEL       8

#define RBL_OPT_HALO_PUSH     9

typedef struct rbl_ctx rbl_ctx;

int rbl_abi_version(void);
#define RBL_BUILD_VARIANTS 1
int rbl_build_flags(void);

int rbl_create(rbl_ctx** ctx, int device);
int rbl_get_unique_id(uint8_t unique_id[128]);
int rbl_comm_selftest(int device, char* msg, int msg_len);
int rbl_create_dist(rbl_ctx** ctx, int device, int nranks, int rank, const uint8_t unique_id[128]);
typedef struct rbl_group rbl_group;
int rbl_local_group_create(rbl_group** group, int nranks);
int rbl_local_group_free(rbl_group* group);
int rbl_create_local(rbl_ctx** ctx, int device, rbl_group* group, int rank);
int rbl_create_shm(rbl_ctx** ctx, int device, int nranks, int rank, const char* path);
int rbl_free(rbl_ctx* ctx);
const char* rbl_last_error(const rbl_ctx* ctx);
int rbl_comm_info(rbl_ctx* ctx, int* nranks, int* rank, char* transport, int transport_len);
int rbl_rccl_version(int* version, char* path, int path_len);
int rbl_set_option(rbl_ctx* ctx, int option, int64_t value);
int rbl_device_memory(rbl_ctx* ctx, int64_t* free_bytes, int64_t* total_bytes);

int rbl_set_matrix_csc(rbl_ctx* ctx, int64_t n, int64_t nnz, const int64_t* colptr,
                       const int64_t* rowval, const double* nzval, int index_base);
int rbl_set_matrix_csr_rows(rbl_ctx* ctx, int64_t n, int64_t row_begin, int64_t row_end,
                            const int64_t* rowptr, const int64_t* colind, const double* val,
                            int index_base);
int rbl_set_matrix_dense(rbl_ctx* ctx, int64_t n, int64_t row_begin, int64_t row_end,
                         const double* A, int64_t lda);
#define RBL_SPMM_KERNEL_RECT   8
#define RBL_MATRIX_FORMAT_RECT 5
int rbl_set_matrix_normal(rbl_ctx* ctx, int64_t nrows, int64_t ncols, int64_t nnz,
                          const int64_t* ptr, const int64_t* ind, const double* val,
                          int index_base, int layout);
int rbl_rect_info(rbl_ctx* ctx, int64_t* nrows, int64_t* ncols, int64_t* nnz);
int rbl_get_matrix_rect(rbl_ctx* ctx, int trans, int64_t* rowptr, int32_t* colind, double* val);
int rbl_apply_rect(rbl_ctx* ctx, int trans, int b, const double* X, double* Y);
int rbl_left_vectors(rbl_ctx* ctx, int k, const double* V, const double* sigma, double* U_out);
int rbl_set_rect_shift(rbl_ctx* ctx, const double* u, const double* v);
int rbl_get_rect_shift(rbl_ctx* ctx, double* u_out, double* v_out);
int rbl_apply_rect_shifted(rbl_ctx* ctx, int trans, int b, const double* X, double* Y);
int rbl_gen_matrix_hashwindow(rbl_ctx* ctx, int64_t n, int64_t halfwidth, double density,
                              uint64_t seed, int nplant, const double* plant);
int rbl_gen_matrix_rmat(rbl_ctx* ctx, int64_t n, int scale, int64_t edges, double a, double b,
                        double c, uint64_t seed, int nplant, const double* plant);
int rbl_gen_matrix_circuit(rbl_ctx* ctx, int64_t n, int64_t width, double p_edge, uint64_t seed,
                           int nplant, const double* plant);
int rbl_matrix_info(rbl_ctx* ctx, int64_t* n, int64_t* row_begin, int64_t* row_end,
                    int64_t* nnz_local);
int rbl_row_ids(rbl_ctx* ctx, int64_t* ids);
int rbl_get_matrix_csr(rbl_ctx* ctx, int64_t* rowptr, int32_t* colind, double* val);
int rbl_apply(rbl_ctx* ctx, int b, const double* X, double* Y);
// ... 15 lines not shown
int rbl_bench_series_pass(rbl_ctx* ctx, int64_t len, int reps, double* fused_ms, double* pair_ms);
int rbl_cheb_moments(rbl_ctx* ctx, int b, int degree, double lo, double hi, const double* X,
                     uint64_t seed, double* mom_out);
int rbl_bench_moment_pass(rbl_ctx* ctx, int64_t len_rows, int b, int reps, double* ms);

int rbl_set_lowrank(rbl_ctx* ctx, int r, const double* P, const double* S);
int rbl_get_lowrank(rbl_ctx* ctx, int* r_out, double* P_out, double* S_out);
int rbl_bench_lowrank_pass(rbl_ctx* ctx, int64_t rows, int b, int r, int reps, double* project_ms,
                           double* update_ms);

int rbl_ritz_project(rbl_ctx* ctx, int nblocks, int k, const double* S, double* H_out);
int rbl_ritz_finish(rbl_ctx* ctx, int k, const double* Y, const double* theta, double* V_out,
                    double* resid_out);
int rbl_ritz_finish_cols(rbl_ctx* ctx, int kproj, int k, const double* Y, const double* theta,
                         double* V_out, double* resid_out);

int rbl_restart(rbl_ctx* ctx, int nblocks, const double* S);
int rbl_lock(rbl_ctx* ctx, int nblocks, int nvec, const double* S);
int rbl_num_locked(rbl_ctx* ctx);
int rbl_get_locked(rbl_ctx* ctx, double* V_out);
int rbl_reorth_last(rbl_ctx* ctx, int nblocks, int flags);

int rbl_num_stages(void);
const char* rbl_stage_name(int stage);
int rbl_timers(rbl_ctx* ctx, double* ms, int nstages);
int rbl_reset_timers(rbl_ctx* ctx);
int rbl_synchronize(rbl_ctx* ctx);

#define RBL_COMM_ALLREDUCE_CALLS 0
#define RBL_COMM_ALLREDUCE_BYTES 1
#define RBL_COMM_EXCHANGE_CALLS  2
#define RBL_COMM_SEND_BYTES      3
#define RBL_COMM_RECV_BYTES      4
#define RBL_COMM_NSTATS          5
#define RBL_COMM_HALO_PUSH       5
#define RBL_COMM_PUSH_ROWS       6
#define RBL_COMM_PULL_ROWS       7
#define RBL_COMM_ALLREDUCE_HOST_NS 8
#define RBL_COMM_EXCHANGE_HOST_NS  9
#define RBL_COMM_ALLREDUCE_DEV_NS  10
#define RBL_COMM_EXCHANGE_DEV_NS   11
int rbl_comm_stats(rbl_ctx* ctx, int64_t* out, int nstats, int reset);

int rbl_allgather_host(rbl_ctx* ctx, const int64_t* mine, int64_t* all, int n);

#define RBL_PATH_SPMM            0
#define RBL_PATH_SPMM_LOC_FUSED  1
#define RBL_PATH_LOC_SEPARATE    2
#define RBL_PATH_LOC_GRAM        3
#define RBL_PATH_LOCFIX_EDGES    4
#define RBL_PATH_LOCFIX_REST     5
#define RBL_PATH_SPMM_TWO_WAVE   6
#define RBL_PATH_RITZ_PIECES     7
#define RBL_PATH_NSTATS          8
int rbl_path_stats(rbl_ctx* ctx, int64_t* out, int nstats, int reset);

int rbl_plan_row_partition(int64_t n, const int64_t* rowptr, int nranks, int64_t* bounds_out);
int rbl_plan_halo(int64_t nrows_local, const int64_t* rowptr, const int64_t* colind,
                  int index_base, int nranks, const int64_t* bounds, int64_t* lo, int64_t* hi);
int rbl_hashwindow_rows_host(int64_t n, int64_t halfwidth, double density, uint64_t seed,
                             int nplant, const double* plant, int64_t row_begin,
                             int64_t row_end, int64_t* rowptr_out, int64_t* colind_out,
                             double* val_out);

#ifdef __cplusplus
}
#endif
#endif
```

Baseline: 45.02.

## Defer CholQR second-pass apply and fuse it into the next band-tile SpMM

Adds a deferred CholQR mode for single-rank fp64 b=32 runs. The final triangular apply that writes Q_i is postponed and folded into the next step's band-tile SpMM kernel, which reads U and the two R-inverse tables from LDS. A materialise path writes the pending block back whenever any other API needs the basis. The aim is to drop one full pass that writes and re-reads the basis block each iteration. In exchange it adds extra LDS and MFMA work to the SpMM kernel, skip-flag plumbing, and more state management that carries correctness risk.

```diff
diff --git a/gpu-randomized-block-lanczos_amd/csrc/kernels.hpp b/gpu-randomized-block-lanczos_amd/csrc/kernels.hpp
--- a/gpu-randomized-block-lanczos_amd/csrc/kernels.hpp
+++ b/gpu-randomized-block-lanczos_amd/csrc/kernels.hpp
@@ -60,6 +60,10 @@
   double* lfix_q = nullptr;
   int* two_wave = nullptr;
   int64_t lfix_lo = 0, lfix_hi = 0;
+  const double* defer_u = nullptr;
+  const double* defer_r1 = nullptr;
+  const double* defer_r2 = nullptr;
+  const int* bt_skip = nullptr;
   const uint64_t* btp_hdr = nullptr;
   const double* btp_val = nullptr;
   const double* bth = nullptr;
@@ -169,7 +173,7 @@
 void spmm_bt_locfix_edges(const CsrDev& A, double* Q, const double* Qprev, const double* C,
                           int64_t lo0, int64_t hi0, int64_t lo1, int64_t hi1, hipStream_t s);
 void spmm_bt_locfix_rest(const CsrDev& A, double* Q, const double* Qprev, const double* C,
-                         hipStream_t s);
+                         hipStream_t s, const int* skip = nullptr);
 bool spmm_bt(const CsrDev& A, const double* Qin, int64_t col_off, int b, double* U,
              const double* Qprev, const double* Bi, hipStream_t s, double* ai_slab = nullptr,
              int* ai_parts = nullptr, const float* Q32 = nullptr, const float* Qprev32 = nullptr);
@@ -245,6 +249,7 @@
                double* scratch);
 void copy_small(const double* src, double* dst, int64_t len, hipStream_t s, const int* skip = nullptr);
 void cloc_rinv(double* C, const double* Rinv, int b, const int* skip, hipStream_t s);
+void copy_flags(const int* src, int* dst, int n, hipStream_t s);
 void transpose_small(const double* src, double* dst, int b, hipStream_t s);
 void stash_step(const double* Ai, const double* Rtot, double* Bprev, int* flags, double* stash,
                 int b, hipStream_t s);
diff --git a/gpu-randomized-block-lanczos_amd/csrc/rbl_api.cpp b/gpu-randomized-block-lanczos_amd/csrc/rbl_api.cpp
--- a/gpu-randomized-block-lanczos_amd/csrc/rbl_api.cpp
+++ b/gpu-randomized-block-lanczos_amd/csrc/rbl_api.cpp
@@ -192,6 +192,10 @@
   int cloc_step = 0;
   bool cloc_final = false;
   std::vector<int> step_flags;
+  bool qr_defer = true;
+  int pend_block = -1;
+  const double* pend_u = nullptr;
+  bool pend_consume = false;
   double stage_ms[RBL_NUM_STAGES] = {0};
   int64_t comm_stats[RBL_COMM_NSTATS] = {0};
   int64_t comm_host_ns[2] = {0, 0};
@@ -1408,6 +1412,23 @@
       A.lfix_lo = lf_lo;
       A.lfix_hi = lf_hi;
     }
+    if (ctx->pend_consume) {
+      if (!lfix_c || !ctx->pend_u || U == ctx->pend_u)
+        return fail(ctx, RBL_ERR_INVALID, "internal: deferred CholQR apply without the fused local reorth");
+      CsrDev D = A;
+      D.defer_u = ctx->pend_u;
+      D.defer_r1 = smallp(ctx, S_RINV1);
+      D.defer_r2 = smallp(ctx, S_RINV);
+      D.bt_skip = ctx->d_flags + 4;
+      int dparts = 0;
+      if (!spmm_bt(D, Qin, off, b, U, Qprev, Bi, ctx->stream, slab, &dparts))
+        return fail(ctx, RBL_ERR_INVALID, "internal: deferred CholQR apply not applicable to this SpMM");
+      A.bt_skip = ctx->d_flags + 5;
+      ctx->path_stats[RBL_PATH_SPMM_QR_DEFERRED] += 1;
+      ctx->pend_block = -1;
+      ctx->pend_u = nullptr;
+      ctx->pend_consume = false;
+    }
     const int parts = spmm(A, Qin, off, b, U, Qprev, Bi, ctx->spmm_variant, ctx->stream, slab);
     if (parts < 0) return fail(ctx, RBL_ERR_INVALID, "internal: split-source SpMM needs the band-tile kernel");
     ctx->path_stats[RBL_PATH_SPMM] += 1;
@@ -1416,7 +1437,7 @@
       ctx->path_stats[RBL_PATH_SPMM_LOC_FUSED] += 1;
       ctx->path_stats[RBL_PATH_LOCFIX_REST] += 1;
       StageScope t(ctx, RBL_STAGE_LOC_REORTH);
-      spmm_bt_locfix_rest(A, lfix_q, Qprev, lfix_c, ctx->stream);
+      spmm_bt_locfix_rest(A, lfix_q, Qprev, lfix_c, ctx->stream, A.bt_skip);
     }
     return parts;
   }
@@ -1735,7 +1756,7 @@
   if (G) a.slab = ctx->d_slab;
   if (a.Z) a.slab2 = ctx->d_slab + (size_t)gmax * b * b;
   const int xgrid = rowgram_grid(ctx->nloc, 2);
-  int grid = a.Z ? xgrid : 0;
+  int grid = a.Z && a.mode != 1 ? xgrid : 0;
   a.grid_out = &grid;
   if (ctx->nloc > 0) {
     if (!rowgram_ex(ctx->nloc, b, a, grid, ctx->stream))
@@ -1752,14 +1773,15 @@
     CHK(allreduce(ctx, G, (size_t)b * b));
   }
   if (Gx && reduce_x) {
-    reduce_slab(ctx->d_slab + (size_t)gmax * b * b, xgrid, (int64_t)b * b, Gx, nullptr, ctx->stream);
+    reduce_slab(ctx->d_slab + (size_t)gmax * b * b, a.mode == 1 ? grid : xgrid, (int64_t)b * b, Gx,
+                a.skip, ctx->stream);
     if (comm_x) CHK(allreduce(ctx, Gx, (size_t)b * b));
   }
   return RBL_OK;
 }
 
 int tsqr(rbl_ctx* ctx, const double* U, double* Qout, bool g1_ready = false, float* Qout32 = nullptr,
-         const double* Zloc = nullptr) {
+         const double* Zloc = nullptr, bool defer = false) {
   StageScope t(ctx, RBL_STAGE_QR);
   ctx->flags_clean = false;
   const int b = ctx->b;
@@ -1779,16 +1801,21 @@
   if (!g1_ready) CHK(gram(ctx, run1(U, b), pan1(U, b), G, nullptr));
   chol_step(G, b, ctx->n, 0, smallp(ctx, S_R), smallp(ctx, three ? S_RINV1 : S_RINV), smallp(ctx, S_RTOT),
             need3, status, nullptr, ctx->stream, smallp(ctx, S_CHS0));
+  if (defer && !(three && Zloc && !Qout32 && ctx->nranks == 1))
+    return fail(ctx, RBL_ERR_INVALID, "internal: the deferred CholQR apply needs the 3-pass QR with Zloc");
   if (three) {
+    if (defer) copy_flags(need3, ctx->d_flags + 4, 2, ctx->stream);
     RowOpArgs a1;
     a1.X = U;
     a1.C = smallp(ctx, S_RINV1);
     a1.ldc = b;
     a1.mode = 1;
     a1.tri = true;
-    CHK(rowop_ex(ctx, a1, G, nullptr, false));
+    if (defer) a1.Z = Zloc;
+    CHK(rowop_ex(ctx, a1, G, defer ? smallp(ctx, S_CLOC) : nullptr, defer, false));
     chol_step(G, b, ctx->n, 1, smallp(ctx, S_R), smallp(ctx, S_RINV), smallp(ctx, S_RTOT), need3,
               status, nullptr, ctx->stream, smallp(ctx, S_CHS0));
+    if (defer) cloc_rinv(smallp(ctx, S_CLOC), smallp(ctx, S_RINV), b, need3, ctx->stream);
     RowOpArgs a2;
     a2.X = U;
     a2.C = smallp(ctx, S_RINV1);
@@ -1800,6 +1827,7 @@
     a2.f64flag = Qout32 ? need3 : nullptr;
     a2.Z = Zloc;
     a2.mode = 2;
+    a2.skip = defer ? skip3 : nullptr;
     CHK(rowop_ex(ctx, a2, nullptr, Zloc ? smallp(ctx, S_CLOC) : nullptr, Zloc != nullptr, false));
     CHK(gram(ctx, run1(Qout, b), pan1(Qout, b), G, skip3, Zloc == nullptr));
     if (Zloc) CHK(allreduce(ctx, G, (size_t)2 * b * b));
@@ -1848,6 +1876,41 @@
   return RBL_OK;
 }
 
+bool defer_on(const rbl_ctx* ctx) {
+  const char* e = std::getenv("RBL_QR_DEFER");
+  return e && *e ? std::atoi(e) != 0 : ctx->qr_defer;
+}
+bool defer_ok(rbl_ctx* ctx, int b) {
+  if (!defer_on(ctx) || (ctx->fuse & 7) != 7 || ctx->basis_bits != 64 || b != 32) return false;
+  if (ctx->nranks != 1 || ctx->nloc <= 0 || ctx->dense || ctx->rect || ctx->lr_r != 0) return false;
+  if (has_filter(ctx) || spilled(ctx) || ctx->spmm_variant != 0) return false;
+  if (rbl_spmm_kernel_for(ctx, b) != 5) return false;
+  const CsrDev A = csr(ctx);
+  return A.bt != nullptr && !A.bth && !A.btp_hdr && spmm_bt_locfix_ok(A, b);
+}
+int materialise_pending(rbl_ctx* ctx) {
+  if (!ctx || ctx->pend_block < 0) return RBL_OK;
+  const int j = ctx->pend_block;
+  ctx->pend_block = -1;
+  ctx->pend_consume = false;
+  if (!ctx->d_basis || !ctx->pend_u) return RBL_OK;
+  HIPC(hipSetDevice(ctx->device));
+  RowOpArgs a2;
+  a2.X = ctx->pend_u;
+  a2.C = smallp(ctx, S_RINV1);
+  a2.C2 = smallp(ctx, S_RINV);
+  a2.ldc = ctx->b;
+  a2.tri = true;
+  a2.Y = slotp(ctx, j);
+  a2.mode = 2;
+  a2.skip = ctx->d_flags + 4;
+  ctx->pend_u = nullptr;
+  CHK(rowop_ex(ctx, a2, nullptr, nullptr, false, false));
+  HIPC(hipGetLastError());
+  ctx->path_stats[RBL_PATH_QR_MATERIALISE] += 1;
+  return RBL_OK;
+}
+
 int halo_exchange(rbl_ctx* ctx, const double* Q, const double** Qin, int64_t* off,
                   bool copy_local = true, hipStream_t st = nullptr) {
   if (ctx->nranks == 1) {
@@ -2030,6 +2093,7 @@
 }
 
 void free_run(rbl_ctx* ctx) {
+  (void)materialise_pending(ctx);
   if (ctx->cstream) hipStreamSynchronize(ctx->cstream);
   hipFree(ctx->d_basis); ctx->d_basis = nullptr;
   for (void* h : ctx->h_spill)
@@ -2467,6 +2531,7 @@
       if (value < 0 || value > 1) return fail(ctx, RBL_ERR_INVALID, "RBL_OPT_RELABEL must be 0|1");
       ctx->relabel_opt = (int)value;
       return RBL_OK;
+    case RBL_OPT_QR_DEFER: ctx->qr_defer = value != 0; return RBL_OK;
     case RBL_OPT_FUSE:
       if (value < 0 || value > 7) return fail(ctx, RBL_ERR_INVALID, "RBL_OPT_FUSE is a 3-bit mask");
       ctx->fuse = (int)value;
@@ -3074,6 +3139,7 @@
     return fail(ctx, RBL_ERR_INVALID, "rbl_start: a Chebyshev series (rbl_set_filter_series) runs on "
                                       "one rank and a square A only");
   HIPC(hipSetDevice(ctx->device));
+  CHK(materialise_pending(ctx));
   HIPC(hipStreamSynchronize(ctx->stream));
   int dev_slots = max_blocks + 1;
   const bool same_shape = (ctx->d_basis || ctx->d_basis32) && ctx->b == b &&
@@ -3151,7 +3217,7 @@
   }
   HIPC(hipMalloc(&ctx->d_U, (nl + kRowPad) * b * sizeof(double)));
   ctx->T_cols = b;
-  HIPC(hipMalloc(&ctx->d_T, nl * b * sizeof(double)));
+  HIPC(hipMalloc(&ctx->d_T, (nl + kRowPad) * b * sizeof(double)));
   if (ctx->nranks > 1) {
     CHK(ensure_qext(ctx, b, ctx->stream));
     if (ctx->ghost)
@@ -3163,8 +3229,8 @@
   ctx->C_elems = (size_t)std::max(1, max_blocks) * b * 2 * b;
   HIPC(hipMalloc(&ctx->d_C, ctx->C_elems * sizeof(double)));
   HIPC(hipMalloc(&ctx->d_small, (size_t)S_NSMALL * b * b * sizeof(double)));
-  HIPC(hipMalloc(&ctx->d_flags, 4 * sizeof(int)));
-  HIPC(hipMemset(ctx->d_flags, 0, 4 * sizeof(int)));
+  HIPC(hipMalloc(&ctx->d_flags, 6 * sizeof(int)));
+  HIPC(hipMemset(ctx->d_flags, 0, 6 * sizeof(int)));
   {
 #ifdef RBL_VARIANTS
     const char* e = std::getenv("RBL_STASH_COPY");
@@ -3310,6 +3376,14 @@
     return fail(ctx, RBL_ERR_INVALID, "rbl_step: locked-vector reorth needs the fp64 basis");
   const bool direct32 = f32 && i >= 2 && direct32_ok(ctx, b);
   if (f32 && !direct32) CHK(ensure_qm64(ctx));
+  if (ctx->pend_block >= 0) {
+    const bool reorths = ((part_reorth & 1) && i >= 3) || ((part_reorth & 2) && ctx->nlock > 0);
+    ctx->pend_consume = ctx->pend_block == i - 1 && i >= 2 && !reorths && ctx->cloc_step == i &&
+                        defer_ok(ctx, b);
+    if (!ctx->pend_consume) CHK(materialise_pending(ctx));
+  }
+  const bool consume = ctx->pend_consume;
+  double* const Uout = consume ? ctx->d_T : ctx->d_U;
   double* Qi = f32 ? ctx->d_Qi64 : slotp(ctx, i - 1);
   double* Qm = i >= 2 ? (f32 ? ctx->d_Qm64 : slotp(ctx, i - 2)) : nullptr;
   float* Qi32 = f32 ? slotp32(ctx, i - 1) : nullptr;
@@ -3470,8 +3544,11 @@
                    ctx->d_slab, &ai_parts, Qin32, Qm32))
         return fail(ctx, RBL_ERR_INVALID, "internal: fp32 band-tile SpMM not applicable");
     } else {
-      ai_parts = apply_A(ctx, Qin, off, b, ctx->d_U, Qm, i >= 2 ? smallp(ctx, S_BPREV) : nullptr,
+      if (consume && !(lfuse && Cloc == smallp(ctx, S_CLOC)))
+        return fail(ctx, RBL_ERR_INVALID, "internal: deferred CholQR apply without the fused local reorth");
+      ai_parts = apply_A(ctx, Qin, off, b, Uout, Qm, i >= 2 ? smallp(ctx, S_BPREV) : nullptr,
                          ctx->d_slab, split ? Qi : nullptr, Cloc, Qi, lf_lo, lf_hi, halo_ev);
+      if (consume && ai_parts >= 0) std::swap(ctx->d_U, ctx->d_T);
     }
     if (ai_parts < 0) return ai_parts;
     HIPC(hipGetLastError());
@@ -3506,10 +3583,15 @@
   if (!f32) {
     const int guess = i >= 2 ? ctx->step_flags[i - 1] : 0;
     const bool zfuse = fused && (ctx->fuse & 3) == 3 && !modifies(i + 1, guess) && i + 1 <= ctx->max_blocks;
-    CHK(tsqr(ctx, ctx->d_U, slotp(ctx, i), fused, nullptr, zfuse ? Qi : nullptr));
+    const bool defer = zfuse && i >= 2 && defer_ok(ctx, b);
+    CHK(tsqr(ctx, ctx->d_U, slotp(ctx, i), fused, nullptr, zfuse ? Qi : nullptr, defer));
     if (zfuse) {
       ctx->cloc_step = i + 1;
       ctx->cloc_final = false;
+    }
+    if (defer) {
+      ctx->pend_block = i;
+      ctx->pend_u = ctx->d_U;
     }
   } else {
     CHK(tsqr(ctx, ctx->d_U, ctx->d_Qi64, fused, slotp32(ctx, i)));
@@ -3677,6 +3759,7 @@
   if (nblocks > ctx->nblocks) return fail(ctx, RBL_ERR_INVALID, "rbl_ritz: more blocks than computed");
   if (k > nblocks * ctx->b) return fail(ctx, RBL_ERR_INVALID, "rbl_ritz: k > nblocks*b");
   HIPC(hipSetDevice(ctx->device));
+  CHK(materialise_pending(ctx));
   const int b = ctx->b;
   const int64_t rows = (int64_t)nblocks * b;
   const int64_t nl = std::max<int64_t>(ctx->nloc, 1);
@@ -4111,6 +4194,7 @@
   if (ctx->nranks > 1) return fail(ctx, RBL_ERR_INVALID, "rbl_ritz_project: one rank only");
   if (!ctx->d_basis && !ctx->d_basis32) return fail(ctx, RBL_ERR_STATE, "rbl_ritz_project before rbl_start");
   if (nblocks > ctx->nblocks) return fail(ctx, RBL_ERR_INVALID, "rbl_ritz_project: more blocks than computed");
+  CHK(materialise_pending(ctx));
   if (k > nblocks * ctx->b) return fail(ctx, RBL_ERR_INVALID, "rbl_ritz_project: k > nblocks*b");
   HIPC(hipSetDevice(ctx->device));
   HIPC(hipStreamSynchronize(ctx->stream));
@@ -4200,6 +4284,7 @@
   if (!ctx->d_rv || !ctx->d_rw || ctx->ritz_k != kproj)
     return fail(ctx, RBL_ERR_STATE, "rbl_ritz_finish_cols: no rbl_ritz_project of this kproj precedes it");
   HIPC(hipSetDevice(ctx->device));
+  CHK(materialise_pending(ctx));
   const int kpr = (kproj + 1) & ~1;
   const int kp = (k + 1) & ~1;
   const int64_t nl = std::max<int64_t>(ctx->nloc, 1);
@@ -4245,6 +4330,7 @@
 int rbl_get_block(rbl_ctx* ctx, int j, double* Q_out) {
   if (!ctx || j < 1 || j > ctx->nblocks || !Q_out) return fail(ctx, RBL_ERR_INVALID, "rbl_get_block: bad block");
   HIPC(hipSetDevice(ctx->device));
+  CHK(materialise_pending(ctx));
   const int b = ctx->b;
   int st = 0;
   const double* src = ctx->basis_bits == 64 ? block_dev(ctx, j - 1, ctx->nblocks, &st) : nullptr;
@@ -4272,6 +4358,7 @@
   if (!ctx->d_basis) return fail(ctx, RBL_ERR_STATE, "rbl_restart: needs an fp64 run (rbl_start)");
   if (spilled(ctx)) return fail(ctx, RBL_ERR_STATE, "rbl_restart: needs an HBM-resident basis");
   HIPC(hipSetDevice(ctx->device));
+  CHK(materialise_pending(ctx));
   const int b = ctx->b;
   CHK(basis_combine(ctx, nblocks, b, S, ctx->d_T));
   HIPC(hipMemcpyAsync(slotp(ctx, 0), ctx->d_T, ctx->nloc * b * sizeof(double),
@@ -4291,6 +4378,7 @@
   if (spilled(ctx)) return fail(ctx, RBL_ERR_STATE, "rbl_lock: needs an HBM-resident basis");
   if (nvec == 0) return RBL_OK;
   HIPC(hipSetDevice(ctx->device));
+  CHK(materialise_pending(ctx));
   const int64_t nl = std::max<int64_t>(ctx->nloc, 1);
   if (ctx->nlock + nvec > ctx->lock_cap) {
     const int cap = std::max(2 * ctx->lock_cap, ctx->nlock + nvec);
@@ -4331,6 +4419,7 @@
   if (!ctx->d_basis) return fail(ctx, RBL_ERR_STATE, "rbl_reorth_last: needs an fp64 run");
   if (spilled(ctx)) return fail(ctx, RBL_ERR_STATE, "rbl_reorth_last: needs an HBM-resident basis");
   HIPC(hipSetDevice(ctx->device));
+  CHK(materialise_pending(ctx));
   CHK(reorth_pair(ctx, nblocks, flags));
   HIPC(hipStreamSynchronize(ctx->stream));
   harvest_timers(ctx);
diff --git a/gpu-randomized-block-lanczos_amd/csrc/rowop.hip b/gpu-randomized-block-lanczos_amd/csrc/rowop.hip
--- a/gpu-randomized-block-lanczos_amd/csrc/rowop.hip
+++ b/gpu-randomized-block-lanczos_amd/csrc/rowop.hip
@@ -1,6 +1,7 @@
 #include <atomic>
 
 #include "kernels.hpp"
+#include "tri_apply.hpp"
 
 namespace rbl {
 
@@ -19,9 +20,7 @@
 constexpr int kBlockRows = 16;
 
 typedef double d4v __attribute__((ext_vector_type(4)));
-__device__ __forceinline__ double mfma4r(double a, double b, double c) {
-  return __builtin_amdgcn_mfma_f64_4x4x4f64(a, b, c, 0, 0, 0);
-}
+using tri::mfma4r;
 #ifndef RBL_ROWOP_NT
 #define RBL_ROWOP_NT 1
 #endif
@@ -32,21 +31,6 @@
 __device__ __forceinline__ void stnt(d2v v, d2v* p) {
   if constexpr (RBL_ROWOP_NT) __builtin_nontemporal_store(v, p);
   else *p = v;
-}
-
-template <bool TRI, int CG>
-__device__ __forceinline__ void mfma_row(const int k0, double a, const double* cb, double (&acc)[CG]) {
-#pragma unroll
-  for (int cp = 0; cp < CG / 2; ++cp) {
-    const bool z0 = TRI && k0 > 8 * cp + 3, z1 = TRI && k0 > 8 * cp + 7;
-    if (z0 && z1) continue;
-    const d2v bf = *reinterpret_cast<const d2v*>(cb + 8 * cp);
-    if (!z0) acc[2 * cp] = mfma4r(a, bf.x, acc[2 * cp]);
-    if (!z1) acc[2 * cp + 1] = mfma4r(a, bf.y, acc[2 * cp + 1]);
-  }
-  if constexpr (CG % 2) {
-    if (!(TRI && k0 > 4 * (CG - 1) + 3)) acc[CG - 1] = mfma4r(a, cb[8 * (CG / 2)], acc[CG - 1]);
-  }
 }
 
 template <int B, bool GRAM, bool XF = false, bool YF = false, int MODE = 0, bool XG = false,
@@ -77,15 +61,12 @@
   const int tid = threadIdx.x, lane = tid & 63, wave = tid >> 6;
   const int q = lane >> 4, g = (lane >> 2) & 3, j = lane & 3;
 
-  for (int e = tid; e < B * B; e += kRowThreads) {
-    const int k = e / B, c = e % B;
-    cs[k * LDC + perm8(c)] = alpha * C[(int64_t)k * ldc + c];
-    if constexpr (TWO) cs2[k * LDC + perm8(c)] = C2[(int64_t)k * ldc + c];
-  }
+  tri::table<B>(C, ldc, alpha, cs, tid, kRowThreads);
+  if constexpr (TWO) tri::table<B>(C2, ldc, 1.0, cs2, tid, kRowThreads);
   __syncthreads();
 
   double* ot = lds + B * LDC + (TWO ? B * LDC : 0) + wave * 16 * B;
-  auto swz = [](int row, int c) { return row * B + (c ^ (4 * ((row >> 2) & 3))); };
+  auto swz = [](int row, int c) { return tri::swz<B>(row, c); };
 
   const int64_t nblk = (nrows + kBlockRows - 1) / kBlockRows;
   const int64_t stride = (int64_t)gridDim.x * 4;
@@ -157,42 +138,22 @@
     double acc[1][CG];
 #pragma unroll
     for (int rt = 0; rt < 1; ++rt) {
-      if (by) {
-#pragma unroll
-        for (int m = 0; m < kYPer; ++m) {
-          const int e = 2 * lane + 128 * m;
-          *reinterpret_cast<d2v*>(ot + swz(e / B, e % B)) = beta * ya[rt][m];
-        }
-#pragma unroll
-        for (int cg = 0; cg < CG; ++cg) acc[rt][cg] = ot[swz(4 * g + q, 4 * cg + j)];
+      if constexpr (TWO) {
+        tri::apply2<TRI, B>(xa[rt], cs, cs2, ot, lane, acc[rt]);
       } else {
-#pragma unroll
-        for (int cg = 0; cg < CG; ++cg) acc[rt][cg] = 0.0;
-      }
-#pragma unroll
-      for (int h = 0; h < NH; ++h)
-#pragma unroll
-        for (int v = 0; v < 2; ++v) {
-          const double a = v ? xa[rt][h].y : xa[rt][h].x;
-          const double* cb = cs + (8 * h + 2 * q + v) * LDC + 2 * j;
-          mfma_row<TRI>(8 * h + v, a, cb, acc[rt]);
-        }
-      if constexpr (TWO) {
-#pragma unroll
-        for (int cg = 0; cg < CG; ++cg) ot[swz(4 * g + q, 4 * cg + j)] = acc[rt][cg];
-        d2v x2[NH];
-#pragma unroll
-        for (int h = 0; h < NH; ++h) x2[h] = *reinterpret_cast<const d2v*>(ot + swz(lane & 15, 8 * h + 2 * q));
-#pragma unroll
-        for (int cg = 0; cg < CG; ++cg) acc[rt][cg] = 0.0;
-#pragma unroll
-        for (int h = 0; h < NH; ++h)
-#pragma unroll
-          for (int v = 0; v < 2; ++v) {
-            const double a = v ? x2[h].y : x2[h].x;
-            const double* cb = cs2 + (8 * h + 2 * q + v) * LDC + 2 * j;
-            mfma_row<TRI>(8 * h + v, a, cb, acc[rt]);
+        if (by) {
+#pragma unroll
+          for (int m = 0; m < kYPer; ++m) {
+            const int e = 2 * lane + 128 * m;
+            *reinterpret_cast<d2v*>(ot + swz(e / B, e % B)) = beta * ya[rt][m];
           }
+#pragma unroll
+          for (int cg = 0; cg < CG; ++cg) acc[rt][cg] = ot[swz(4 * g + q, 4 * cg + j)];
+        } else {
+#pragma unroll
+          for (int cg = 0; cg < CG; ++cg) acc[rt][cg] = 0.0;
+        }
+        tri::apply_acc<TRI, B>(xa[rt], cs, lane, acc[rt]);
       }
       const int64_t rbase = blk * kBlockRows + 16 * rt;
       if constexpr (GRAM) {
@@ -344,8 +305,15 @@
     else launch_rg<B, false, false, false, 0, true>(a, nrows, grid, s);
     return true;
   }
-  if (a.mode == 1 && gram && !xg && !a.Y32) {
-    launch_rg<B, true, false, false, 1, false>(a, nrows, grid, s);
+  if (a.mode == 1 && gram && !a.Y32) {
+    if (xg) {
+      if (grid <= 0)
+        grid = rowgram_grid(nrows, a.tri ? rg_per_cu<B, true, false, false, 1, false, true>()
+                                         : rg_per_cu<B, true, false, false, 1, false, false>());
+      launch_rg<B, true, false, false, 1, true>(a, nrows, grid, s);
+    } else {
+      launch_rg<B, true, false, false, 1, false>(a, nrows, grid, s);
+    }
     return true;
   }
   if (a.mode == 2 && !gram) {
diff --git a/gpu-randomized-block-lanczos_amd/csrc/smallmat.hip b/gpu-randomized-block-lanczos_amd/csrc/smallmat.hip
--- a/gpu-randomized-block-lanczos_amd/csrc/smallmat.hip
+++ b/gpu-randomized-block-lanczos_amd/csrc/smallmat.hip
@@ -524,6 +524,13 @@
   hipLaunchKernelGGL(k_cloc_rinv, dim3(1), dim3(256), 0, s, C, Rinv, b, skip);
 }
 
+__global__ void k_copy_flags(const int* __restrict__ src, int* __restrict__ dst, int n) {
+  if ((int)threadIdx.x < n) dst[threadIdx.x] = src[threadIdx.x];
+}
+void copy_flags(const int* src, int* dst, int n, hipStream_t s) {
+  hipLaunchKernelGGL(k_copy_flags, dim3(1), dim3(64), 0, s, src, dst, n);
+}
+
 __global__ void k_transpose_small(const double* __restrict__ src, double* __restrict__ dst, int b) {
   for (int e = threadIdx.x; e < b * b; e += blockDim.x) dst[(e % b) * b + e / b] = src[e];
 }
diff --git a/gpu-randomized-block-lanczos_amd/csrc/spmm_bt.hip b/gpu-randomized-block-lanczos_amd/csrc/spmm_bt.hip
--- a/gpu-randomized-block-lanczos_amd/csrc/spmm_bt.hip
+++ b/gpu-randomized-block-lanczos_amd/csrc/spmm_bt.hip
@@ -4,6 +4,7 @@
 #include <hipcub/hipcub.hpp>
 
 #include "kernels.hpp"
+#include "tri_apply.hpp"
 
 namespace rbl {
 
@@ -59,12 +60,19 @@
   const double* Cl;
   double* Qw;
   int64_t lf_lo, lf_hi;
+  const double* Ud = nullptr;
+  const double* Rd1 = nullptr;
+  const double* Rd2 = nullptr;
+  const int* skip = nullptr;
 };
 
 constexpr int kCtLd = 36;
 constexpr int kCtBytes = 32 * kCtLd * 8;
 constexpr int kTrLd = 18;
 constexpr int kTrBytes = 16 * kTrLd * 8;
+constexpr int kTriTab = 32 * 40;
+constexpr int kDfBytes = (2 * kTriTab + 4 * 16 * 32) * 8;
+static_assert(kDfBytes <= 4 * 4 * kTrBytes, "the deferred apply's tables fit the LDS budget");
 #ifndef RBL_BT_QNT
 #define RBL_BT_QNT 0
 #endif
@@ -124,6 +132,7 @@
   const int64_t T0 = (int64_t)blockIdx.x * a.tiles_per_wg;
   const int64_t T1 = T0 + a.tiles_per_wg < a.ntiles ? T0 + a.tiles_per_wg : a.ntiles;
   if (T0 >= T1) return;
+  if (a.skip && *a.skip) return;
   const int q = lane >> 4, j = lane & 3, G = (lane >> 2) & 3, i16 = lane & 15;
   const int64_t gq = a.row0 - H;
 
@@ -158,21 +167,48 @@
   constexpr bool LF = (VAR & 1024) != 0;
   static_assert(!LF || (B == 32 && !(VAR & (64 | 128))), "fused local reorth: b = 32, fp64, dense tiles");
   double* const ct = reinterpret_cast<double*>(smem + L::kCtOff);
-  const int64_t own_lo = 16 * T0 + H > a.lf_lo ? 16 * T0 + H : a.lf_lo;
-  int64_t own_hi = 16 * T1 - H < a.nrows ? 16 * T1 - H : a.nrows;
+  constexpr bool DF = (VAR & 8192) != 0;
+  static_assert(!DF || (LF && !(VAR & 2048)), "deferred CholQR apply: with the fused local reorth, whole tiles");
+  double* const r1t = reinterpret_cast<double*>(smem + L::kTrOff);
+  double* const r2t = r1t + kTriTab;
+  double* const otw = r2t + kTriTab + wave * (16 * 32);
+  constexpr int kEdge = DF ? 0 : H;
+  const int64_t own_lo = 16 * T0 + kEdge > a.lf_lo ? 16 * T0 + kEdge : a.lf_lo;
+  int64_t own_hi = 16 * T1 - kEdge < a.nrows ? 16 * T1 - kEdge : a.nrows;
   own_hi = own_hi < a.lf_hi ? own_hi : a.lf_hi;
   auto lf_issue = [&](int64_t rho0, d2v (&raw)[4], d2v (&qa)[4]) {
     const int64_t cr = rho0 + gq + 4 * G + q, ca = rho0 + gq + i16;
     const bool inr = cr >= a.q_lo && cr < a.q_hi;
     const bool ownr = cr >= a.loc_lo && cr < a.loc_hi;
     const int64_t la = ca - a.row0;
+    if constexpr (DF) {
+      const bool in = la >= a.lf_lo && la < a.lf_hi;
+      const double* up = in ? a.Ud + la * B : a.zrow;
+#pragma unroll
+      for (int m = 0; m < 4; ++m) raw[m] = qld(reinterpret_cast<const d2v*>(up + 2 * q) + 4 * m);
+      const double* pp = in ? a.Qprev + la * B : a.zrow;
+#pragma unroll
+      for (int m = 0; m < 4; ++m) qa[m] = qld(reinterpret_cast<const d2v*>(pp + 2 * q) + 4 * m);
+      return;
+    }
     const double* rp = ownr ? static_cast<const double*>(a.Qloc) + (cr - a.loc_lo) * B
                             : inr ? a.Q + (cr - a.col_off) * B : a.zrow;
     lf_loads(rp, la >= a.lf_lo && la < a.lf_hi ? a.Qprev + la * B : a.zrow, lane, raw, qa);
   };
   auto lf_finish = [&](int64_t rho0, const d2v (&raw)[4], const d2v (&qa)[4]) {
     double f[4][2];
-    lf_block(raw, qa, ct, lane, f);
+    if constexpr (DF) {
+      double t8[8];
+      tri::apply2<true, 32>(raw, r1t, r2t, otw, lane, t8);
+#pragma unroll
+      for (int cg = 0; cg < 8; ++cg) otw[tri::swz<32>(4 * G + q, 4 * cg + j)] = t8[cg];
+      d2v rw[4];
+#pragma unroll
+      for (int p = 0; p < 4; ++p) rw[p] = *reinterpret_cast<const d2v*>(otw + tri::swz<32>(4 * G + q, 8 * p + 2 * j));
+      lf_block(rw, qa, ct, lane, f);
+    } else {
+      lf_block(raw, qa, ct, lane, f);
+    }
     const int64_t rr = rho0 + 4 * G + q;
     const int64_t lr = rr + gq - a.row0;
     const bool wb = lr >= own_lo && lr < own_hi;
@@ -185,6 +221,10 @@
   };
   if constexpr (LF) {
     lf_table(a.Cl, ct, tid, bt::kThreads);
+    if constexpr (DF) {
+      tri::table<32>(a.Rd1, 32, 1.0, r1t, tid, bt::kThreads);
+      tri::table<32>(a.Rd2, 32, 1.0, r2t, tid, bt::kThreads);
+    }
     __syncthreads();
     for (int bb = wave; bb < kRingSpan / 16; bb += 4) {
       d2v raw[4], qa[4];
@@ -870,6 +910,7 @@
 template <int B, int NG, bool EPI, bool AIG, int VAR>
 static void launch_bt_v(const BtArgs& a, int grid, hipStream_t s) {
   constexpr int lds = bt::Geo<B>::kLds + ((VAR & 2048) ? 9216 + 4 * ((NG - 1) / 2) * kTrBytes
+                                                      : (VAR & 8192) ? 9216 + kDfBytes
                                                       : (VAR & 1024) ? kCtBytes : 0);
   ensure_lds_attr(reinterpret_cast<const void*>(&k_spmm_bt<B, NG, EPI, AIG, VAR>), lds);
   hipLaunchKernelGGL((k_spmm_bt<B, NG, EPI, AIG, VAR>), dim3(grid), dim3(bt::kThreads), lds, s, a);
@@ -945,12 +986,26 @@
   if (ai_parts) *ai_parts = aig ? grid : 0;
   a.Cl = A.lfix_c;
   a.Qw = A.lfix_q;
+  a.skip = A.bt_skip;
+  if (A.defer_u) {
+    if (!A.lfix_c || b != 32 || f32 || a.hdr || a.Ah || !a.A || !epi || !aig || A.qloc ||
+        A.row0 != 0 || A.lfix_lo != 0 || A.lfix_hi != A.nrows)
+      return false;
+    a.lf_lo = 0;
+    a.lf_hi = A.nrows;
+    a.Ud = A.defer_u;
+    a.Rd1 = A.defer_r1;
+    a.Rd2 = A.defer_r2;
+    if (A.bt_ng == 9) launch_bt_v<32, 9, true, true, 3 | 1024 | 8192>(a, grid, s);
+    else launch_bt_v<32, 5, true, true, 3 | 1024 | 8192>(a, grid, s);
+    return true;
+  }
   if (A.lfix_c) {
     if (b != 32 || f32 || a.hdr || !epi || !aig) return false;
     a.lf_lo = A.lfix_lo;
     a.lf_hi = A.lfix_hi;
 #ifdef RBL_VARIANTS
-    if (bt2_on()) {
+    if (bt2_on() && !a.skip) {
       if (A.two_wave) *A.two_wave = 1;
       if (a.Ah) {
         if (A.bt_ng == 9) launch_bt2_v<9, true, true, 1024 | 2048>(a, grid, s);
@@ -1009,8 +1064,9 @@
 __global__ __launch_bounds__(64) void k_locfix(double* Q, const double* __restrict__ Qprev,
                                                const double* __restrict__ C, int64_t nrows,
                                                int64_t ntiles, int64_t tpw, const double* zrow,
-                                               int64_t wlo, int64_t whi) {
+                                               int64_t wlo, int64_t whi, const int* skip) {
   __shared__ __attribute__((aligned(16))) double ct[32 * kCtLd];
+  if (skip && *skip) return;
   const int lane = threadIdx.x;
   lf_table(C, ct, lane, 64);
   __syncthreads();
@@ -1074,14 +1130,14 @@
 }
 
 void spmm_bt_locfix_rest(const CsrDev& A, double* Q, const double* Qprev, const double* C,
-                         hipStream_t s) {
+                         hipStream_t s, const int* skip) {
   const int64_t grid = (A.ntiles + A.bt_tiles_per_wg - 1) / A.bt_tiles_per_wg;
   if (A.bt_ng == 9)
     hipLaunchKernelGGL(k_locfix<64>, dim3((unsigned)(grid * 8)), dim3(64), 0, s, Q, Qprev, C, A.nrows,
-                       A.ntiles, A.bt_tiles_per_wg, A.zrow, A.lfix_lo, A.lfix_hi);
+                       A.ntiles, A.bt_tiles_per_wg, A.zrow, A.lfix_lo, A.lfix_hi, skip);
   else
     hipLaunchKernelGGL(k_locfix<32>, dim3((unsigned)(grid * 4)), dim3(64), 0, s, Q, Qprev, C, A.nrows,
-                       A.ntiles, A.bt_tiles_per_wg, A.zrow, A.lfix_lo, A.lfix_hi);
+                       A.ntiles, A.bt_tiles_per_wg, A.zrow, A.lfix_lo, A.lfix_hi, skip);
 }
 
 __global__ void k_bt_fill(int64_t nrows, const int64_t* __restrict__ rowptr,
diff --git a/gpu-randomized-block-lanczos_amd/csrc/tri_apply.hpp b/gpu-randomized-block-lanczos_amd/csrc/tri_apply.hpp
--- /dev/null
+++ b/gpu-randomized-block-lanczos_amd/csrc/tri_apply.hpp
@@ -0,0 +1,73 @@
+#pragma once
+#include "rbl_common.hpp"
+
+namespace rbl {
+namespace tri {
+
+__device__ __forceinline__ double mfma4r(double a, double b, double c) {
+  return __builtin_amdgcn_mfma_f64_4x4x4f64(a, b, c, 0, 0, 0);
+}
+
+template <int B>
+__device__ __forceinline__ void table(const double* C, int ldc, double alpha, double* cs, int tid,
+                                      int nthreads) {
+  for (int e = tid; e < B * B; e += nthreads) {
+    const int k = e / B, c = e % B;
+    cs[k * (B + 8) + perm8(c)] = alpha * C[(int64_t)k * ldc + c];
+  }
+}
+
+template <bool TRI, int CG>
+__device__ __forceinline__ void mfma_row(const int k0, double a, const double* cb, double (&acc)[CG]) {
+#pragma unroll
+  for (int cp = 0; cp < CG / 2; ++cp) {
+    const bool z0 = TRI && k0 > 8 * cp + 3, z1 = TRI && k0 > 8 * cp + 7;
+    if (z0 && z1) continue;
+    const d2v bf = *reinterpret_cast<const d2v*>(cb + 8 * cp);
+    if (!z0) acc[2 * cp] = mfma4r(a, bf.x, acc[2 * cp]);
+    if (!z1) acc[2 * cp + 1] = mfma4r(a, bf.y, acc[2 * cp + 1]);
+  }
+  if constexpr (CG % 2) {
+    if (!(TRI && k0 > 4 * (CG - 1) + 3)) acc[CG - 1] = mfma4r(a, cb[8 * (CG / 2)], acc[CG - 1]);
+  }
+}
+
+template <bool TRI, int B>
+__device__ __forceinline__ void apply_acc(const d2v (&xa)[B / 8], const double* cs, int lane,
+                                          double (&acc)[B / 4]) {
+  const int q = lane >> 4, j = lane & 3;
+#pragma unroll
+  for (int h = 0; h < B / 8; ++h)
+#pragma unroll
+    for (int v = 0; v < 2; ++v) {
+      const double a = v ? xa[h].y : xa[h].x;
+      const double* cb = cs + (8 * h + 2 * q + v) * (B + 8) + 2 * j;
+      mfma_row<TRI>(8 * h + v, a, cb, acc);
+    }
+}
+
+template <int B>
+__device__ __forceinline__ int swz(int row, int c) {
+  return row * B + (c ^ (4 * ((row >> 2) & 3)));
+}
+
+template <bool TRI, int B>
+__device__ __forceinline__ void apply2(const d2v (&xa)[B / 8], const double* cs, const double* cs2,
+                                       double* ot, int lane, double (&acc)[B / 4]) {
+  constexpr int CG = B / 4, NH = B / 8;
+  const int q = lane >> 4, g = (lane >> 2) & 3, j = lane & 3;
+#pragma unroll
+  for (int cg = 0; cg < CG; ++cg) acc[cg] = 0.0;
+  apply_acc<TRI, B>(xa, cs, lane, acc);
+#pragma unroll
+  for (int cg = 0; cg < CG; ++cg) ot[swz<B>(4 * g + q, 4 * cg + j)] = acc[cg];
+  d2v x2[NH];
+#pragma unroll
+  for (int h = 0; h < NH; ++h) x2[h] = *reinterpret_cast<const d2v*>(ot + swz<B>(lane & 15, 8 * h + 2 * q));
+#pragma unroll
+  for (int cg = 0; cg < CG; ++cg) acc[cg] = 0.0;
+  apply_acc<TRI, B>(x2, cs2, lane, acc);
+}
+
+}
+}
diff --git a/gpu-randomized-block-lanczos_amd/rbl/_lib.py b/gpu-randomized-block-lanczos_amd/rbl/_lib.py
--- a/gpu-randomized-block-lanczos_amd/rbl/_lib.py
+++ b/gpu-randomized-block-lanczos_amd/rbl/_lib.py
@@ -28,6 +28,7 @@
 RBL_OPT_HALO_OVERLAP = 7
 RBL_OPT_RELABEL = 8
 RBL_OPT_HALO_PUSH = 9
+RBL_OPT_QR_DEFER = 10
 RBL_PATH_SPMM = 0
 RBL_PATH_SPMM_LOC_FUSED = 1
 RBL_PATH_LOC_SEPARATE = 2
@@ -36,7 +37,9 @@
 RBL_PATH_LOCFIX_REST = 5
 RBL_PATH_SPMM_TWO_WAVE = 6
 RBL_PATH_RITZ_PIECES = 7
-RBL_PATH_NSTATS = 8
+RBL_PATH_SPMM_QR_DEFERRED = 8
+RBL_PATH_QR_MATERIALISE = 9
+RBL_PATH_NSTATS = 10
 RBL_BUILD_VARIANTS = 1
 RBL_SPMM_KERNEL_RECT = 8
 RBL_MATRIX_FORMAT_RECT = 5
diff --git a/gpu-randomized-block-lanczos_amd/rbl/rbl_gpu.py b/gpu-randomized-block-lanczos_amd/rbl/rbl_gpu.py
--- a/gpu-randomized-block-lanczos_amd/rbl/rbl_gpu.py
+++ b/gpu-randomized-block-lanczos_amd/rbl/rbl_gpu.py
@@ -447,7 +447,8 @@
         self._check(lib.rbl_path_stats(self._h, i64ptr(out), L.RBL_PATH_NSTATS, int(reset)),
                     "rbl_path_stats")
         return dict(zip(("spmm", "spmm_loc_fused", "loc_separate", "loc_gram", "locfix_edges",
-                         "locfix_rest", "spmm_two_wave", "ritz_pieces"), (int(x) for x in out)))
+                         "locfix_rest", "spmm_two_wave", "ritz_pieces", "spmm_qr_deferred",
+                         "qr_materialise"), (int(x) for x in out)))
 
     def allgather(self, values) -> np.ndarray:
         mine = np.ascontiguousarray(np.asarray(values, dtype=np.int64).ravel())
diff --git a/include/rbl_hip.h b/include/rbl_hip.h
--- a/include/rbl_hip.h
+++ b/include/rbl_hip.h
@@ -43,6 +43,8 @@
 #define RBL_OPT_RELABEL       8
 
 #define RBL_OPT_HALO_PUSH     9
+
+#define RBL_OPT_QR_DEFER     10
 
 typedef struct rbl_ctx rbl_ctx;
 
@@ -164,7 +166,9 @@
 #define RBL_PATH_LOCFIX_REST     5
 #define RBL_PATH_SPMM_TWO_WAVE   6
 #define RBL_PATH_RITZ_PIECES     7
-#define RBL_PATH_NSTATS          8
+#define RBL_PATH_SPMM_QR_DEFERRED 8
+#define RBL_PATH_QR_MATERIALISE  9
+#define RBL_PATH_NSTATS          10
 int rbl_path_stats(rbl_ctx* ctx, int64_t* out, int nstats, int reset);
 
 int rbl_plan_row_partition(int64_t n, const int64_t* rowptr, int nranks, int64_t* bounds_out);
```

Result: no change. 45.39, median of 6 (+0.8%).
